# Gadersd/stable-diffusion-xl-burn

Measured on AMD Instinct MI355X. Metric: images/sec SDXL-base 1024x1024 30-step CFG7.5 (whole job); UNet step ms p50, higher is better.
Workload: dtype f16; 1 GPU; SDXL-base 1024x1024, n_steps=30 (31 CFG UNet step pairs), CFG 7.5, batch 1 prompt/GPU + VAE decode to u8 (BASELINE configs[1]); precision=f16, vae_dtype=f32_split, weights=synthetic seeded (random-init SDXL-base architecture), mix_classes=0, parallelism=replica x1, 1 prompt per GPU, weights broadcast once over RCCL, hipgraph=True, split_cfg=False, fused_xattn=True, pipelined_decode=False, prompts_per_call=1, full=False, library=stable-diffusion-xl-burn_amd/lib/libsdxl_mi355.so, debug_set=

## Files before the change

include/sdxl_mi355.h:

```cpp
#ifndef SDXL_MI355_H
#define SDXL_MI355_H

#include <stddef.h>
#include <stdint.h>

#ifdef __cplusplus
extern "C" {
#endif

typedef struct sdxl_ctx sdxl_ctx;
typedef struct sdxl_unet sdxl_unet;
typedef struct sdxl_diffuser sdxl_diffuser;
typedef struct sdxl_vae sdxl_vae;
typedef struct sdxl_clip sdxl_clip;

enum { SDXL_OK = 0, SDXL_ERR_INVALID = 1, SDXL_ERR_RUNTIME = 2 };
enum {
  SDXL_DTYPE_F32 = 0,
  SDXL_DTYPE_F16 = 1,
  SDXL_DTYPE_F16_F32RES = 2,
  SDXL_DTYPE_F32_SPLIT = 3,
  SDXL_DTYPE_F32_SPLIT_MIX = 4,
  SDXL_DTYPE_F32_SPLIT_MIX_F16W = 5,
  SDXL_DTYPE_F32_SPLIT_MIX_F16W_GEGLU2 = 6,
// ... 147 lines not shown
int sdxl_clip_create_synthetic(sdxl_ctx* ctx, const sdxl_clip_config* cfg, int dtype, uint64_t seed, sdxl_clip** out);
void sdxl_clip_destroy(sdxl_clip* c);
int sdxl_clip_forward_hidden(sdxl_clip* c, void* stream, const int32_t* tokens, int n, int seq, int hidden_idx, float* out_hidden);
int sdxl_clip_forward_hidden_pooled(sdxl_clip* c, void* stream, const int32_t* tokens, int n, int seq, int hidden_idx,
                                    float* out_hidden, float* out_pooled);
int sdxl_conditioning_embedding(sdxl_ctx* ctx, void* stream, const float* pooled, int n, int E, const int32_t* values, int w,
                                int dim, float* out);
int sdxl_clip_weight_arena(sdxl_clip* c, void** base, size_t* bytes);

int sdxl_unet_weight_arena(sdxl_unet* u, void** base, size_t* bytes);
int sdxl_vae_weight_arena(sdxl_vae* v, void** base, size_t* bytes);
int sdxl_diffuser_create_empty(sdxl_ctx* ctx, const sdxl_unet_config* cfg, int dtype, const float* alphas_cumprod_host,
                               int n_train_steps, sdxl_diffuser** out);
int sdxl_vae_create_empty(sdxl_ctx* ctx, const sdxl_vae_config* cfg, int dtype, int with_encoder, sdxl_vae** out);

typedef struct sdxl_comm sdxl_comm;
int sdxl_comm_unique_id(void* id_out_128);
int sdxl_comm_create(int device_id, int rank, int world, const void* id_128, sdxl_comm** out);
void sdxl_comm_destroy(sdxl_comm* c);
int sdxl_bcast_buffer(sdxl_comm* c, void* stream, void* base_dev, size_t bytes, int root);
int sdxl_unet_bcast_weights(sdxl_comm* c, sdxl_unet* u, int root);
int sdxl_vae_bcast_weights(sdxl_comm* c, sdxl_vae* v, int root);
int sdxl_clip_bcast_weights(sdxl_comm* c, sdxl_clip* k, int root);
int sdxl_bcast_plan(size_t bytes, int world, int rank, size_t* piece_off, size_t* piece_len, size_t* tail_off, size_t* tail_len);

int sdxl_unet_profile(sdxl_unet* u, void* stream, int B, int H, int W, float class_ms[5], int class_launches[5],
                      double class_flops[5]);
int sdxl_unet_eager_forward_ms(sdxl_unet* u, void* stream, int B, int H, int W, float* ms_out);
int sdxl_bench_igemm(sdxl_ctx* ctx, void* stream, int B, int H, int W, int Cin, int Cout, int ksize, int geglu, int iters,
                     float* avg_ms);
int sdxl_bench_attention(sdxl_ctx* ctx, void* stream, int B, int H, int Nq, int Nk, int iters, float* avg_ms);
int sdxl_debug_set(const char* key, int value);
int sdxl_debug_warm_schedule(int n, const unsigned* bytes, const unsigned char* host, int* warmed_by);
enum {
  SDXL_SEL_WF = 1 << 0, SDXL_SEL_R = 1 << 1, SDXL_SEL_EBIAS = 1 << 2, SDXL_SEL_STAT_OUT = 1 << 3, SDXL_SEL_LN_STAT = 1 << 4, SDXL_SEL_GN_PART = 1 << 5,
  SDXL_SEL_SHADOW = 1 << 6, SDXL_SEL_XA_K = 1 << 7, SDXL_SEL_XA_K_LO = 1 << 8, SDXL_SEL_ACC_SCALE = 1 << 9, SDXL_SEL_SPLITK_WS = 1 << 10,
  SDXL_SEL_XSPLIT_WS = 1 << 11, SDXL_SEL_MASK = 1 << 12, SDXL_SEL_WARM = 1 << 13
};
typedef struct sdxl_select_knobs {
  int igemm_variant, igemm_wreg, wreg_xattn, hl_tile96, igemm_tsw, igemm_unrolled, wide_db, attn_variant, attn_xsplit, zero_page;
} sdxl_select_knobs;
typedef struct sdxl_igemm_case {
  int batch, rows_per_entry;
  int N, cin, ksize, stride, up;
  int act, n_split;
  int a_dt, c_dt, compute_dt;
  int xa_nctx, shadow_lo_sign;
  unsigned present; int misaligned;
} sdxl_igemm_case;
typedef struct sdxl_igemm_choice {
  int family, bm, bn, ns, wgm, nw, elem, a_elem, xa, xh, tsw, s2, splitk, mode, db, measure, grid, block, lds;
  int gn_part_ok, wreg_selected, wreg_xattn_selected;
} sdxl_igemm_choice;
int sdxl_debug_igemm_select(const sdxl_igemm_case* c, const sdxl_select_knobs* knobs, sdxl_igemm_choice* out);
typedef struct sdxl_attn_case { int B, H, Nq, Nk, dt; unsigned present; int misaligned; } sdxl_attn_case;
typedef struct sdxl_attn_choice { int kernel, mix, big_heads, ns, elem, ko, grid_x, grid_y, block, lds; } sdxl_attn_choice;
int sdxl_debug_attn_select(const sdxl_attn_case* c, const sdxl_select_knobs* knobs, sdxl_attn_choice* out);

int sdxl_group_norm(sdxl_ctx* ctx, void* stream, const float* x, const float* gamma, const float* beta, int B, int C,
                    int HW, int n_group, float eps, int silu, int dtype, float* out);
int sdxl_layer_norm(sdxl_ctx* ctx, void* stream, const float* x, const float* gamma, const float* beta, int rows, int C,
                    float eps, int dtype, float* out);
int sdxl_conv2d(sdxl_ctx* ctx, void* stream, const float* x, const float* weight, const float* bias, int B, int Cin,
                int H, int W, int Cout, int ksize, int stride, int pad, int upsample, int dtype, float* out);
int sdxl_linear(sdxl_ctx* ctx, void* stream, const float* x, const float* weight, const float* bias, int M, int K, int N,
                int geglu, int dtype, float* out);
int sdxl_layer_norm_linear(sdxl_ctx* ctx, void* stream, const float* x, const float* gamma, const float* beta, float eps,
                           const float* weight, const float* bias, int M, int K, int N, int geglu, int dtype, float* out);

int sdxl_ln_query_cross_attention(sdxl_ctx* ctx, void* stream, const float* x, const float* gamma, const float* beta, float eps,
                                  const float* wq, const float* k, const float* v, int B, int Nq, int Nk, int C, int fused,
                                  float* out);

enum { SDXL_FORM_NATIVE = 0, SDXL_FORM_F16 = 1, SDXL_FORM_F16_WHILO = 2, SDXL_FORM_F16_AHILO = 3, SDXL_FORM_X2 = 4 };
enum { SDXL_PROJ_QKV = 0, SDXL_PROJ_QUERY = 1, SDXL_PROJ_GEGLU = 2 };
int sdxl_transformer_projection(sdxl_ctx* ctx, void* stream, int B, int rows_per_entry, int C, const float* a, const float* wp, const float* bp,
                                const float* r, int Kp, int producer_form, const float* gamma, const float* beta, float eps, const float* w,
                                const float* b, int N, int proj, int form, int shadow, float* t_out, float* out, int* shadow_taken);

int sdxl_conv2d_group_norm(sdxl_ctx* ctx, void* stream, const float* x, const float* weight, const float* bias, const float* residual,
                           const float* gamma, const float* beta, float eps, int B, int Cin, int H, int W, int Cout, int n_group,
                           int silu, int fused, int* fused_taken, float* out);

#ifdef __cplusplus
}
#endif
#endif
```

stable-diffusion-xl-burn_amd/__init__.py:

```python
from __future__ import annotations

import ctypes
import os
from dataclasses import dataclass, field
from typing import List, Optional, Sequence, Tuple

import numpy as np

_HERE = os.path.dirname(os.path.abspath(__file__))
LIB_PATH = os.path.join(_HERE, "lib", "libsdxl_mi355_measure.so" if os.environ.get("SDXL_MEASURE_LIB") == "1" else "libsdxl_mi355.so")
if os.environ.get("SDXL_LIB_PATH"):
    LIB_PATH = os.environ["SDXL_LIB_PATH"]

DTYPE_F32 = 0
DTYPE_F16 = 1
DTYPE_F16_F32RES = 2
DTYPE_F32_SPLIT_MIX_F16W = 5
DTYPE_F32_SPLIT_MIX_F16W_GEGLU2 = 6
DTYPE_F32_SPLIT_F16W = 7
DTYPE_F32_SPLIT_MIX = 4
DTYPE_F32_SPLIT = 3

_c_p = ctypes.c_void_p
_f_p = ctypes.c_void_p
# ... 22 lines not shown
class _ClipConfigC(ctypes.Structure):
    _fields_ = [(n, ctypes.c_int32) for n in ("n_vocab", "n_state", "embed_dim", "n_head", "n_ctx", "n_layer", "quick_gelu")]


class _ConditioningC(ctypes.Structure):
    _fields_ = [("unconditional_context_full", _f_p), ("unconditional_context_open_clip", _f_p),
                ("context_full", _f_p), ("context_open_clip", _f_p), ("unconditional_channel_context", _f_p),
                ("unconditional_channel_context_refiner", _f_p), ("channel_context", _f_p),
                ("channel_context_refiner", _f_p), ("n", ctypes.c_int32), ("n_ctx", ctypes.c_int32),
                ("height", ctypes.c_int32), ("width", ctypes.c_int32)]


class LoraEntry(ctypes.Structure):
    _fields_ = [("param_index", ctypes.c_int32), ("rank", ctypes.c_int32), ("left", _f_p), ("right", _f_p), ("scale", ctypes.c_float)]


LORA_ROUND_F16 = 1


ABI_SYMBOLS = [
    "sdxl_last_error", "sdxl_build_info", "sdxl_ctx_create", "sdxl_ctx_destroy", "sdxl_ctx_synchronize",
    "sdxl_unet_config_base", "sdxl_unet_config_refiner", "sdxl_vae_config_default",
    "sdxl_unet_param_count", "sdxl_unet_param_spec", "sdxl_vae_param_count", "sdxl_vae_param_spec",
    "sdxl_unet_create", "sdxl_unet_create_synthetic", "sdxl_unet_destroy", "sdxl_unet_forward", "sdxl_unet_set_graph", "sdxl_unet_set_split_cfg", "sdxl_unet_set_fused_cross_attention", "sdxl_unet_set_gn_from_producer", "sdxl_unet_mix_classes",
    "sdxl_qkv_attention", "sdxl_attn_decoder_mask",
    "sdxl_diffuser_create", "sdxl_diffuser_create_synthetic", "sdxl_diffuser_destroy", "sdxl_diffuser_unet",
    "sdxl_sample_latent", "sdxl_sample_latent_with_inpainting", "sdxl_refine_latent", "sdxl_step_count",
    "sdxl_diffuser_enable_step_timing", "sdxl_diffuser_step_times", "sdxl_diffuser_set_trace",
    "sdxl_gen_noise", "sdxl_sample_latent_seeded", "sdxl_sample_latent_with_inpainting_seeded", "sdxl_refine_latent_seeded",
    "sdxl_diffuser_set_solver", "sdxl_diffuser_get_solver", "sdxl_solver_coefficients",
    "sdxl_vae_create", "sdxl_vae_create_synthetic", "sdxl_vae_destroy", "sdxl_vae_decode_latent",
    "sdxl_latent_to_image", "sdxl_vae_encode_image", "sdxl_image_to_latent",
    "sdxl_unet_weight_arena", "sdxl_vae_weight_arena", "sdxl_diffuser_create_empty", "sdxl_vae_create_empty",
    "sdxl_unet_profile", "sdxl_unet_eager_forward_ms", "sdxl_bench_igemm", "sdxl_bench_attention", "sdxl_debug_set", "sdxl_debug_warm_schedule", "sdxl_debug_igemm_select", "sdxl_debug_attn_select",
    "sdxl_group_norm", "sdxl_layer_norm", "sdxl_conv2d", "sdxl_linear", "sdxl_layer_norm_linear", "sdxl_ln_query_cross_attention", "sdxl_conv2d_group_norm",
    "sdxl_transformer_projection",
    "sdxl_lora_check", "sdxl_lora_merge", "sdxl_unet_create_lora", "sdxl_diffuser_create_lora",
    "sdxl_clip_config_clip_l", "sdxl_clip_config_open_clip_bigg", "sdxl_clip_param_count", "sdxl_clip_param_spec",
    "sdxl_clip_create", "sdxl_clip_create_synthetic", "sdxl_clip_destroy", "sdxl_clip_forward_hidden",
    "sdxl_clip_forward_hidden_pooled", "sdxl_conditioning_embedding", "sdxl_clip_weight_arena",
    "sdxl_unet_create_f16", "sdxl_diffuser_create_f16", "sdxl_vae_create_f16", "sdxl_clip_create_f16",
    "sdxl_comm_unique_id", "sdxl_comm_create", "sdxl_comm_destroy", "sdxl_bcast_buffer", "sdxl_unet_bcast_weights",
    "sdxl_vae_bcast_weights", "sdxl_clip_bcast_weights", "sdxl_bcast_plan",
]

_lib = None


def lib() -> ctypes.CDLL:
    global _lib
    if _lib is None:
        if not os.path.exists(LIB_PATH):
            raise EngineError(f"{LIB_PATH} is missing: run `python stable-diffusion-xl-burn_amd/build.py` "
                              "(hipcc --offload-arch=gfx950). There is no fallback path.")
        try:
            import torch
        except ImportError:
            pass
        l = ctypes.CDLL(LIB_PATH)
        l.sdxl_last_error.restype = ctypes.c_char_p
        l.sdxl_build_info.restype = ctypes.c_char_p
        l.sdxl_diffuser_unet.restype = ctypes.c_void_p
        l.sdxl_diffuser_unet.argtypes = [ctypes.c_void_p]
        for name in ("sdxl_ctx_destroy", "sdxl_unet_destroy", "sdxl_diffuser_destroy", "sdxl_vae_destroy", "sdxl_clip_destroy",
                     "sdxl_comm_destroy"):
            getattr(l, name).restype = None
            getattr(l, name).argtypes = [ctypes.c_void_p]
# ... 834 lines not shown
    return out


def layer_norm(ctx: Context, x, gamma, beta, eps: float = 1e-5, dtype: int = DTYPE_F16):
    torch = _torch()
    x, px = _dev(x)
    gamma, pg = _dev(gamma)
    beta, pb = _dev(beta)
    C = x.shape[-1]
    out = torch.empty_like(x)
    _check(lib().sdxl_layer_norm(ctx.h, _stream(), px, pg, pb, int(x.numel() // C), C, ctypes.c_float(eps), dtype,
                                ctypes.c_void_p(out.data_ptr())))
    return out


def conv2d(ctx: Context, x, weight, bias, stride: int = 1, padding: int = 0, upsample: bool = False,
           dtype: int = DTYPE_F16):
    torch = _torch()
    x, px = _dev(x)
    weight, pw = _dev(weight)
    pb = None
    if bias is not None:
        bias, pb = _dev(bias)
    B, Cin, H, W = x.shape
    Cout, _, k, _ = weight.shape
    Hs, Ws = (2 * H, 2 * W) if upsample else (H, W)
    Ho, Wo = (Hs + 2 * padding - k) // stride + 1, (Ws + 2 * padding - k) // stride + 1
    out = torch.empty((B, Cout, Ho, Wo), device=x.device, dtype=torch.float32)
    _check(lib().sdxl_conv2d(ctx.h, _stream(), px, pw, pb, B, Cin, H, W, Cout, k, stride, padding, int(upsample), dtype,
                            ctypes.c_void_p(out.data_ptr())))
    return out


def linear(ctx: Context, x, weight, bias, geglu: bool = False, dtype: int = DTYPE_F16):
    torch = _torch()
    x, px = _dev(x)
    weight, pw = _dev(weight)
    pb = None
    if bias is not None:
        bias, pb = _dev(bias)
    K, N = weight.shape
    M = int(x.numel() // K)
    out = torch.empty(tuple(x.shape[:-1]) + ((N // 2) if geglu else N,), device=x.device, dtype=torch.float32)
    _check(lib().sdxl_linear(ctx.h, _stream(), px, pw, pb, M, K, N, int(geglu), dtype, ctypes.c_void_p(out.data_ptr())))
    return out


def layer_norm_linear(ctx: Context, x, gamma, beta, weight, bias, eps: float = 1e-5, geglu: bool = False,
                      dtype: int = DTYPE_F16):
    torch = _torch()
    x, px = _dev(x)
    gamma, pg = _dev(gamma)
    beta, pbeta = _dev(beta)
    weight, pw = _dev(weight)
    pb = None
    if bias is not None:
        bias, pb = _dev(bias)
    K, N = weight.shape
    M = int(x.numel() // K)
    out = torch.empty(tuple(x.shape[:-1]) + ((N // 2) if geglu else N,), device=x.device, dtype=torch.float32)
    _check(lib().sdxl_layer_norm_linear(ctx.h, _stream(), px, pg, pbeta, ctypes.c_float(eps), pw, pb, M, K, N, int(geglu),
                                       dtype, ctypes.c_void_p(out.data_ptr())))
    return out


def ln_query_cross_attention(ctx: Context, x, gamma, beta, wq, k, v, eps: float = 1e-5, fused: bool = True):
# ... 112 lines not shown
```

stable-diffusion-xl-burn_amd/build.py:

```python
from __future__ import annotations

import hashlib
import os
import subprocess
import sys
from concurrent.futures import ThreadPoolExecutor

HERE = os.path.dirname(os.path.abspath(__file__))
CSRC = os.path.join(HERE, "csrc")
OBJ = os.path.join(HERE, "build")
LIBDIR = os.path.join(HERE, "lib")
LIB = os.path.join(LIBDIR, "libsdxl_mi355.so")
ARCH = "gfx950"
SOURCES = ["igemm.hip", "igemm_glds.hip", "igemm_wreg.hip", "igemm_measure.hip", "norm.hip", "attention.hip", "elementwise.hip", "capi.hip", "capi_ops.hip",
           "select.cpp", "specs.cpp", "weights.cpp", "unet.cpp", "vae.cpp", "sampler.cpp", "clip.cpp", "comm.cpp"]
FLAGS = ["-O3", "-std=c++17", "-fPIC", f"--offload-arch={ARCH}", "-Wall", "-Wno-unused-function",
         "-Wno-unused-result"]


def _hipcc() -> str:
    for c in (os.environ.get("HIPCC"), "/opt/rocm/bin/hipcc", "hipcc"):
        if c and (os.path.isabs(c) and os.path.exists(c) or not os.path.isabs(c)):
            return c
    raise RuntimeError("hipcc not found")


def _measure() -> bool:
    return os.environ.get("SDXL_MEASURE") == "1"


def _paths():
    return (OBJ + "_measure", LIB.replace(".so", "_measure.so")) if _measure() else (OBJ, LIB)


def _flags() -> list:
    return FLAGS + (["-DSDXL_MEASURE"] if _measure() else [])


def _deps_hash(src: str) -> str:
    h = hashlib.sha256()
    for f in [src] + [os.path.join(CSRC, x) for x in ("kernels.h", "engine.h", "igemm_common.h", "capi_internal.h", "select_debug.h")] + \
            [os.path.join(HERE, "..", "include", "sdxl_mi355.h")]:
        with open(f, "rb") as fh:
            h.update(fh.read())
    h.update(" ".join(_flags()).encode())
    return h.hexdigest()


def _compile(name: str, force: bool) -> str:
    src = os.path.join(CSRC, name)
    obj = os.path.join(_paths()[0], name + ".o")
    stamp = obj + ".sha"
    want = _deps_hash(src)
    if not force and os.path.exists(obj) and os.path.exists(stamp) and open(stamp).read() == want:
        return obj
    cmd = [_hipcc()] + _flags() + (["-x", "hip"] if name.endswith(".hip") else []) + ["-c", src, "-o", obj]
    r = subprocess.run(cmd, capture_output=True, text=True)
    if r.returncode != 0:
        raise RuntimeError(f"hipcc failed for {name}:\n{r.stdout}\n{r.stderr}")
    with open(stamp, "w") as fh:
        fh.write(want)
    return obj


def build(force: bool = False, verbose: bool = True) -> str:
    obj_dir, lib = _paths()
    os.makedirs(obj_dir, exist_ok=True)
    os.makedirs(LIBDIR, exist_ok=True)
    with ThreadPoolExecutor(max_workers=min(8, len(SOURCES))) as ex:
        objs = list(ex.map(lambda n: _compile(n, force), SOURCES))
    newest = max(os.path.getmtime(o) for o in objs)
    if force or not os.path.exists(lib) or os.path.getmtime(lib) < newest:
        cmd = [_hipcc(), "-shared", "-fPIC", f"--offload-arch={ARCH}", "-o", lib] + objs + ["-ldl"]
        r = subprocess.run(cmd, capture_output=True, text=True)
# ... 12 lines not shown
```

stable-diffusion-xl-burn_amd/csrc/capi.hip:

```cpp
#include "capi_internal.h"
#include "select_debug.h"
#include <algorithm>
#include <cstring>

using namespace sdxl;

thread_local std::string sdxl::g_err;

namespace {
template <class H, class F> void create_handle(sdxl_ctx* ctx, H** out, F make) {
  std::unique_ptr<H> h(new H());
  h->ctx = ctx;
  make(*h);
  *out = h.release();
}
UNetCfg to_cfg(const sdxl_unet_config* c) {
  SDXL_REQUIRE(c != nullptr, "null config");
  SDXL_REQUIRE(c->n_levels >= 1 && c->n_levels <= 8, "n_levels out of range");
  UNetCfg u;
  u.adm_in_channels = c->adm_in_channels; u.in_channels = c->in_channels; u.out_channels = c->out_channels;
  u.model_channels = c->model_channels; u.n_head_channels = c->n_head_channels; u.context_dim = c->context_dim;
  u.is_refiner = c->is_refiner != 0;
  for (int i = 0; i < c->n_levels; ++i) { u.channel_mults.push_back(c->channel_mults[i]); u.transformer_depths.push_back(c->transformer_depths[i]); }
  SDXL_REQUIRE(u.model_channels > 0 && u.n_head_channels > 0 && u.context_dim > 0 && u.adm_in_channels > 0, "bad UNet config");
  return u;
}
ClipCfg to_ccfg(const sdxl_clip_config* c) {
  SDXL_REQUIRE(c != nullptr, "null config");
  ClipCfg k;
  k.n_vocab = c->n_vocab; k.n_state = c->n_state; k.embed_dim = c->embed_dim; k.n_head = c->n_head; k.n_ctx = c->n_ctx;
  k.n_layer = c->n_layer; k.quick_gelu = c->quick_gelu != 0;
  return k;
}
VaeCfg to_vcfg(const sdxl_vae_config* c) {
// ... 73 lines not shown
#ifdef SDXL_MEASURE
  return "sdxl_mi355 engine, HIP kernels for gfx950 (CDNA4, wave64, MFMA 32x32x16 f16 / 32x32x2 f32) [measure build: A/B variants + debug knobs]";
#else
  return "sdxl_mi355 engine, HIP kernels for gfx950 (CDNA4, wave64, MFMA 32x32x16 f16 / 32x32x2 f32)";
#endif
}

int sdxl_ctx_create(int device_id, sdxl_ctx** out) {
  API_BEGIN
  SDXL_REQUIRE(out != nullptr, "null out");
  int n = 0;
  SDXL_HIP(hipGetDeviceCount(&n));
  SDXL_REQUIRE(n > 0, "no HIP device visible: the MI355X engine has no CPU fallback");
  SDXL_REQUIRE(device_id >= 0 && device_id < n, "device id out of range");
  SDXL_HIP(hipSetDevice(device_id));
  sdxl_ctx* c = new sdxl_ctx();
  c->device = device_id;
  SDXL_HIP(hipStreamCreate(&c->stream));
  igemm_glds_init();
  *out = c;
  API_END
}
int sdxl_debug_set(const char* key, int value) {
  API_BEGIN
  SDXL_REQUIRE(key != nullptr, "null key");
  if (select_knob_set(key, value)) return SDXL_OK;
  else if (std::strcmp(key, "igemm_epilogue_staged") == 0) igemm_set_epilogue_staged(value);
  else if (std::strcmp(key, "hl_weights_exact") == 0) igemm_set_hl_weights_exact(value);
  else if (std::strcmp(key, "igemm_warm") == 0) igemm_set_warm(value);
  else if (std::strcmp(key, "splitk_wt") == 0) igemm_set_splitk_wt(value);
  else if (std::strcmp(key, "hl_demote") == 0) unet_set_hl_demote(value);
  else if (std::strcmp(key, "mix_classes") == 0) unet_set_mix_classes(value);
  else if (std::strcmp(key, "wreg_xcd2d") == 0) igemm_set_wreg_xcd2d(value);
#ifdef SDXL_MEASURE
  else if (std::strcmp(key, "xa_vec64") == 0) igemm_set_xa_vec64(value);
  else if (std::strcmp(key, "no_cfg") == 0) g_debug_no_cfg = value != 0;
#endif
  else throw Error(std::string("unknown debug key ") + key);
  API_END
}
int sdxl_debug_warm_schedule(int n, const unsigned* bytes, const unsigned char* host, int* warmed_by) {
  API_BEGIN
  WarmSeq ws;
  for (int j = 0; j < n; ++j)
    ws.seq.push_back(WarmSeq::Item{reinterpret_cast<const void*>((uintptr_t)(j + 1) << 12), bytes[j], host[j] != 0, host[j] ? 14u << 20 : 0u, {nullptr, nullptr, nullptr}, {0u, 0u, 0u}});
  ws.finish();
  for (int j = 0; j < n; ++j) warmed_by[j] = -1;
  for (int i = 0; i < n; ++i)
    for (int r = 0; r < 3; ++r)
      if (ws.seq[i].warm[r]) warmed_by[(int)(reinterpret_cast<uintptr_t>(ws.seq[i].warm[r]) >> 12) - 1] = i;
  API_END
}
int sdxl_debug_igemm_select(const sdxl_igemm_case* c, const sdxl_select_knobs* knobs, sdxl_igemm_choice* out) {
  API_BEGIN
  SDXL_REQUIRE(c && knobs && out, "null argument");
  const IgemmParams p = select_debug_igemm(*c);
  const SelectKnobs k = select_debug_knobs(*knobs);
  *out = sdxl_igemm_choice{};
  out->gn_part_ok = igemm_gn_part_ok(p, k); out->wreg_selected = igemm_wreg_selected(p, k); out->wreg_xattn_selected = igemm_wreg_xattn_selected(p, k);
  const IgemmChoice s = igemm_select(p, c->compute_dt, k);
  out->family = s.family; out->bm = s.bm; out->bn = s.bn; out->ns = s.ns; out->wgm = s.wgm; out->nw = s.nw; out->elem = s.elem; out->a_elem = s.a_elem;
  out->xa = s.xa; out->xh = s.xh; out->tsw = s.tsw; out->s2 = s.s2; out->splitk = s.splitk; out->mode = s.mode; out->db = s.db; out->measure = s.measure;
  out->grid = s.grid; out->block = s.block; out->lds = s.lds;
  API_END
}
int sdxl_debug_attn_select(const sdxl_attn_case* c, const sdxl_select_knobs* knobs, sdxl_attn_choice* out) {
  API_BEGIN
  SDXL_REQUIRE(c && knobs && out, "null argument");
  const AttnChoice s = attn_select(select_debug_attn(*c), select_debug_knobs(*knobs));
  *out = sdxl_attn_choice{s.kernel, s.mix, s.big_heads, s.ns, s.elem, s.ko, s.grid_x, s.grid_y, s.block, s.lds};
  API_END
}
#ifdef SDXL_MEASURE
int sdxl_debug_timeline(void* device_buf) {
  API_BEGIN
  igemm_set_timeline(device_buf);
  API_END
}
int sdxl_debug_timeline_words(void) { return igemm_timeline_words(); }
int sdxl_debug_attn_timeline(void* device_buf) {
  API_BEGIN
  attention_set_timeline(device_buf);
  API_END
// ... 534 lines not shown
```

stable-diffusion-xl-burn_amd/csrc/capi_ops.hip:

```cpp
#include "capi_internal.h"
#include <algorithm>
#include <cmath>

using namespace sdxl;

namespace {
__global__ void transpose_pad_kernel(const float* src, int lds_, int rows, int C, void* dst, int dt, int ldd) {
  const size_t i = (size_t)blockIdx.x * blockDim.x + threadIdx.x;
  if (i >= (size_t)rows * C) return;
  const int r = i / C, c = i - (size_t)r * C;
  const float v = src[(size_t)r * lds_ + c];
  if (dt == DT_F16) reinterpret_cast<_Float16*>(dst)[(size_t)c * ldd + r] = (_Float16)v;
  else reinterpret_cast<float*>(dst)[(size_t)c * ldd + r] = v;
}
__global__ void causal_mask_kernel(float* out, int n) {
  const int i = blockIdx.x * blockDim.x + threadIdx.x;
  if (i >= n * n) return;
  const int r = i / n, c = i - r * n;
  out[i] = c > r ? -INFINITY : 0.f;
}

struct Operand { std::string name; std::vector<int> shape; int kind; const float* data = nullptr; float eps = 0.f; int ld = 0; };
using Operands = std::vector<Operand>;
void add_linear(Operands& o, const std::string& n, int K, int N, const float* w, const float* b, int ld = 0) {
// ... 288 lines not shown
                int W, int Cout, int ksize, int stride, int pad, int upsample, int dtype, float* out) {
  API_BEGIN
  SDXL_REQUIRE(ctx && x && weight && out, "null argument");
  use(ctx);
  hipStream_t s = pick(ctx, stream);
  int cdt, sdt;
  if (dtype == SDXL_DTYPE_F32_SPLIT) { cdt = DT_HL; sdt = DT_HL; }
  else { no_mix(dtype); dtypes(dtype, cdt, sdt); }
  SDXL_REQUIRE(cdt != DT_HL || Cin % 32 == 0, "SDXL_DTYPE_F32_SPLIT convolutions need Cin % 32 == 0");
  const int Hs = upsample ? 2 * H : H, Ws = upsample ? 2 * W : W;
  const int Ho = (Hs + 2 * pad - ksize) / stride + 1, Wo = (Ws + 2 * pad - ksize) / stride + 1;
  Operands ops;
  add_conv(ops, "conv", Cout, Cin, ksize, weight, bias);
  Packed pk(ops, cdt, s);
  const Lin l = pk.wb.conv("conv");
  Tmp tmp;
  void* xi = tmp.get((size_t)B * H * W * Cin * dt_size(sdt));
  float* yo = (float*)tmp.get((size_t)B * Ho * Wo * Cout * sizeof(float));
  Act xa(xi, Cin, sdt);
  if (cdt == DT_HL) {
    float* x32 = (float*)tmp.get((size_t)B * H * W * Cin * sizeof(float));
    float* sc = (float*)tmp.get(hl_scale_floats(B) * sizeof(float));
    launch_nchw_to_nhwc(x, Cin * H * W, x32, DT_F32, B, Cin, H * W, Cin, 1.0f, s);
    launch_f32_to_hl_scaled(x32, Cin, xi, Cin, (size_t)B * H * W, Cin, sc, s, B);
    xa.a_scale = hl_scale_inv(sc, B); xa.a_scale_n = B;
  } else launch_nchw_to_nhwc(x, Cin * H * W, xi, sdt, B, Cin, H * W, Cin, 1.0f, s);
  Exec ex; ex.s = s; ex.cdt = cdt; ex.sdt = sdt;
  give_splitk_ws(ex, tmp, B, Ho * Wo, Cout, s);
  run_conv(ex, l, xa, Cin, ConvGeom{B, H, W, Ho, Wo, ksize, stride, pad, upsample ? 1 : 0}, Act(yo, Cout, DT_F32));
  launch_nhwc_to_nchw(yo, DT_F32, Cout, out, B, Cout, Ho * Wo, 1.0f, s);
  SDXL_HIP(hipStreamSynchronize(s));
  API_END
}
int sdxl_linear(sdxl_ctx* ctx, void* stream, const float* x, const float* weight, const float* bias, int M, int K, int N,
                int geglu, int dtype, float* out) {
  API_BEGIN
  SDXL_REQUIRE(ctx && x && weight && out, "null argument");
  SDXL_REQUIRE(!geglu || (N % 32 == 0), "GEGLU width must be a multiple of 32");
  use(ctx);
  hipStream_t s = pick(ctx, stream);
  int cdt, sdt;
  if (dtype == SDXL_DTYPE_F32_SPLIT) { cdt = DT_HL; sdt = DT_HL; }
  else { no_mix(dtype); dtypes(dtype, cdt, sdt); }
  SDXL_REQUIRE(cdt != DT_HL || K % 32 == 0, "SDXL_DTYPE_F32_SPLIT linear layers need K % 32 == 0");
  Operands ops;
  add_linear(ops, "lin", K, N, weight, bias);
  Packed pk(ops, cdt, s);
  const Lin l = pk.wb.linear("lin", geglu != 0);
  Tmp tmp;
  void* xi = tmp.get((size_t)M * K * dt_size(sdt));
  Act xa(xi, K, sdt);
  if (cdt == DT_HL) {
    float* sc = (float*)tmp.get(hl_scale_floats(1) * sizeof(float));
    launch_f32_to_hl_scaled(x, K, xi, K, (size_t)M, K, sc, s, 1);
    xa.a_scale = hl_scale_inv(sc, 1);
  } else launch_copy_rows(x, DT_F32, K, xi, sdt, K, M, K, s);
  Exec ex; ex.s = s; ex.cdt = cdt; ex.sdt = sdt;
  give_splitk_ws(ex, tmp, 1, M, N, s);
  Epi e; e.act = geglu ? 1 : 0;
  run_linear(ex, l, xa, M, Act(out, geglu ? N / 2 : N, DT_F32), e);
  SDXL_HIP(hipStreamSynchronize(s));
  API_END
}
int sdxl_layer_norm_linear(sdxl_ctx* ctx, void* stream, const float* x, const float* gamma, const float* beta, float eps,
                           const float* weight, const float* bias, int M, int K, int N, int geglu, int dtype, float* out) {
  API_BEGIN
// ... 237 lines not shown
```

stable-diffusion-xl-burn_amd/csrc/elementwise.hip:

```cpp
#include "kernels.h"
#include <algorithm>
#include <stdexcept>

namespace sdxl {

typedef _Float16 half_t;
typedef _Float16 half8 __attribute__((ext_vector_type(8)));
typedef float f32x4 __attribute__((ext_vector_type(4)));

__device__ __forceinline__ float ld_f(const void* p, size_t i, int dt) {
  if (dt == DT_HL) { const half_t* b = reinterpret_cast<const half_t*>(p) + ((i >> 4) << 5) + (i & 15); return (float)b[0] + (float)b[16]; }
  return dt == DT_F16 ? (float)reinterpret_cast<const half_t*>(p)[i] : reinterpret_cast<const float*>(p)[i];
}
__device__ __forceinline__ void st_f(void* p, size_t i, int dt, float v) {
  if (dt == DT_HL) {
    half_t* b = reinterpret_cast<half_t*>(p) + ((i >> 4) << 5) + (i & 15);
    const half_t hi = (half_t)v;
    b[0] = hi; b[16] = (half_t)(v - (float)hi);
  } else if (dt == DT_F16) reinterpret_cast<half_t*>(p)[i] = (half_t)v; else reinterpret_cast<float*>(p)[i] = v;
}
__device__ __forceinline__ float silu_f(float x) { return x / (1.0f + expf(-x)); }

template <typename WT>
__global__ __launch_bounds__(256) void gemv_kernel(const GemvParams p, int cols) {
  constexpr int CE = 16 / sizeof(WT);
  extern __shared__ __attribute__((aligned(16))) float gx[];
  const int lane = threadIdx.x & 63, wave = threadIdx.x >> 6;
  const int Kx = (p.K + 64 * CE - 1) / (64 * CE) * (64 * CE);
  for (int i = threadIdx.x; i < p.Bm * Kx; i += 256) {
    const int b = i / Kx, k = i - b * Kx;
    float x = 0.f;
    if (k < p.K) {
      x = p.X[(size_t)b * p.ldx + k];
// ... 772 lines not shown
  for (int o = 32; o > 0; o >>= 1) acc += __shfl_xor(acc, o);
  if (lane == 0) cs[row] = acc;
}
void launch_colsum_packed(const void* wp, int dt, int Kpad, int nrows, float* cs, hipStream_t s, const float* kscale, int K, int interleave) {
  hipLaunchKernelGGL(colsum_packed_kernel, dim3((nrows + 3) / 4), dim3(256), 0, s, wp, dt, Kpad, nrows, cs, kscale, K, interleave);
}
__global__ void beta_dot_kernel(const float* w, const float* beta, const float* bias, float* out, int K, int N) {
  const int n = blockIdx.x * blockDim.x + threadIdx.x;
  if (n >= N) return;
  float acc = bias ? bias[n] : 0.f;
  for (int k = 0; k < K; ++k) acc += beta[k] * w[(size_t)k * N + n];
  out[n] = acc;
}
void launch_beta_dot(const float* w, const float* beta, const float* bias, float* out, int K, int N, hipStream_t s) {
  hipLaunchKernelGGL(beta_dot_kernel, dim3((N + 255) / 256), dim3(256), 0, s, w, beta, bias, out, K, N);
}
__global__ void pack_conv_kernel(const float* src, void* dst, int dt, int Cout, int Cin, int ks, int Kpad, int Npad, float wscale) {
  const size_t i = (size_t)blockIdx.x * blockDim.x + threadIdx.x;
  if (i >= (size_t)Npad * Kpad) return;
  const int n = i / Kpad;
  const int k = i - (size_t)n * Kpad;
  float v = 0.f;
  if (n < Cout && k < ks * ks * Cin) {
    const int tap = k / Cin, c = k - tap * Cin;
    const int ky = tap / ks, kx = tap - ky * ks;
    v = src[(((size_t)n * Cin + c) * ks + ky) * ks + kx] * wscale;
  }
  st_f(dst, i, dt, v);
}
void launch_pack_conv(const float* src, void* dst, int dt, int Cout, int Cin, int ks, int Kpad, int Npad, hipStream_t s, float wscale) {
  const size_t total = (size_t)Npad * Kpad;
  hipLaunchKernelGGL(pack_conv_kernel, dim3((total + 255) / 256), dim3(256), 0, s, src, dst, dt, Cout, Cin, ks, Kpad, Npad, wscale);
}
__global__ void pack_bias_kernel(const float* src, float* dst, int N, int Npad, int geglu, int n_offset) {
  const int i = blockIdx.x * blockDim.x + threadIdx.x;
  if (i >= Npad) return;
  float v = 0.f;
  if (i < N && src) v = src[geglu ? geglu_unpermute(i, N) : i];
  dst[n_offset + i] = v;
}
void launch_pack_bias(const float* src, float* dst, int N, int Npad, int geglu, int n_offset, hipStream_t s) {
  hipLaunchKernelGGL(pack_bias_kernel, dim3((Npad + 255) / 256), dim3(256), 0, s, src, dst, N, Npad, geglu, n_offset);
}

}
```

stable-diffusion-xl-burn_amd/csrc/engine.h:

```cpp
#pragma once
#include "kernels.h"

#include <map>
#include <memory>
#include <stdexcept>
#include <string>
#include <utility>
#include <vector>

namespace sdxl {

struct Error : std::runtime_error {
  explicit Error(const std::string& m) : std::runtime_error(m) {}
};
#define SDXL_HIP(x)                                                                                   \
  do {                                                                                                \
    hipError_t e__ = (x);                                                                             \
    if (e__ != hipSuccess) throw ::sdxl::Error(std::string(#x) + " failed: " + hipGetErrorString(e__)); \
  } while (0)
#define SDXL_REQUIRE(cond, msg)                          \
  do {                                                   \
    if (!(cond)) throw ::sdxl::Error(std::string(msg));  \
  } while (0)

// ... 70 lines not shown
struct FlatSourceF16 : WeightSource {
  const uint16_t* base; std::vector<size_t> offsets;
  void* stage = nullptr; size_t stage_numel = 0;
  FlatSourceF16(const uint16_t* b, const std::vector<ParamSpec>& specs);
  ~FlatSourceF16() override;
  void fetch(const ParamSpec& s, size_t index, float* dst_dev, hipStream_t st) override;
};

struct LoraEntry { int param_index = 0, rank = 0; const float* left = nullptr; const float* right = nullptr; float scale = 0.f; };
constexpr int kLoraRoundF16 = 1;
std::string lora_check(const std::vector<ParamSpec>& specs, const LoraEntry* entries, int n_entries);
struct LoraSource : WeightSource {
  WeightSource& inner;
  std::vector<LoraEntry> entries;
  std::vector<std::vector<int>> by_param;
  int flags;
  float* stage = nullptr; size_t stage_numel = 0;
  LoraSource(WeightSource& in, const std::vector<ParamSpec>& specs, const LoraEntry* e, int n_entries, int flags);
  ~LoraSource() override;
  void fetch(const ParamSpec& s, size_t index, float* dst_dev, hipStream_t st) override;
  bool empty() const override { return inner.empty(); }
};

struct Lin {
  const void* w = nullptr; const float* b = nullptr;
  const void* wf = nullptr;
  int N = 0, K = 0, Kpad = 0, Npad = 0, ksize = 1, cin = 0;
  const float* cs = nullptr;
  const float* ln_eps = nullptr;
  int ln_k = 0;
  int k_form = 0;
  int dt = -1;
  const float* acc_scale = nullptr;
};
struct NormW { const float* gamma = nullptr; const float* beta = nullptr; const float* eps = nullptr; int C = 0; };

struct WeightBuilder {
  const std::vector<ParamSpec>& specs;
  std::map<std::string, size_t> index;
  WeightSource& src;
  DeviceArena& arena;
  int dt;
  hipStream_t st;
  float* tmp = nullptr; size_t tmp_numel = 0;
  std::string last_fetched;
  WeightBuilder(const std::vector<ParamSpec>& sp, WeightSource& s, DeviceArena& a, int dtype, hipStream_t stream);
  ~WeightBuilder();
  bool wfrag = true;
  static size_t arena_bound(const std::vector<ParamSpec>& specs, int dt, bool wfrag = true);
  const ParamSpec& spec(const std::string& name, size_t* idx = nullptr) const;
  bool has(const std::string& name) const { return index.count(name) != 0; }
  const float* fetch(const std::string& name);
  Lin linear(const std::string& name, bool geglu = false, int dt_override = -1);
  Lin fused_linear(const std::vector<std::string>& names, int dt_override = -1);
  Lin linear_hilo(const std::string& name, bool geglu, bool dup = false, bool hl_interleave = false);
  float hl_scale(Lin& l, const std::vector<std::string>& weight_names);
  Lin linear_ln(const std::string& name, bool geglu, const std::string& norm, bool xattn_query = false);
  Lin fused_linear_ln(const std::vector<std::string>& names, const std::string& norm);
  Lin fold_ln(const std::vector<std::string>& names, const std::string& norm, bool geglu, int dt_override = -1, bool shadow = false, Lin* plain = nullptr, bool hilo_dup = false,
              bool hl_interleave = false);
  bool all_f16_exact(const std::vector<std::string>& names);
  float* tmp2 = nullptr; size_t tmp2_numel = 0;
  Lin conv(const std::string& name);
  void attach_wfrag(Lin& l, bool fill, bool folded = false);
  NormW norm(const std::string& name);
};

struct Act {
  void* p = nullptr; int ld = 0; int dt = DT_F16;
  const float* gn_part = nullptr; int gn_rt = 0;
  const float* a_scale = nullptr;
  int a_scale_n = 1;
  Act() {}
  Act(void* p_, int ld_, int dt_) : p(p_), ld(ld_), dt(dt_) {}
  Act cols(int c0) const { Act a((char*)p + (size_t)c0 * dt_size(dt), ld, dt); a.a_scale = a_scale; a.a_scale_n = a_scale_n; return a; }
};

struct Profiler {
  enum { IGEMM = 0, ATTENTION = 1, GROUPNORM = 2, LAYERNORM = 3, OTHER = 4, NCLS = 5 };
  struct Rec { hipEvent_t a, b; int cls; double flops; int m, n, k, ks, tag; };
  std::vector<Rec> recs;
  void begin(int cls, double flops, hipStream_t s, int m = 0, int n = 0, int k = 0, int ks = 0, int tag = 0);
  void end(hipStream_t s);
  void collect(float ms[NCLS], int launches[NCLS], double flops[NCLS]);
};

struct WarmSeq {
  struct Item { const void* w; unsigned bytes; bool host; unsigned budget; const void* warm[3]; unsigned warm_bytes[3]; };
  std::vector<Item> seq;
  size_t pos = 0;
  bool recording = false, ready = false;
  void finish();
};
struct Exec {
  Profiler* prof = nullptr;
  hipStream_t s = nullptr;
// ... 19 lines not shown
  MIX_ATTN_F16 = 1,
  MIX_GEGLU_F16 = 2,
  MIX_QKV_F16 = 4,
  MIX_FF_F16 = 8,
  MIX_OUT1_F16 = 16,
  MIX_OUT2_F16 = 32,
  MIX_XATTN_F16 = 64,
  MIX_Q2_F16 = 128,
  MIX_XATTN_SPLIT = 512,
  MIX_GEGLU_HILO = 1024,
  MIX_GEGLU_AHILO = 2048,
  MIX_LINEAR_F16X2 = 4096,
  MIX_LN_SHADOW = 256
};
enum DemoteClass { DM_QKV = 1, DM_ATTN = 2, DM_OUT = 4, DM_XATTN = 8, DM_GEGLU = 16, DM_FF = 32, DM_CONV_RES = 64, DM_CONV_SKIP = 128,
                   DM_CONV_IO = 256, DM_CONV_UPDOWN = 512, DM_CONV_PROJ = 1024 };
void unet_set_mix_classes(int v);
void unet_set_hl_demote(int mask);
int unet_hl_demote();

struct ConvGeom { int B, Hin, Win, Hout, Wout, ksize, stride, pad, up; };
struct Epi {
  const float* ln_stat = nullptr;
  float* stat_out = nullptr;
  const float* ebias = nullptr; int ebias_ld = 0;
  int act = 0;
  Act R;
  int n_split = -1;
  void* Ct = nullptr; int ct_rows = 0, ct_ld = 0;
  int rpb = 0;
  const void* xa_k = nullptr; int xa_nctx = 0; float xa_scale = 0.f;
  const void* xa_k_lo = nullptr;
  float* gn_part = nullptr;
  int cls = 0;
  void* shadow = nullptr; int shadow_ld = 0; const float* shadow_gamma = nullptr; bool* shadow_done = nullptr; float shadow_lo_scale = 0.f;
};
bool run_conv(Exec& ex, const Lin& w, const Act& a, int cin, const ConvGeom& g, const Act& out, const Epi& e = Epi());
bool run_linear(Exec& ex, const Lin& w, const Act& a, int M, const Act& out, const Epi& e = Epi());
Act hl_operand(Exec& ex, const Lin& w, const Act& x, size_t rows, int C, int nb = 1, float* have_max = nullptr);
void run_groupnorm(Exec& ex, const NormW& n, const Act& x, int B, int HW, const Act& y, bool silu, int groups = 32, float* absmax_out = nullptr);
void run_layernorm(Exec& ex, const NormW& n, const Act& x, int rows, const Act& y, float dup_scale = 0.f);

struct ResBlockW { NormW norm_in, norm_out; Lin conv_in, conv_out, skip; bool has_skip = false; int emb_off = 0, cin = 0, cout = 0; };
struct TBlockW { NormW n1, n2, n3; Lin qkv, out1, q2, kv2, out2, geglu, ff;
                 Lin qkv_sh, q2_sh, geglu_sh; };
enum LinForm {
  LF_NATIVE,
  LF_F16,
  LF_F16_WHILO,
  LF_F16_AHILO,
  LF_X2
};
inline bool packs_f16_values(LinForm f) { return f == LF_F16 || f == LF_F16_AHILO || f == LF_X2; }
enum XattnForm { XA_LAUNCH, XA_F16, XA_SPLIT };
struct StPlan {
  LinForm qkv = LF_NATIVE, out1 = LF_NATIVE, q2 = LF_NATIVE, out2 = LF_NATIVE, geglu = LF_NATIVE, ff = LF_NATIVE;
  bool qkv_sh = false, q2_sh = false, geglu_sh = false;
  bool attn_f16 = false;
  XattnForm xattn = XA_LAUNCH;
};
struct STW { NormW norm; Lin proj_in, proj_out; std::vector<TBlockW> blocks; int C = 0, heads = 0; StPlan plan; };
Lin pack_proj(WeightBuilder& wb, LinForm f, const std::vector<std::string>& names, bool geglu, Lin* sh = nullptr, const std::string& norm = "");
inline bool reads_f16(LinForm f) { return f == LF_F16 || f == LF_F16_WHILO || f == LF_F16_AHILO; }
inline Act x2_operand(LinForm f, const Act& a) { return f == LF_X2 ? Act(a.p, 2 * a.ld, DT_F16) : a; }
struct LnOperands {
  Act ln;
  Act ln16;
  Act ln16x2;
  Act sh16; float* shst = nullptr;
  Act sh16g;
// ... 82 lines not shown
  hipGraphExec_t graph_ = nullptr;
  const float* graph_t_ = nullptr; int graph_ts_ = 0; int plan_runs_ = 0;
};

struct VaeResW { NormW n1, n2; Lin c1, c2, nin; bool has_nin = false; int cin = 0, cout = 0; };
struct VaeMidW { VaeResW b1, b2; NormW an; Lin q, k, v, proj; int C = 0; };

class Vae {
 public:
  Vae(const VaeCfg& cfg, int compute_dt, WeightSource* dec_src, WeightSource* enc_src, hipStream_t st);
  ~Vae();
  const VaeCfg& cfg() const { return cfg_; }
  const float* decode(const float* latent_nchw, int n, int h, int w, hipStream_t s);
  void decode_nchw(const float* latent_nchw, int n, int h, int w, float* out_nchw, hipStream_t s);
  void latent_to_image(const float* latent_nchw, int n, int h, int w, unsigned char* out_hwc, hipStream_t s);
  void encode_nchw(const float* img_nchw, int n, int H, int W, float* latent_out, hipStream_t s);
  void image_to_latent(const unsigned char* img_hwc, int n, int H, int W, float* latent_out, hipStream_t s);
  size_t weight_bytes() const { return warena_.off; }
  void* weight_base() const { return warena_.base; }

 private:
  void res_block(Exec& ex, const VaeResW& w, const Act& x, int B, int H, int W, const Act& out);
  void mid(Exec& ex, const VaeMidW& w, const Act& x, int B, int H, int W);
  void run_decode(Exec& ex, const Act& in, int n, int h, int w, const Act& out);
  void run_encode(Exec& ex, const Act& in, int n, int H, int W, const Act& out);
  VaeResW load_res(WeightBuilder& wb, const std::string& p, int cin, int cout);
  VaeMidW load_mid(WeightBuilder& wb, const std::string& p, int c);

  VaeCfg cfg_;
  int cdt_;
  DeviceArena warena_;
  bool has_dec_ = false, has_enc_ = false;
  Lin post_quant_, d_conv_in_, d_conv_out_; NormW d_norm_out_; VaeMidW d_mid_;
  struct DecBlk { VaeResW r[3]; Lin up; bool has_up = false; };
  std::vector<DecBlk> d_blocks_;
  Lin quant_, e_conv_in_, e_conv_out_; NormW e_norm_out_; VaeMidW e_mid_;
  struct EncBlk { VaeResW r[2]; Lin down; bool has_down = false; };
  std::vector<EncBlk> e_blocks_;
  DeviceArena act_;
  size_t act_peak_ = 0;
  float* gn_workspace(Exec& ex, int n);
  int io_dt() const { return cdt_ == DT_HL ? DT_F32 : cdt_; }
};

struct ClipBlockW { NormW attn_ln, mlp_ln; Lin qkv, out, fc1, fc2; };

class ClipText {
 public:
  ClipText(const ClipCfg& cfg, int compute_dt, int stream_dt, WeightSource& src, hipStream_t st);
  ~ClipText();
  void set_use_graph(bool g) { use_graph_ = g; }
  const ClipCfg& cfg() const { return cfg_; }
  void forward_hidden(const int* ids, int B, int S, int hidden_idx, float* out, hipStream_t s);
  void forward_hidden_pooled(const int* ids, int B, int S, int hidden_idx, float* hidden, float* pooled, hipStream_t s);
  size_t weight_bytes() const { return warena_.off; }
  void* weight_base() const { return warena_.base; }

 private:
  void run(const int* ids, int B, int S, int n_blocks, int tap, float* hidden, float* pooled, hipStream_t s);
  void block(Exec& ex, const ClipBlockW& w, const Act& x, int B, int S, const Act& ln, const Act& qk, void* vt, int npad,
             const Act& ao, const Act& h);
  ClipCfg cfg_;
  int cdt_, sdt_;
  DeviceArena warena_, act_;
  const void* tok_ = nullptr; const void* pos_ = nullptr;
  std::vector<ClipBlockW> blocks_;
  NormW final_ln_; Lin proj_;
// ... 67 lines not shown
```

stable-diffusion-xl-burn_amd/csrc/igemm_common.h:

```cpp
#pragma once
#include "kernels.h"
#include <stdexcept>
#include <type_traits>

namespace sdxl {

typedef _Float16 half_t;
typedef _Float16 half8 __attribute__((ext_vector_type(8)));
typedef _Float16 half4 __attribute__((ext_vector_type(4)));
typedef float f32x4 __attribute__((ext_vector_type(4)));
typedef float f32x16 __attribute__((ext_vector_type(16)));

typedef const __attribute__((address_space(1))) void* gptr_t;
typedef float f32x8 __attribute__((ext_vector_type(8)));
__device__ __forceinline__ f32x8 uniform_load8(const float* ptr) {
  const unsigned long long a = (unsigned long long)(uintptr_t)ptr;
  const unsigned long long u = ((unsigned long long)__builtin_amdgcn_readfirstlane((unsigned)(a >> 32)) << 32) | (unsigned)__builtin_amdgcn_readfirstlane((unsigned)a);
  return *(const __attribute__((address_space(4))) f32x8*)(uintptr_t)u;
}
__device__ __forceinline__ f32x4 col_vec4(const float* arr, bool present, int nbu, int fh, const void* zeros) {
  const f32x8 c = uniform_load8(present ? arr + nbu : reinterpret_cast<const float*>(zeros));
  return fh ? f32x4{c[4], c[5], c[6], c[7]} : f32x4{c[0], c[1], c[2], c[3]};
}
typedef __attribute__((address_space(3))) void* lptr_t;
// ... 87 lines not shown
  __device__ __forceinline__ static float combine(const float (&P)[NC]) {
    if constexpr (TPR == 4) { const float t = P[0] + __shfl_xor(P[0], 1); return t + __shfl_xor(t, 2); }
    else { const float u = P[0] + __shfl_xor(P[0], 1), w = P[1] + __shfl_xor(P[1], 1); return u + w; }
  }
  __device__ __forceinline__ void finish(const IgemmParams& p, int m0, float* coef) {
    if (!live) return;
    float P[NC];
#pragma unroll
    for (int c = 0; c < NC; ++c) {
      P[c] = 0.f;
#pragma unroll
      for (int q = 0; q < PERC; ++q) if (sub + c * TPR + 4 * q < p.ln_slots) P[c] += v[c][q][0];
    }
    const float mu = combine(P) / (float)p.ln_slots;
    float Q[NC], D[NC];
#pragma unroll
    for (int c = 0; c < NC; ++c) {
      Q[c] = 0.f; D[c] = 0.f;
#pragma unroll
      for (int q = 0; q < PERC; ++q)
        if (sub + c * TPR + 4 * q < p.ln_slots) { const float d = v[c][q][0] - mu; Q[c] += v[c][q][1]; D[c] = fmaf(d, d, D[c]); }
    }
    const float s2 = combine(Q), sd = combine(D);
    const float var = (s2 + 64.f * sd) * p.ln_invc;
    const float a = 1.0f / sqrtf(var + (p.ln_eps_ptr ? *p.ln_eps_ptr : p.ln_eps));
    if (sub == 0) {
      const bool ok = m0 + row < p.M;
      coef[row * 2] = ok ? a : 1.f;
      coef[row * 2 + 1] = ok ? -a * mu : 0.f;
    }
  }
};

template <int TM, int TN>
__device__ __forceinline__ void igemm_epilogue(const IgemmParams& p, const f32x16 (&acc)[TM][TN], int mw, int nw, int fr, int fh,
                                               const float (&lnA)[TM], const float (&lnC)[TM]) {
  const bool geglu = p.act == 1;
  const int nlim = geglu ? (p.N >> 1) : p.N;
#pragma unroll
  for (int i = 0; i < TM; ++i) {
    const int m = mw + i * 32 + fr;
    if (m >= p.M) continue;
    const int bidx = m / p.rpb;
    const int key = m - bidx * p.rpb;
    const float lna = lnA[i], lnc = lnC[i];
#pragma unroll
    for (int j = 0; j < TN; ++j) {
      const int nt = nw + j * 32;
#pragma unroll
      for (int q = 0; q < 4; ++q) {
        if (geglu && q >= 2) continue;
        const int nb = nt + 8 * q + 4 * fh;
        if (nb >= p.N) continue;
        float v[4];
#pragma unroll
        for (int r = 0; r < 4; ++r) v[r] = acc[i][j][q * 4 + r];
        if (p.ln_stat) {
          const f32x4 cz = *reinterpret_cast<const f32x4*>(p.ln_cs + nb);
#pragma unroll
          for (int r = 0; r < 4; ++r) v[r] = lna * v[r] + lnc * cz[r];
        }
        if (p.bias) {
          const f32x4 bz = *reinterpret_cast<const f32x4*>(p.bias + nb);
#pragma unroll
          for (int r = 0; r < 4; ++r) v[r] += bz[r];
        }
        if (p.ebias) {
          const f32x4 ez = *reinterpret_cast<const f32x4*>(p.ebias + (size_t)bidx * p.ebias_ld + nb);
#pragma unroll
          for (int r = 0; r < 4; ++r) v[r] += ez[r];
        }
        int nout = nb;
        if (geglu) {
          f32x4 gz = {0.f, 0.f, 0.f, 0.f};
          if (p.bias) gz = *reinterpret_cast<const f32x4*>(p.bias + nb + 16);
          f32x4 gc = {0.f, 0.f, 0.f, 0.f};
          if (p.ln_stat) gc = *reinterpret_cast<const f32x4*>(p.ln_cs + nb + 16);
#pragma unroll
          for (int r = 0; r < 4; ++r) v[r] *= gelu_erf2(lna * acc[i][j][(q + 2) * 4 + r] + lnc * gc[r] + gz[r]);
          nout = (nt >> 1) + 8 * q + 4 * fh;
        }
        if (geglu || nb < p.n_split) {
          const bool vec = nout + 3 < nlim && (nout & 3) == 0;
          if (p.R) {
            if (vec && p.r_dt == DT_F16 && (p.ldr & 3) == 0) {
              const half4 rr = *reinterpret_cast<const half4*>(reinterpret_cast<const half_t*>(p.R) + (size_t)m * p.ldr + nout);
#pragma unroll
              for (int r = 0; r < 4; ++r) v[r] += (float)rr[r];
            } else if (vec && p.r_dt == DT_F32 && (p.ldr & 3) == 0) {
              const f32x4 rr = *reinterpret_cast<const f32x4*>(reinterpret_cast<const float*>(p.R) + (size_t)m * p.ldr + nout);
#pragma unroll
              for (int r = 0; r < 4; ++r) v[r] += rr[r];
            } else {
#pragma unroll
              for (int r = 0; r < 4; ++r)
                if (nout + r < nlim)
                  v[r] += p.r_dt == DT_F16 ? (float)reinterpret_cast<const half_t*>(p.R)[(size_t)m * p.ldr + nout + r]
                                           : reinterpret_cast<const float*>(p.R)[(size_t)m * p.ldr + nout + r];
            }
          }
          if (vec && p.c_dt == DT_F16 && (p.ldc & 3) == 0) {
            half4 h; h[0] = (half_t)v[0]; h[1] = (half_t)v[1]; h[2] = (half_t)v[2]; h[3] = (half_t)v[3];
            *reinterpret_cast<half4*>(reinterpret_cast<half_t*>(p.C) + (size_t)m * p.ldc + nout) = h;
          } else if (vec && p.c_dt == DT_F32 && (p.ldc & 3) == 0) {
            f32x4 o = {v[0], v[1], v[2], v[3]};
            *reinterpret_cast<f32x4*>(reinterpret_cast<float*>(p.C) + (size_t)m * p.ldc + nout) = o;
          } else {
#pragma unroll
            for (int r = 0; r < 4; ++r)
              if (nout + r < nlim) {
                if (p.c_dt == DT_F16) reinterpret_cast<half_t*>(p.C)[(size_t)m * p.ldc + nout + r] = (half_t)v[r];
                else reinterpret_cast<float*>(p.C)[(size_t)m * p.ldc + nout + r] = v[r];
              }
          }
        } else {
#pragma unroll
          for (int r = 0; r < 4; ++r)
            if (nb + r < p.N) {
              const size_t o = ((size_t)bidx * p.ct_rows + (nb + r - p.n_split)) * p.ct_ld + key;
              if (p.c_dt == DT_F16) reinterpret_cast<half_t*>(p.Ct)[o] = (half_t)v[r];
              else reinterpret_cast<float*>(p.Ct)[o] = v[r];
            }
        }
      }
    }
  }
}

__host__ __device__ constexpr int pipe_lds_total(int ring, int extra) { return ring + extra + 2048 <= 163840 ? ring + extra + 2048 : ring + extra; }

typedef int warm_i32x4 __attribute__((ext_vector_type(4)));
template <int NT>
__device__ __forceinline__ void igemm_warm_body(const void* base, unsigned bytes, int wi, int nw) {
  const char* b = reinterpret_cast<const char*>(base);
  constexpr unsigned span = NT * 16, step = span * 8;
  warm_i32x4 acc = {0, 0, 0, 0};
  for (size_t off = (size_t)wi * step; off < bytes; off += (size_t)nw * step) {
    warm_i32x4 v[8];
#pragma unroll
    for (int u = 0; u < 8; ++u) {
      const size_t o = off + (size_t)u * span + (size_t)threadIdx.x * 16;
      v[u] = o + 16 <= bytes ? *reinterpret_cast<const warm_i32x4*>(b + o) : warm_i32x4{0, 0, 0, 0};
    }
#pragma unroll
    for (int u = 0; u < 8; ++u) acc ^= v[u];
// ... 115 lines not shown
    bool rfast[NIT];
    constexpr bool GNP = TM == 2 && TN == 2 && !GEGLU;
    const bool gnp = GNP && gc != nullptr && p.gn_part != nullptr;
    float gpiv[8], gs1[8], gs2[8];
#pragma unroll
    for (int e = 0; e < 8; ++e) { gpiv[e] = 0.f; gs1[e] = 0.f; gs2[e] = 0.f; }
    float st_piv[NIT], st_s1[NIT], st_s2[NIT];
    size_t st_off[NIT];
    bool st_ok[NIT];
#pragma unroll
    for (int it = 0; it < NIT; ++it) { st_piv[it] = 0.f; st_s1[it] = 0.f; st_s2[it] = 0.f; st_off[it] = 0; st_ok[it] = false; }
#pragma unroll
    for (int it = 0; it < NIT; ++it) {
      const int idx = it * 64 + lane;
      const int row = idx / LPR, piece = idx - row * LPR;
      const int n0 = nwo + piece * 8;
      const int m = mw + row;
      const half_t* rp = reinterpret_cast<const half_t*>(p.R) + (size_t)m * p.ldr + n0;
      rfast[it] = p.R && p.r_dt == DT_F16 && idx < ITEMS && m < p.M && n0 + 8 <= nlim && (reinterpret_cast<uintptr_t>(rp) & 15) == 0;
      rpre[it] = *(rfast[it] ? reinterpret_cast<const half8*>(rp) : reinterpret_cast<const half8*>(zeros));
    }
#pragma unroll
    for (int it = 0; it < NIT; ++it) {
      const int idx = it * 64 + lane;
      const int row = idx / LPR, piece = idx - row * LPR;
      if (ITEMS % 64 != 0 && idx >= ITEMS) continue;
      const int n0 = nwo + piece * 8;
      const int m = mw + row;
      const f32x4 a = *reinterpret_cast<const f32x4*>(lds + row * RB + (((2 * piece) ^ (row & SWN)) << 4));
      const f32x4 b = *reinterpret_cast<const f32x4*>(lds + row * RB + (((2 * piece + 1) ^ (row & SWN)) << 4));
      const bool valid = m < p.M && n0 < nlim;
      float rr[8] = {0.f, 0.f, 0.f, 0.f, 0.f, 0.f, 0.f, 0.f};
      if (valid) {
      float v[8] = {a[0], a[1], a[2], a[3], b[0], b[1], b[2], b[3]};
      const bool full = n0 + 8 <= nlim;
      if (rfast[it]) {
#pragma unroll
        for (int e = 0; e < 8; ++e) v[e] += (float)rpre[it][e];
      } else if (p.R) {
        if (p.r_dt == DT_F16) {
          const half_t* rp = reinterpret_cast<const half_t*>(p.R) + (size_t)m * p.ldr + n0;
          if (full && (reinterpret_cast<uintptr_t>(rp) & 15) == 0) {
            const half8 rr = *reinterpret_cast<const half8*>(rp);
#pragma unroll
            for (int e = 0; e < 8; ++e) v[e] += (float)rr[e];
          } else {
#pragma unroll
            for (int e = 0; e < 8; ++e) if (n0 + e < nlim) v[e] += (float)rp[e];
          }
        } else {
          const float* rp = reinterpret_cast<const float*>(p.R) + (size_t)m * p.ldr + n0;
          if (full && (reinterpret_cast<uintptr_t>(rp) & 15) == 0) {
            const f32x4 r0 = *reinterpret_cast<const f32x4*>(rp), r1 = *reinterpret_cast<const f32x4*>(rp + 4);
#pragma unroll
            for (int e = 0; e < 4; ++e) { v[e] += r0[e]; v[4 + e] += r1[e]; }
          } else {
#pragma unroll
            for (int e = 0; e < 8; ++e) if (n0 + e < nlim) v[e] += rp[e];
          }
        }
      }
      if (p.stat_out || gnp) {
#pragma unroll
        for (int e = 0; e < 8; ++e) rr[e] = p.c_dt == DT_F16 ? (float)(half_t)v[e] : v[e];
      }
      if (p.c_dt == DT_F16) {
        half_t* cp = reinterpret_cast<half_t*>(p.C) + (size_t)m * p.ldc + n0;
        if (full && (reinterpret_cast<uintptr_t>(cp) & 15) == 0) {
          half8 h;
#pragma unroll
          for (int e = 0; e < 8; ++e) h[e] = (half_t)v[e];
          *reinterpret_cast<half8*>(cp) = h;
        } else {
#pragma unroll
          for (int e = 0; e < 8; ++e) if (n0 + e < nlim) cp[e] = (half_t)v[e];
        }
      } else if (p.c_dt == DT_HL) {
        if (full) store_hl8(reinterpret_cast<float*>(p.C) + (size_t)m * p.ldc, n0, v);
      } else {
        float* cp = reinterpret_cast<float*>(p.C) + (size_t)m * p.ldc + n0;
        if (full && (reinterpret_cast<uintptr_t>(cp) & 15) == 0) {
          *reinterpret_cast<f32x4*>(cp) = f32x4{v[0], v[1], v[2], v[3]};
          *reinterpret_cast<f32x4*>(cp + 4) = f32x4{v[4], v[5], v[6], v[7]};
        } else {
#pragma unroll
          for (int e = 0; e < 8; ++e) if (n0 + e < nlim) cp[e] = v[e];
        }
      }
      }
      if constexpr (GNP) {
        if (gnp) {
          if (it == 0) {
#pragma unroll
            for (int e = 0; e < 8; ++e) gpiv[e] = __shfl(rr[e], lane & 7);
          }
#pragma unroll
          for (int e = 0; e < 8; ++e) { const float d = rr[e] - gpiv[e]; gs1[e] += d; gs2[e] = fmaf(d, d, gs2[e]); }
        }
      }
      if constexpr (COLS % 64 == 0) {
        if (p.stat_out) {
          const float piv = __shfl(rr[0], lane & ~7);
          float s1 = 0.f, s2 = 0.f;
#pragma unroll
          for (int e = 0; e < 8; ++e) { const float d = rr[e] - piv; s1 += d; s2 = fmaf(d, d, s2); }
          st_piv[it] = piv; st_s1[it] = s1; st_s2[it] = s2;
          st_ok[it] = (piece & 7) == 0 && valid;
          st_off[it] = ((size_t)(n0 >> 6) * p.M + m) * 2;
        }
      }
    }
    if constexpr (COLS % 64 == 0) {
      if (p.stat_out) {
// ... 89 lines not shown
          const int m = mbase + e;
          if (m < p.M) {
            const int bb = m / p.rpb;
            reinterpret_cast<float*>(p.Ct)[((size_t)bb * p.ct_rows + (n - p.n_split)) * p.ct_ld + (m - bb * p.rpb)] = v[e];
          }
        }
      }
    }
  }
}

template <int TM, int TN, bool GEGLU>
__device__ __forceinline__ bool igemm_rows_ok(const IgemmParams& p, int nw) {
  constexpr int WN = TN * 32;
  const int nlim = GEGLU ? (p.N >> 1) : (p.n_split < p.N ? p.n_split : p.N);
  const int n_lo = GEGLU ? (nw >> 1) : nw, n_w = GEGLU ? WN / 2 : WN;
  if (n_lo + n_w > nlim || p.gn_part) return false;
  if ((p.ldc & 7) != 0 || (reinterpret_cast<uintptr_t>(p.C) & 15) != 0) return false;
  if (p.R && ((p.ldr & 7) != 0 || (reinterpret_cast<uintptr_t>(p.R) & 15) != 0)) return false;
  if (p.stat_out && (TN != 2 || GEGLU)) return false;
  if (p.ebias && (p.ebias_ld & 3) != 0) return false;
  return true;
}
struct NoStamp { __device__ __forceinline__ void operator()(int) const {} };
template <int TM, int TN, bool GEGLU, typename ST = NoStamp>
__device__ __forceinline__ void igemm_epilogue_rows(const IgemmParams& p, const f32x16 (&acc)[TM][TN], int mw, int nw, int lane,
                                                    const float (&lnA)[TM], const float (&lnC)[TM], const void* zeros, const ST& stamp = ST()) {
  const int fr = lane & 31, fh = lane >> 5;
  const f32x4* zv = reinterpret_cast<const f32x4*>(zeros);
  constexpr int NQ = GEGLU ? 2 : 4;
  constexpr int NP = NQ / 2;
  const int nwo = GEGLU ? (nw >> 1) : nw;
  int m[TM], bidx[TM];
  bool mok[TM];
#pragma unroll
  for (int i = 0; i < TM; ++i) {
    m[i] = mw + i * 32 + fr;
    mok[i] = m[i] < p.M;
    bidx[i] = (p.ebias && mok[i]) ? m[i] / p.rpb : 0;
  }
  const bool r16 = p.R && p.r_dt == DT_F16, r32 = p.R && p.r_dt == DT_F32;
  half8 rh[TM][TN][NP];
  f32x4 rf[TM][TN][NP][2];
#pragma unroll
  for (int i = 0; i < TM; ++i)
#pragma unroll
    for (int j = 0; j < TN; ++j)
#pragma unroll
      for (int t = 0; t < NP; ++t) {
        const int n0 = nwo + (GEGLU ? j * 16 : j * 32 + t * 16) + 8 * fh;
        const size_t o = (size_t)(mok[i] ? m[i] : 0) * p.ldr + n0;
        rh[i][j][t] = *((r16 && mok[i]) ? reinterpret_cast<const half8*>(reinterpret_cast<const half_t*>(p.R) + o) : reinterpret_cast<const half8*>(zeros));
        if (r32) {
          rf[i][j][t][0] = *(mok[i] ? reinterpret_cast<const f32x4*>(reinterpret_cast<const float*>(p.R) + o) : zv);
          rf[i][j][t][1] = *(mok[i] ? reinterpret_cast<const f32x4*>(reinterpret_cast<const float*>(p.R) + o + 4) : zv);
        }
      }
  stamp(0);
  float st_s1[TM][4], st_s2[TM][4], st_piv[TM];
#pragma unroll
  for (int i = 0; i < TM; ++i) {
    st_piv[i] = 0.f;
#pragma unroll
    for (int k = 0; k < 4; ++k) { st_s1[i][k] = 0.f; st_s2[i][k] = 0.f; }
  }
#pragma unroll
  for (int j = 0; j < TN; ++j) {
    const int nt = nw + j * 32;
    f32x4 bz[NQ], cz[NQ], gz[NQ], gc[NQ], ez[TM][NQ];
#pragma unroll
    for (int q = 0; q < NQ; ++q) {
      const int nb = nt + 8 * q + 4 * fh;
// ... 13 lines not shown
      const float lna = lnA[i], lnc = lnC[i];
      f32x4 v[NQ];
#pragma unroll
      for (int q = 0; q < NQ; ++q) {
#pragma unroll
        for (int r = 0; r < 4; ++r) v[q][r] = acc[i][j][q * 4 + r];
        v[q] = lna * v[q] + lnc * cz[q] + bz[q] + ez[i][q];
        if constexpr (GEGLU) {
#pragma unroll
          for (int r = 0; r < 4; ++r) v[q][r] *= gelu_erf2(lna * acc[i][j][(q + 2) * 4 + r] + lnc * gc[q][r] + gz[q][r]);
        }
      }
#pragma unroll
      for (int t = 0; t < NP; ++t) {
        float w[8];
#pragma unroll
        for (int r = 0; r < 4; ++r) {
          const auto sw = __builtin_amdgcn_permlane32_swap(__float_as_uint(v[2 * t][r]), __float_as_uint(v[2 * t + 1][r]), false, false);
          w[r] = __uint_as_float(sw[0]);
          w[4 + r] = __uint_as_float(sw[1]);
        }
        if (r16) {
#pragma unroll
          for (int e = 0; e < 8; ++e) w[e] += (float)rh[i][j][t][e];
        } else if (r32) {
#pragma unroll
          for (int e = 0; e < 4; ++e) { w[e] += rf[i][j][t][0][e]; w[4 + e] += rf[i][j][t][1][e]; }
        }
        const int n0 = nwo + (GEGLU ? j * 16 : j * 32 + t * 16) + 8 * fh;
        if (p.c_dt == DT_F16) {
          half8 h;
#pragma unroll
          for (int e = 0; e < 8; ++e) h[e] = (half_t)w[e];
          if (mok[i]) *reinterpret_cast<half8*>(reinterpret_cast<half_t*>(p.C) + (size_t)m[i] * p.ldc + n0) = h;
          if constexpr (TN == 2 && !GEGLU) {
            if (p.stat_out) {
#pragma unroll
              for (int e = 0; e < 8; ++e) w[e] = (float)h[e];
            }
          }
        } else if (p.c_dt == DT_HL) {
          if (mok[i]) store_hl8(reinterpret_cast<float*>(p.C) + (size_t)m[i] * p.ldc, n0, w);
        } else if (mok[i]) {
          float* cp = reinterpret_cast<float*>(p.C) + (size_t)m[i] * p.ldc + n0;
          *reinterpret_cast<f32x4*>(cp) = f32x4{w[0], w[1], w[2], w[3]};
          *reinterpret_cast<f32x4*>(cp + 4) = f32x4{w[4], w[5], w[6], w[7]};
        }
        if constexpr (TN == 2 && !GEGLU) {
          if (p.stat_out) {
            if (j == 0 && t == 0) st_piv[i] = __shfl(w[0], fr);
            float s1 = 0.f, s2 = 0.f;
#pragma unroll
            for (int e = 0; e < 8; ++e) { const float d = w[e] - st_piv[i]; s1 += d; s2 = fmaf(d, d, s2); }
            st_s1[i][j * 2 + t] = s1; st_s2[i][j * 2 + t] = s2;
          }
        }
      }
    }
  }
  stamp(7);
  if constexpr (TN == 2 && !GEGLU) {
    if (p.stat_out) {
#pragma unroll
      for (int i = 0; i < TM; ++i) {
#pragma unroll
        for (int k = 0; k < 4; ++k) { st_s1[i][k] += __shfl_xor(st_s1[i][k], 32); st_s2[i][k] += __shfl_xor(st_s2[i][k], 32); }
        const float s1 = (st_s1[i][0] + st_s1[i][1]) + (st_s1[i][2] + st_s1[i][3]);
        const float s2 = (st_s2[i][0] + st_s2[i][1]) + (st_s2[i][2] + st_s2[i][3]);
        if (fh == 0 && mok[i]) {
          float* dst = p.stat_out + ((size_t)(nw >> 6) * p.M + m[i]) * 2;
          dst[0] = st_piv[i] + s1 * (1.0f / 64.0f);
          dst[1] = fmaxf(s2 - s1 * s1 * (1.0f / 64.0f), 0.f);
        }
      }
    }
  }
}
// ... 342 lines not shown
```

stable-diffusion-xl-burn_amd/csrc/igemm_glds.hip:

```cpp
#include "igemm_common.h"
#include <atomic>

namespace sdxl {

template <int BM, int BN, int NS, int MINB = 2>
__global__ __launch_bounds__(256, MINB) void igemm_glds_kernel(const IgemmParams p, const void* zeros) {
  kernarg_prefetch<(int)sizeof(IgemmParams) + 8>();
  constexpr int WM = BM / 2, WN = BN / 2;
  constexpr int TM = WM / 32, TN = WN / 32;
  constexpr int AJ = BM / 32, BJ = BN / 32;
  constexpr int PER = AJ + BJ;
  constexpr int KT = 64;
  constexpr int STAGE = (BM + BN) * 128;
  extern __shared__ __attribute__((aligned(16))) char smem[];

  const int tid = threadIdx.x, lane = tid & 63;
  const int wave = __builtin_amdgcn_readfirstlane(tid >> 6);
  const int wm = wave >> 1, wn = wave & 1;

  const int tilesN = (p.N + BN - 1) / BN;
  const int nwg = gridDim.x;
  int bid = blockIdx.x;
  {
    const int q = nwg >> 3, r = nwg & 7, xcd = bid & 7, idx = bid >> 3;
// ... 130 lines not shown
  constexpr int AJ = BM / (8 * NW), BJ = (BPC + NW - 1) / NW;
  constexpr int REM = BPC % NW;
  constexpr int PER = AJ + BJ;
  static_assert(BM % (8 * NW) == 0 && WM % 32 == 0 && WN % 32 == 0 && BN % 8 == 0, "bad tile");
  constexpr int KT = 8 * CE;
  constexpr int STAGE = (BM + BN) * 128;
  constexpr bool LIN = XA;
  static_assert(NS >= 3, "counted-wait pipeline needs a ring of at least 3 slots");
  static_assert(BM * 128 + (TN - 1) * 4096 < 65536, "fragment offsets must fit the ds_read immediate");
  extern __shared__ __attribute__((aligned(16))) char smem[];
  const unsigned lds0 = (unsigned)(uintptr_t)(lptr_t)smem;

  const int tid = threadIdx.x, lane = tid & 63;
  const int wave = __builtin_amdgcn_readfirstlane(tid >> 6);
  const int wm = wave / WGN, wn = wave % WGN;
  const bool lastb = REM == 0 || wave < REM;

  const int tilesN = (p.N + BN - 1) / BN;
  const int tilesM = (p.M + BM - 1) / BM;
  const int nwg = gridDim.x;
  int bid = blockIdx.x;
  {
    const int q = nwg >> 3, r = nwg & 7, xcd = bid & 7, idx = bid >> 3;
    bid = (xcd < r ? xcd * (q + 1) : r * (q + 1) + (xcd - r) * q) + idx;
  }
  const int SK = p.splitk > 1 ? p.splitk : 1;
  const int slice = SK > 1 ? bid % SK : 0;
  if (SK > 1) bid /= SK;
  const int tile_id = bid;
  int tm, tn;
  if ((size_t)p.N * p.K > (size_t)p.M * p.Cin) { tn = bid / tilesM; tm = bid - tn * tilesM; }
  else { tm = bid / tilesN; tn = bid - tm * tilesN; }
  const int m0 = tm * BM, n0 = tn * BN;
  bool tsw_swapped = false;
  if constexpr (TSW) {
    const int ok = n0 >= p.n_split && n0 + BN <= p.N && p.c_dt == DT_F16 && p.act == 0 && !p.epi_staged && (p.rpb % BM) == 0 && m0 + BM <= p.M &&
                   (p.ct_ld & 7) == 0 && (reinterpret_cast<uintptr_t>(p.Ct) & 15) == 0 && (!p.ln_stat || p.ln_slots <= 24);
    tsw_swapped = __builtin_amdgcn_readfirstlane(ok) != 0;
  }
  auto wait_tiles = [&](auto KK) {
    constexpr int k = decltype(KK)::value;
    if constexpr (REM == 0) wait_vmcnt<PER * k>();
    else { if (lastb) wait_vmcnt<PER * k>(); else wait_vmcnt<(PER - 1) * k>(); }
  };

  const int lrow = lane >> 3, slot = lane & 7;
  const T* wptr[BJ];
#pragma unroll
  for (int j = 0; j < BJ; ++j) {
    const int row = (j * NW + wave) * 8 + lrow;
    wptr[j] = reinterpret_cast<const T*>(p.W) + (size_t)(n0 + row) * p.Kpad + (slot ^ ((row >> 1) & 7)) * CE;
  }
  const int nk_all = p.Kpad / KT;
  const int kbeg = SK > 1 ? (int)((long)slice * nk_all / SK) : 0;
  const int nk = SK > 1 ? (int)((long)(slice + 1) * nk_all / SK) - kbeg : nk_all;
  if (kbeg > 0) {
#pragma unroll
    for (int j = 0; j < BJ; ++j) wptr[j] += kbeg * KT;
  }
  constexpr bool B0_EARLY = !LIN;
  if constexpr (B0_EARLY) {
    if (nk > 0) {
      char* lb0 = smem + BM * 128 + wave * 1024;
      static_for<BJ>([&](auto J) {
        constexpr int j = decltype(J)::value;
        if (j < BJ - 1 || lastb) {
          __builtin_amdgcn_global_load_lds((gptr_t)wptr[j], (lptr_t)(lb0 + j * (NW * 1024)), 16, 0, 0);
          wptr[j] += KT;
        }
      });
      __builtin_amdgcn_sched_barrier(0);
    }
  }
  const int HWo = p.Hout * p.Wout;
  const int Hup = p.Hin << p.up, Wup = p.Win << p.up;
  const bool lin_rows = p.ksize == 1 && p.stride == 1 && p.up == 0 && p.pad == 0;
  const bool pow2 = (HWo & (HWo - 1)) == 0 && (p.Wout & (p.Wout - 1)) == 0;
  const int sh_hw = __builtin_ctz((unsigned)HWo | 0x40000000u), sh_w = __builtin_ctz((unsigned)p.Wout | 0x40000000u);
  int rb[AJ], ry[AJ], rx[AJ], rsw[AJ];
#pragma unroll
  for (int j = 0; j < AJ; ++j) {
    const int row = (j * NW + wave) * 8 + lrow;
    const int m = m0 + row;
    rsw[j] = (slot ^ ((row >> 1) & 7)) * CE;
    rb[j] = m < p.M ? m : -1; ry[j] = 0; rx[j] = 0;
    if (!lin_rows) {
      if (m < p.M) {
        int b, rem, oy;
        if (pow2) { b = m >> sh_hw; rem = m & (HWo - 1); oy = rem >> sh_w; }
        else { b = m / HWo; rem = m - b * HWo; oy = rem / p.Wout; }
        rb[j] = b; ry[j] = oy * p.stride - p.pad; rx[j] = (rem - oy * p.Wout) * p.stride - p.pad;
      } else { rb[j] = -1; ry[j] = -(1 << 28); rx[j] = 0; }
    }
  }
  const T* Ag = reinterpret_cast<const T*>(p.A);
  const T* aptr[AJ];
  int aadv[AJ];
  int s_c0 = 0, s_dy = 0, s_dx = 0;
  if (kbeg > 0) {
    const int e0 = kbeg * KT, tap = e0 / p.Cin;
    s_c0 = e0 - tap * p.Cin; s_dy = tap / p.ksize; s_dx = tap - s_dy * p.ksize;
  }
  auto retap = [&]() {
    if (lin_rows) {
#pragma unroll
      for (int j = 0; j < AJ; ++j) {
        const bool ok = rb[j] >= 0 && s_dy == 0;
        aptr[j] = ok ? Ag + (size_t)rb[j] * p.lda + rsw[j] + s_c0 : reinterpret_cast<const T*>(zeros);
        aadv[j] = ok ? KT : 0;
      }
      return;
    }
#pragma unroll
    for (int j = 0; j < AJ; ++j) {
      const int iy = ry[j] + s_dy, ix = rx[j] + s_dx;
      const bool ok = (unsigned)iy < (unsigned)Hup && (unsigned)ix < (unsigned)Wup;
      const size_t off = (((size_t)(rb[j] < 0 ? 0 : rb[j]) * p.Hin + ((ok ? iy : 0) >> p.up)) * p.Win + ((ok ? ix : 0) >> p.up)) * p.lda + rsw[j] + s_c0;
      aptr[j] = ok ? Ag + off : reinterpret_cast<const T*>(zeros);
      aadv[j] = ok ? KT : 0;
    }
  };
  retap();
  unsigned long long abase = 0, wbase = 0;
  unsigned aoff[AJ], woff[BJ];
// ... 132 lines not shown
    if (s < nk) {
      if (B0_EARLY && s == 0) issue(0, IAONLY{}); else issue(s, IALL{});
      tile_done();
    }
  __builtin_amdgcn_sched_barrier(0);
#pragma unroll
  for (int i = 0; i < TM; ++i)
#pragma unroll
    for (int j = 0; j < TN; ++j)
#pragma unroll
      for (int r = 0; r < 16; ++r) acc[i][j][r] = 0.f;
  float lnA[TM], lnC[TM];
  bool hl_wexact = false;
  const bool ln_coop = LN_COOP && p.ln_slots <= 24;
  if constexpr (LN_COOP) lnc.finish(p, m0, ln_coef);
  if (!ln_coop) ln_prologue<TM>(p, m0 + wm * WM, fr, lnA, lnC);
  if (NPRO <= nk) wait_tiles(std::integral_constant<int, NPRO - (S2 ? 2 : 1)>{}); else wait_vmcnt<0>();
  if constexpr (LN_COOP) wait_lgkmcnt<0>();
  __builtin_amdgcn_s_barrier();
  asm volatile("" ::: "memory");
  __builtin_amdgcn_sched_barrier(0);
  if (ln_coop) {
#pragma unroll
    for (int i = 0; i < TM; ++i) {
      lnA[i] = p.ln_stat ? ln_coef[(wm * WM + i * 32 + fr) * 2] : 1.f;
      lnC[i] = p.ln_stat ? ln_coef[(wm * WM + i * 32 + fr) * 2 + 1] : 0.f;
    }
  }
  if constexpr (HL) {
    const float wsc = p.acc_scale ? *p.acc_scale : 1.f;
#pragma unroll
    for (int i = 0; i < TM; ++i) {
      const int m = m0 + wm * WM + i * 32 + fr;
      const int be = p.a_scale_rpb > 0 ? (m < p.M ? m : p.M - 1) / p.a_scale_rpb : 0;
      lnA[i] = wsc * (p.a_scale ? p.a_scale[be] : 1.f); lnC[i] = 0.f;
    }
    const int wx = (p.acc_scale && p.hl_wexact_ok && p.acc_scale[1] != 0.f) ? 1 : 0;
    hl_wexact = __builtin_amdgcn_readfirstlane(wx) != 0;
  }
  ldfrag(0, 0, I0{});
  constexpr bool PERSLOT = TM > 4 || TN > 4 || NS * STAGE > 131072;
  constexpr int NSET = PERSLOT ? NS : 2;
  unsigned fa[NSET][4], fb[NSET][4];
#pragma unroll
  for (int kk = 0; kk < 4; ++kk)
#pragma unroll
    for (int q = 0; q < NSET; ++q) {
      fa[q][kk] = (basea ^ (kk << 5)) + (PERSLOT ? q * STAGE : q * 65536u);
      fb[q][kk] = (baseb ^ (kk << 5)) + (PERSLOT ? q * STAGE : q * 65536u);
    }
  auto ldf = [&](auto SO, auto KK, auto SET, auto NOB) {
    constexpr unsigned so = decltype(SO)::value;
    constexpr int kk = decltype(KK)::value, set = decltype(SET)::value;
    constexpr bool nob = decltype(NOB)::value;
    constexpr int hi = PERSLOT ? (int)(so / STAGE) : (so >= 65536u ? 1 : 0);
    constexpr unsigned lo = PERSLOT ? 0u : so - hi * 65536u;
    static_assert(lo + (TM - 1) * 4096 < 65536u && lo + (TN - 1) * 4096 < 65536u, "fragment immediate out of range");
    static_for<TM>([&](auto I) { fA[set][decltype(I)::value] = lds_read128<lo + decltype(I)::value * 4096, frag_t>(fa[hi][kk]); });
    if constexpr (!nob) static_for<TN>([&](auto J) { fB[set][decltype(J)::value] = lds_read128<lo + decltype(J)::value * 4096, frag_t>(fb[hi][kk]); });
  };
  using NB0 = std::false_type;
  auto ktile = [&](int kt, auto CUR, auto WXT) {
    constexpr bool wx = decltype(WXT)::value;
    using WX = std::integral_constant<bool, wx>;
    constexpr int NFL = wx ? TM : NF;
    constexpr int c = decltype(CUR)::value;
    constexpr int nslot = (c + 1) % NS, fl = (c + NS - (S2 ? 2 : 1)) % NS;
// ... 484 lines not shown
```

stable-diffusion-xl-burn_amd/csrc/kernels.h:

```cpp
#pragma once
#include <hip/hip_runtime.h>
#include <stdint.h>
#include <stdexcept>

namespace sdxl {

enum DType : int { DT_F32 = 0, DT_F16 = 1, DT_HL = 2 };

static inline size_t dt_size(int dt) { return dt == DT_F16 ? 2 : 4; }

struct IgemmParams {
  const void* A;
  const void* W;
  const void* Wf;
  int a_dt;
  int B, Hin, Win, Cin, lda;
  int Hout, Wout;
  int ksize, stride, pad, up;
  int M, N, K, Kpad;
  const float* bias;
  const float* ebias;
  int ebias_ld;
  int rpb;
  int act;
  const void* R; int ldr; int r_dt;
  void* C; int ldc; int c_dt;
  int n_split;
  void* Ct; int ct_rows; int ct_ld;
  const float* ln_stat; int ln_slots; const float* ln_cs; float ln_invc; float ln_eps;
  const float* ln_eps_ptr;
  float* stat_out; int stat_slots;
  float* splitk_ws; size_t splitk_ws_bytes; unsigned* splitk_cnt; int splitk;
  const void* xa_k; int xa_nctx; float xa_scale;
  const void* xa_k_lo;
  float* gn_part;
  const float* acc_scale;
  const float* a_scale;
  int a_scale_rpb;
  int hl_wexact_ok;
  int xa_vec64;
  const void* warm[3]; unsigned warm_bytes[3];
  int splitk_wt;
  int wreg_xcd2d;
  int epi_staged;
  void* shadow; int shadow_ld; const float* shadow_gamma;
  float shadow_lo_scale;
};
struct SelectKnobs {
  int igemm_variant = 0;
  int igemm_wreg = 1;
  int wreg_xattn = 1;
  int hl_tile96 = 29;
  int igemm_tsw = 1;
  int igemm_unrolled = 1;
  int wide_db = 0;
  int attn_variant = 0;
  int attn_xsplit = 1;
  int zero_page = 0;
};
bool select_knob_set(const char* key, int value);
SelectKnobs select_knobs_snapshot();
enum IgemmFamily : int { IG_NONE = 0, IG_GLDS = 1, IG_PIPE = 2, IG_WIDE = 3, IG_WREG = 4, IG_GENERIC = 5, IG_MEASURE = 6 };
struct IgemmChoice {
  int family;
  int bm, bn, ns;
  int wgm, nw;
  int elem, a_elem;
  int xa, xh, tsw, s2;
  int splitk;
  int mode, db, measure;
  int grid, block, lds;
};
IgemmChoice igemm_select(const IgemmParams& p, int compute_dt, const SelectKnobs& k);
bool igemm_gn_part_ok(const IgemmParams& p, const SelectKnobs& k);
bool igemm_wreg_selected(const IgemmParams& p, const SelectKnobs& k);
bool igemm_wreg_xattn_selected(const IgemmParams& p, const SelectKnobs& k);
bool igemm_xattn_ok(int a_dt, int c_dt, int M, int N, int K, int rpb, int n_ctx);
size_t xattn_pack_bytes(int B, int C);
void launch_xattn_pack(const void* K, const void* Vt, void* out, int B, int C, int n_ctx, int vt_ld, hipStream_t s);
int igemm_splitk_slices(const IgemmParams& p);
size_t igemm_splitk_ws_bytes(int batch, int rows_per_entry, int n_max);
constexpr int kSplitkCounters = 4096;
SelectKnobs igemm_launch_knobs();
void launch_igemm(const IgemmParams& p, int compute_dt, const SelectKnobs& knobs, hipStream_t s);
void launch_igemm(const IgemmParams& p, int compute_dt, hipStream_t s);
void launch_repack_wfrag(const void* w, void* wf, int Npad, int Kpad, hipStream_t s);
void igemm_set_warm(int v);
int igemm_warm_enabled();
void igemm_set_splitk_wt(int v);
void igemm_set_wreg_xcd2d(int v);
void igemm_set_hl_weights_exact(int v);
void igemm_set_xa_vec64(int v);
void igemm_set_epilogue_staged(int v);
#ifdef SDXL_MEASURE
void igemm_set_timeline(void* device_buf);
void igemm_set_wreg_timeline(void* device_buf);
void igemm_set_wide_timeline(void* device_buf);
int igemm_timeline_words();
#endif
constexpr int kMaxDevices = 64;
template <auto Kernel> inline void set_max_dynamic_lds(size_t lds, int dev) {
  static bool done[kMaxDevices] = {};
  if (done[dev]) return;
  if (hipFuncSetAttribute(reinterpret_cast<const void*>(Kernel), hipFuncAttributeMaxDynamicSharedMemorySize, (int)lds) != hipSuccess)
    throw std::runtime_error("hipFuncSetAttribute(MaxDynamicSharedMemorySize) failed");
  done[dev] = true;
}
const void* igemm_zero_page();
int igemm_current_device();
void igemm_glds_init();
// ... 111 lines not shown
static_assert(sizeof(StepCoef) == 32, "one table entry is eight floats in both layouts");
constexpr int kSolverDdim = 0, kSolverDpmpp2M = 1;
constexpr uint32_t kDrawInitial = 0;
constexpr uint32_t draw_blend(uint32_t i) { return 1u + 2u * i; }
constexpr uint32_t draw_sigma(uint32_t i) { return 2u + 2u * i; }
constexpr int kMaxSeeds = 8;
struct DdimSeeds { uint64_t v[kMaxSeeds]; };
struct DdimParams {
  float* latent;
  const void* eps; int eps_dt; int eps_ld;
  const StepCoef* table; int* step_idx;
  int n, HW; int use_cfg;
  const float* ref; const unsigned char* mask; const float* step_noise; int n_steps_total;
  int seeded; DdimSeeds seeds;
  void* unet_in; int in_dt; int in_ld; int in_rep;
  float* t_out;
  int solver; float* hist;
};
void launch_ddim_step(const DdimParams& p, int do_update, hipStream_t s);
void launch_seeded_noise(float* out, const uint64_t* seeds, uint32_t draw, int n, int HW, hipStream_t s);
void launch_axpby(float* dst, const float* a, float sa, const float* b, float sb, size_t n, hipStream_t s);
void launch_to_u8_image(const void* src, int dt, int lds, unsigned char* dst, size_t pixels, hipStream_t s);
void launch_from_u8_image(const unsigned char* src, void* dst, int dt, int ldd, size_t pixels, hipStream_t s);

void launch_synth_fill(float* dst, size_t numel, uint64_t key, float scale, float mean, hipStream_t s);
void launch_pack_linear(const float* src, void* dst, int dt, int K, int N, int Kpad, int Npad, int geglu,
                        int n_offset, hipStream_t s, const float* kscale = nullptr,
                        float wscale = 1.0f);
void launch_pack_linear_hilo(const float* src, void* dst, int K, int N, int Npad, int geglu, float lo_scale, hipStream_t s, int mode = 0, int n_offset = 0);
void launch_colsum_packed(const void* wp, int dt, int Kpad, int nrows, float* cs, hipStream_t s, const float* kscale = nullptr, int K = 0, int interleave = 0);
void launch_beta_dot(const float* w, const float* beta, const float* bias, float* out, int K, int N, hipStream_t s);
void launch_pack_conv(const float* src, void* dst, int dt, int Cout, int Cin, int ks, int Kpad, int Npad,
                      hipStream_t s, float wscale = 1.0f);
void launch_absmax(const float* src, size_t n, float* out_dev, hipStream_t s, bool accumulate = false);
void launch_pack_bias(const float* src, float* dst, int N, int Npad, int geglu, int n_offset, hipStream_t s);

}
```

stable-diffusion-xl-burn_amd/csrc/select.cpp:

```cpp
#include "kernels.h"
#include <algorithm>
#include <atomic>
#include <cstring>
#include <stdexcept>

namespace sdxl {

namespace {
struct KnobSlot { const char* key; int SelectKnobs::*field; };
constexpr KnobSlot kKnobSlots[] = {
    {"igemm_variant", &SelectKnobs::igemm_variant}, {"igemm_wreg", &SelectKnobs::igemm_wreg}, {"wreg_xattn", &SelectKnobs::wreg_xattn},
    {"hl_tile96", &SelectKnobs::hl_tile96},         {"igemm_tsw", &SelectKnobs::igemm_tsw},   {"wide_db", &SelectKnobs::wide_db},
    {"attn_variant", &SelectKnobs::attn_variant},   {"attn_xsplit", &SelectKnobs::attn_xsplit},
#ifdef SDXL_MEASURE
    {"igemm_unrolled", &SelectKnobs::igemm_unrolled},
#endif
};
constexpr int kNumKnobs = sizeof(kKnobSlots) / sizeof(kKnobSlots[0]);
struct KnobStore {
  std::atomic<int> v[kNumKnobs];
  KnobStore() { const SelectKnobs d; for (int i = 0; i < kNumKnobs; ++i) v[i] = d.*kKnobSlots[i].field; }
};
KnobStore g_knobs;
}
// ... 32 lines not shown
}
const Tile& tile(int number) {
  if (const Tile* t = find_tile(number)) return *t;
  throw std::logic_error("igemm_select: no tile of that number");
}
bool tile_takes(const Tile& t, const IgemmParams& p) {
  if (t.bn == 160) return p.N % 160 == 0 && !p.stat_out;
  if (t.bn == 320) return p.act == 1 && is_linear(p) && p.N % 320 == 0;
  return true;
}

double tile_cost(int M, int N, int nk, int bm, int bn, double w) {
  const long tiles = (long)((M + bm - 1) / bm) * ((N + bn - 1) / bn);
  const long full = tiles / 256, rem = tiles % 256;
  const double frac = rem == 0 ? 0.0 : (full == 0 ? 1.0 : (rem / 256.0 > 2.0 / 3.0 ? rem / 256.0 : 2.0 / 3.0));
  return ((double)full + frac) * (bm + bn) * nk * w + (double)(full + (rem ? 1 : 0)) * 3000.0;
}
double tile_cost(const IgemmParams& p, int nk, int number) {
  const Tile& t = tile(number);
  return tile_cost(p.M, p.N, nk, t.bm, t.bn, t.w);
}

int pick_tile(const IgemmParams& p, std::initializer_list<int> among) {
  const int nk = p.Kpad / 64;
  double best = 1e300;
  int number = 35;
  for (int n : among) {
    const Tile& t = tile(n);
    if (!tile_takes(t, p) || (n == 49 && p.act != 0)) continue;
    const double cost = tile_cost(p.M, p.N, nk, t.bm, t.bn, t.w);
    if (cost < best) { best = cost; number = n; }
  }
  if (number == 36 && nk >= 40) number = 44;
  return number;
}

struct Fill { long t96, t128, t256; double eff128, eff256; };
Fill chip_fill(const IgemmParams& p) {
  const long cols = (p.N + 127) / 128;
  const long t96 = (long)((p.M + 95) / 96) * cols, t128 = (long)((p.M + 127) / 128) * cols, t256 = (long)((p.M + 255) / 256) * cols;
  return {t96, t128, t256, (double)t128 / (double)(((t128 + 255) / 256) * 256), (double)t256 / (double)(((t256 + 255) / 256) * 256)};
}
int fill_tile_256_or_128(const IgemmParams& p) {
  const Fill f = chip_fill(p);
  return f.eff256 >= f.eff128 ? 35 : 36;
}

bool wreg_pair_grid_fits(const IgemmParams& p) {
  const long rows = 2L * (p.rpb > 0 ? p.rpb : p.M);
  return ((rows + 95) / 96) * (long)(p.N / 128) <= 512;
}
int wreg_rows(const IgemmParams& p) { return (long)((p.M + 63) / 64) * (p.N / 128) <= 256 ? 64 : 96; }
bool wreg_takes(const IgemmParams& p, const SelectKnobs& k, bool xa) {
  if (!p.Wf || !k.zero_page || (xa ? !p.xa_k || p.xa_k_lo : p.xa_k != nullptr)) return false;
  if (p.a_dt != DT_F16 || (p.c_dt != DT_F16 && (xa || p.c_dt != DT_F32))) return false;
  if (p.ksize != 1 || p.stride != 1 || p.up != 0 || p.pad != 0 || p.Hin != p.Hout || p.Win != p.Wout) return false;
  if (p.N % 128 != 0 || p.Cin != p.K || p.K != p.Kpad || p.Kpad % 64 != 0 || p.Kpad < 128) return false;
  if (p.act != 0 || p.n_split < p.N || p.gn_part || p.acc_scale || p.ebias) return false;
  if ((p.lda & 7) != 0 || misaligned16(p.A) || (p.ldc & 7) != 0 || misaligned16(p.C)) return false;
  if (xa) return !p.stat_out && !p.R && !p.shadow && p.rpb > 0 && p.rpb % 64 == 0 && p.M % p.rpb == 0 && p.xa_nctx >= 1 && p.xa_nctx <= 96;
  if (p.ln_stat || (p.R && ((p.ldr & 7) != 0 || misaligned16(p.R)))) return false;
  if (p.shadow && (p.c_dt != DT_F32 || !p.shadow_gamma || (p.shadow_ld & (p.shadow_lo_scale < 0.f ? 15 : 7)) != 0 || misaligned16(p.shadow))) return false;
  return true;
}
#ifdef SDXL_MEASURE
struct WregForced { int number, bm, depth, mode; };
// ... 25 lines not shown
    default: break;
  }
}
IgemmChoice from_tile(int number, int elem, const IgemmParams& p) {
  const Tile& t = tile(number);
  IgemmChoice c{};
  c.family = t.family; c.bm = t.bm; c.bn = t.bn; c.ns = t.ns; c.wgm = t.wgm; c.nw = t.nw; c.s2 = t.s2; c.elem = elem; c.a_elem = elem; c.splitk = 1;
  set_geometry(c, p);
  return c;
}
IgemmChoice wreg_choice(int bm, int depth, int mode, bool xa, const IgemmParams& p) {
  IgemmChoice c{};
  c.family = IG_WREG; c.bm = bm; c.bn = 128; c.ns = depth; c.nw = 8; c.mode = mode; c.xa = xa; c.elem = c.a_elem = DT_F16; c.splitk = 1;
  set_geometry(c, p);
  return c;
}
IgemmChoice wreg_forced_or_auto(int v, bool xa, const IgemmParams& p) {
#ifdef SDXL_MEASURE
  if (!xa) for (const WregForced& f : kWregForced) if (f.number == v) return wreg_choice(f.bm, f.depth, f.mode, false, p);
#endif
  return wreg_choice(v == 60 ? 96 : v == 62 ? 64 : wreg_rows(p), 2, 0, xa, p);
}

bool select_f16(const IgemmParams& p, int v, const SelectKnobs& k, IgemmChoice& c) {
  if (!k.zero_page) return false;
  if (p.act > 1) return false;
  if (p.a_dt != DT_F16 || (p.Cin % 64) != 0 || (p.lda % 8) != 0 || (p.Kpad % 64) != 0) return false;
  if (misaligned16(p.A)) return false;
  if (p.n_split < p.N && (p.n_split & 3) != 0) return false;
  if (p.ebias && (p.ebias_ld & 3) != 0) return false;
  if (p.stat_out && (v == 2 || v == 5 || v == 19 || v == 38)) return false;
  const bool was_auto = v == 0;
  const int nk = p.Kpad / 64;
  if (p.xa_k) {
    if (p.act != 0 || p.n_split < p.N || p.stat_out || p.R || p.ebias ||
        !igemm_xattn_ok(p.a_dt, p.c_dt, p.M, p.N, p.K, p.rpb, p.xa_nctx))
      throw std::runtime_error("igemm: fused cross-attention needs a plain f16 projection (no residual / split outputs)");
    if (!p.xa_k_lo && p.c_dt != DT_F16) throw std::runtime_error("igemm: the f16 fused cross-attention writes f16 rows");
    const bool forced_pipe = v == 35 || v == 36 || v == 44 || v == 45;
    if (p.xa_k_lo) {
      c = from_tile(pick_tile(p, {36, 45}) == 45 ? 45 : 36, DT_F16, p);
      c.xh = 1;
      if (c.bm == 96) c.ns = 3;
    } else if (!forced_pipe && igemm_wreg_xattn_selected(p, k)) {
      c = wreg_forced_or_auto(v, true, p);
      return true;
    } else {
      c = from_tile(forced_pipe ? v : pick_tile(p, {35, 36, 45}), DT_F16, p);
      if (c.bm == 96) c.ns = 3;
    }
    c.xa = 1;
    set_geometry(c, p);
    return true;
  }
  if (p.gn_part) {
    if (!igemm_gn_part_ok(p, k)) throw std::runtime_error("igemm: GroupNorm statistics requested from a shape the 256x128 epilogue does not take");
    v = 0;
  }
  if (p.shadow) {
    if (!igemm_wreg_selected(p, k)) throw std::runtime_error("igemm: an f16 shadow output needs the weights-in-registers kernel");
    c = wreg_forced_or_auto(0, false, p);
    return true;
  }
  if (v == 0 ? igemm_wreg_selected(p, k) : (v >= 60 && v <= 77 && wreg_takes(p, k, false))) { c = wreg_forced_or_auto(v, false, p); return true; }
  if (v >= 60 && v <= 77) return false;
  if (v == 0 && igemm_splitk_slices(p) > 1) {
// ... 23 lines not shown
  c = from_tile(v, DT_F16, p);
  if (v == 35 && p.n_split < p.N && k.igemm_tsw && p.c_dt == DT_F16) c.tsw = 1;
#ifdef SDXL_MEASURE
  if (c.family == IG_WIDE) c.db = k.wide_db != 0;
#endif
  return true;
}

bool select_f32(const IgemmParams& p, const SelectKnobs& k, IgemmChoice& c) {
  if (!k.zero_page) return false;
  if (p.act > 1 || p.ln_stat || p.stat_out) return false;
  if (p.a_dt != DT_F32 || (p.Cin % 32) != 0 || (p.lda % 4) != 0 || (p.Kpad % 32) != 0) return false;
  if (misaligned16(p.A)) return false;
  if (p.n_split < p.N && (p.n_split & 3) != 0) return false;
  if (p.ebias && (p.ebias_ld & 3) != 0) return false;
  c = from_tile(fill_tile_256_or_128(p), DT_F32, p);
  return true;
}

bool select_hl(const IgemmParams& p, const SelectKnobs& k, IgemmChoice& c) {
  if (!k.zero_page) return false;
  if (p.act > 1 || p.ln_stat || p.stat_out || p.xa_k) return false;
  if (p.a_dt != DT_HL || (p.Cin % 32) != 0 || (p.lda % 4) != 0 || (p.Kpad % 32) != 0) return false;
  if (p.gn_part && !igemm_gn_part_ok(p, k)) throw std::runtime_error("igemm: GroupNorm statistics requested from a split-operand shape the 256x128 split-K epilogue does not take");
  if (misaligned16(p.A)) return false;
  if (p.n_split < p.N && (p.n_split & 3) != 0) return false;
  if (p.c_dt == DT_HL) {
    if (p.n_split < p.N && p.n_split != 0 && ((p.n_split & 127) != 0 || p.act != 0)) return false;
    const int nout = p.act == 1 ? (p.N >> 1) : p.N;
    if (p.n_split != 0 && ((nout & 7) != 0 || (p.ldc & 15) != 0 || misaligned16(p.C))) return false;
    if (p.n_split < p.N && ((p.ct_ld & 15) != 0 || (p.rpb & 7) != 0 || (p.M % 8) != 0 || misaligned16(p.Ct))) return false;
  }
  if (p.ebias && (p.ebias_ld & 3) != 0) return false;
  const int t96mode = k.hl_tile96;
  const bool splitk = (t96mode & 16) && igemm_splitk_slices(p) > 1;
  const bool plain160 = p.N % 160 == 0 && p.n_split >= p.N && !p.stat_out && p.act == 0;
  const Fill f = chip_fill(p);
  int number;
  if ((t96mode & 1) && (p.ksize == 1 || (t96mode & 2)) && p.n_split >= p.N && f.t128 < 256 && f.t96 <= 256 && f.t96 > f.t128 && f.eff256 < (double)f.t96 / 256.0 && !splitk) {
    number = 45;
  } else if (splitk) {
    number = 35;
  } else if ((t96mode & 4) && plain160 && p.N % 128 != 0) {
    number = 49;
  } else if ((t96mode & 8) && plain160 &&
             tile_cost(p, p.Kpad / 32, 49) < std::min(tile_cost(p, p.Kpad / 32, 35), tile_cost(p, p.Kpad / 32, 36))) {
    number = 49;
  } else {
    number = fill_tile_256_or_128(p);
  }
  c = from_tile(number, DT_HL, p);
  if (splitk) { c.splitk = igemm_splitk_slices(p); set_geometry(c, p); }
  return true;
}

IgemmChoice select_generic(const IgemmParams& p, int compute_dt) {
  struct Cand { int bm, bn; float eff; };
  const Cand cands[4] = {{128, 128, 1.0f}, {128, 64, 0.85f}, {64, 128, 0.85f}, {64, 64, 0.70f}};
  int best = 0; float best_cost = 1e30f;
  for (int i = 0; i < 4; ++i) {
    if (p.act == 1 && cands[i].bn < 64) continue;
    const long tiles = (long)((p.M + cands[i].bm - 1) / cands[i].bm) * ((p.N + cands[i].bn - 1) / cands[i].bn);
    const int slots = 256 * (cands[i].bm * cands[i].bn >= 128 * 128 ? 2 : 4);
    const long waves = (tiles + slots - 1) / slots;
    const float cost = (float)waves * cands[i].bm * cands[i].bn / cands[i].eff;
    if (cost < best_cost) { best_cost = cost; best = i; }
// ... 12 lines not shown
  if (p.act != 0 || p.n_split < p.N || p.ln_stat) return 1;
  const int nk = p.Kpad / 64;
  if (p.rpb <= 0 || p.rpb > 1024 || p.N > 1536 || nk < 160) return 1;
  return p.rpb <= 256 ? 8 : 3;
}
size_t igemm_splitk_ws_bytes(int batch, int rows_per_entry, int n_max) {
  if (n_max > 1536) n_max = 1536;
  const long rows3 = (long)batch * (rows_per_entry < 1024 ? rows_per_entry : 1024), rows8 = (long)batch * (rows_per_entry < 256 ? rows_per_entry : 256);
  const size_t slabs3 = (size_t)((rows3 + 255) / 256) * 3, slabs8 = (size_t)((rows8 + 255) / 256) * 8;
  return (slabs3 > slabs8 ? slabs3 : slabs8) * (size_t)((n_max + 127) / 128) * 256 * 128 * 4;
}

bool igemm_gn_part_ok(const IgemmParams& p, const SelectKnobs& k) {
  const bool hl = p.a_dt == DT_HL;
  const int kt = hl ? 32 : 64;
  if (hl ? p.c_dt != DT_F32 : (p.a_dt != DT_F16 || p.c_dt != DT_F16)) return false;
  if ((p.Cin % kt) != 0 || (p.lda % (kt / 8)) != 0 || (p.Kpad % kt) != 0) return false;
  if (p.act != 0 || p.n_split < p.N || p.stat_out || p.ln_stat || p.xa_k) return false;
  if (p.M % 256 != 0 || p.rpb <= 0 || p.rpb % 256 != 0 || p.N % 64 != 0) return false;
  if (p.ebias && (p.ebias_ld & 3) != 0) return false;
  if (hl) return (p.ldc & 3) == 0 && !misaligned16(p.C) && (k.hl_tile96 & 16) && igemm_splitk_slices(p) > 1;
  if (igemm_splitk_slices(p) > 1) return true;
  IgemmParams q = p;
  q.M = 2 * p.rpb;
  if (pick_tile(q, {35, 36, 45, 38, 26}) != 35) return false;
  const int nk = p.Kpad / 64;
  return p.N % 160 != 0 || tile_cost(q, nk, 35) - tile_cost(q, nk, 49) < 6000.0;
}

bool igemm_xattn_ok(int a_dt, int c_dt, int M, int N, int K, int rpb, int n_ctx) {
  return a_dt == DT_F16 && (c_dt == DT_F16 || c_dt == DT_HL) && M > 0 && N % 64 == 0 && K % 64 == 0 && rpb > 0 && rpb % 64 == 0 && M % rpb == 0 &&
         n_ctx >= 1 && n_ctx <= 96;
}
bool igemm_wreg_selected(const IgemmParams& p, const SelectKnobs& k) { return wreg_takes(p, k, false) && k.igemm_wreg && wreg_pair_grid_fits(p); }
bool igemm_wreg_xattn_selected(const IgemmParams& p, const SelectKnobs& k) {
  return wreg_takes(p, k, true) && k.igemm_wreg && k.wreg_xattn && wreg_pair_grid_fits(p);
}

IgemmChoice igemm_select(const IgemmParams& p, int compute_dt, const SelectKnobs& k) {
  IgemmChoice c{};
  if (p.M <= 0 || p.N <= 0) return c;
  const int v = k.igemm_variant;
  if (compute_dt == DT_F16 && v >= 0 && select_f16(p, v, k, c)) return c;
  if (compute_dt == DT_F16 && v > 0 && select_f16(p, 0, k, c)) return c;
  if (p.shadow && compute_dt != DT_F16) throw std::runtime_error("an f16 shadow output needs an f16 GEMM (weights-in-registers kernel)");
  if (compute_dt == DT_F32 && v >= 0 && select_f32(p, k, c)) return c;
  if (compute_dt == DT_HL) {
    if (select_hl(p, k, c)) return c;
    throw std::runtime_error("split-operand (DT_HL) GEMM: shape / alignment outside the direct-to-LDS pipeline");
  }
  if (p.xa_k) throw std::runtime_error("fused cross-attention needs the f16 direct-to-LDS kernels");
  if (p.shadow) throw std::runtime_error("an f16 shadow output needs the f16 weights-in-registers kernel");
  if (p.gn_part) throw std::runtime_error("GroupNorm statistics from the epilogue (gn_part) need the f16 direct-to-LDS 256x128 kernel");
  if (p.ln_stat || p.stat_out)
    throw std::runtime_error("LayerNorm-folded GEMM (ln_stat / stat_out) needs the f16 direct-to-LDS kernels");
  return select_generic(p, compute_dt);
}

int attention_xsplit_heads(int H) { return H - std::max(1, H * 4 / 5); }
size_t attention_xsplit_counters(int B, int H, int Nq) { return (size_t)B * attention_xsplit_heads(H) * ((Nq + 63) / 64) * 2; }
size_t attention_xsplit_ws_bytes(int B, int H, int Nq) { return attention_xsplit_counters(B, H, Nq) * 2 * (9 * 64 * 4 * sizeof(float)); }

#ifdef SDXL_MEASURE
struct AttnKnockout { int number, ko; };
constexpr AttnKnockout kAttnKnockouts[] = {{11, 1}, {12, 2}, {13, 4}, {14, 8}, {15, 16}, {16, 1 | 4}, {17, 2 | 8}};
#endif

AttnChoice attn_select(const AttnParams& p, const SelectKnobs& k) {
  const int v = k.attn_variant;
  AttnChoice c{};
  c.mix = -1; c.block = 256; c.grid_y = 1;
  const int qb128 = (p.Nq + 127) / 128, qb64 = (p.Nq + 63) / 64;
  const bool aligned = ((p.ldq | p.ldk | p.vt_ld | p.ldo) & 7) == 0 &&
                       ((reinterpret_cast<uintptr_t>(p.Q) | reinterpret_cast<uintptr_t>(p.K) |
                         reinterpret_cast<uintptr_t>(p.Vt) | reinterpret_cast<uintptr_t>(p.O)) & 15) == 0;
  if (p.dt == DT_F16 && (v == 0 || (v >= 2 && v <= 17)) && k.zero_page && aligned && !p.mask) {
    c.lds = 3 * 2 * 64 * 128;
// ... 36 lines not shown
```

stable-diffusion-xl-burn_amd/csrc/unet.cpp:

```cpp
#include "engine.h"

#include <atomic>
#include <cmath>
#include <cstring>

namespace sdxl {

namespace {
ResBlockW load_res(WeightBuilder& wb, const std::string& p, int cin, int cout, std::vector<std::string>& emb_names,
                   int& emb_off) {
  ResBlockW r;
  r.cin = cin; r.cout = cout;
  r.norm_in = wb.norm(p + ".norm_in");
  r.conv_in = wb.conv(p + ".conv_in");
  r.norm_out = wb.norm(p + ".norm_out");
  r.conv_out = wb.conv(p + ".conv_out");
  r.has_skip = wb.has(p + ".skip_connection.weight");
  if (r.has_skip) r.skip = wb.conv(p + ".skip_connection");
  r.emb_off = emb_off;
  emb_names.push_back(p + ".lin_embed");
  emb_off += cout;
  return r;
}
const std::vector<std::string> kQkv = {".attn1.query", ".attn1.key", ".attn1.value"};
// ... 219 lines not shown
}

void UNet::build_weights(WeightSource& src, hipStream_t st) {
  const std::vector<ParamSpec> specs = unet_param_specs(cfg_);
  std::vector<BlockDesc> inp, out; BlockDesc mid;
  unet_block_plan(cfg_, inp, mid, out);
  std::vector<std::pair<std::string, int>> sts;
  auto has_st = [](const BlockDesc& d) { return d.kind == BK_REST || d.kind == BK_RESTU; };
  for (size_t i = 0; i < inp.size(); ++i) if (has_st(inp[i])) sts.push_back({"input_blocks." + std::to_string(i) + ".transformer", inp[i].depth});
  sts.push_back({"middle_block.transformer", mid.depth});
  for (size_t i = 0; i < out.size(); ++i) if (has_st(out[i])) sts.push_back({"output_blocks." + std::to_string(i) + ".transformer", out[i].depth});
  std::vector<StPlan> plans;
  std::vector<std::string> f16_names;
  auto plan_all = [&]() {
    plans.clear(); f16_names.clear();
    for (const auto& t : sts) {
      plans.push_back(plan_transformer(mix_, cdt_, specs, t.first));
      for (int j = 0; j < t.second; ++j) f16_valued_weights(plans.back(), t.first + ".blocks." + std::to_string(j), f16_names);
    }
  };
  plan_all();
  WeightBuilder wb(specs, src, warena_, cdt_, st);
  if (!mix_knob_ && !wb.all_f16_exact(f16_names)) {
    mix_ = (mix_ & (MIX_ATTN_F16 | MIX_GEGLU_F16)) ? (MIX_ATTN_F16 | MIX_GEGLU_F16 | MIX_GEGLU_HILO) : 0;
    plan_all();
    SDXL_REQUIRE(f16_names.empty(), "the fallback classes pack no parameter as f16 values");
  }
  bool x2 = false;
  attn16_ = cdt_ == DT_F16;
  for (const StPlan& pl : plans) {
    x2 = x2 || pl.qkv == LF_X2 || pl.out1 == LF_X2 || pl.q2 == LF_X2 || pl.out2 == LF_X2 || pl.geglu == LF_X2 || pl.ff == LF_X2;
    attn16_ = attn16_ || pl.attn_f16;
  }
  size_t bound = WeightBuilder::arena_bound(specs, cdt_);
  if (x2)
    for (const ParamSpec& ps : specs) if (ps.kind == PK_LINEAR_W) bound += round_up(ps.shape[1], 128) * round_up((size_t)ps.shape[0], 64) * 4 + 256;
  warena_.reserve(bound);
  const int gv = cdt_ == DT_HL ? DT_F32 : -1;
  lin1_t_ = wb.linear("lin1_time_embed", false, gv);
  lin2_t_ = wb.linear("lin2_time_embed", false, gv);
  lin1_l_ = wb.linear("lin1_label_embed", false, gv);
  lin2_l_ = wb.linear("lin2_label_embed", false, gv);
  std::vector<std::string> emb_names;
  int emb_off = 0;
  size_t sti = 0;
  auto load_block = [&](const std::string& p, const BlockDesc& d) {
    BlockW b; b.d = d;
    switch (d.kind) {
      case BK_CONV: case BK_DOWN: b.conv = wb.conv(p); break;
      case BK_RES: b.res = load_res(wb, p, d.c_in, d.c_out, emb_names, emb_off); break;
      default:
        b.res = load_res(wb, p + ".res", d.c_in, d.c_out, emb_names, emb_off);
        if (d.kind == BK_REST || d.kind == BK_RESTU) b.st = load_st(wb, p + ".transformer", d.c_out, d.n_head, d.depth, fuse_ln_, plans[sti++]);
        if (d.kind == BK_RESTU || d.kind == BK_RESU) b.conv = wb.conv(p + ".upsample.conv");
    }
    return b;
  };
  for (size_t i = 0; i < inp.size(); ++i) inp_.push_back(load_block("input_blocks." + std::to_string(i), inp[i]));
  mid_res1_.d = mid;
  mid_res1_.res = load_res(wb, "middle_block.res1", mid.c_in, mid.c_out, emb_names, emb_off);
  mid_res1_.st = load_st(wb, "middle_block.transformer", mid.c_out, mid.n_head, mid.depth, fuse_ln_, plans[sti++]);
  mid_res2_.d = mid;
  mid_res2_.res = load_res(wb, "middle_block.res2", mid.c_in, mid.c_out, emb_names, emb_off);
  for (size_t i = 0; i < out.size(); ++i) out_.push_back(load_block("output_blocks." + std::to_string(i), out[i]));
  norm_out_ = wb.norm("norm_out");
  conv_out_ = wb.conv("conv_out");
  embcat_ = wb.fused_linear(emb_names, gv);
  emb_total_ = emb_off;
  SDXL_HIP(hipStreamSynchronize(st));
  for (BlockW& b : inp_) if (!b.st.blocks.empty()) st_list_.push_back(&b.st);
  st_list_.push_back(&mid_res1_.st);
  for (BlockW& b : out_) if (!b.st.blocks.empty()) st_list_.push_back(&b.st);
}

void UNet::set_context(const float* context, int n_ctx, const float* label, int B, hipStream_t s) {
  SDXL_REQUIRE(B >= 1 && B <= 8, "batch must be in 1..8");
  const int vt_ld = (int)round_up(n_ctx, 64);
  bool pack_xs = false, pack_xa = false;
  for (const STW* st : st_list_) { pack_xs = pack_xs || st->plan.xattn == XA_SPLIT; pack_xa = pack_xa || st->plan.xattn != XA_LAUNCH; }
  pack_xs = pack_xs && n_ctx <= 96; pack_xa = pack_xa && n_ctx <= 96;
  const int kvdt = attn_dt();
  const int emb = 4 * cfg_.model_channels;
  {
    const int dm = cdt_ == DT_HL ? unet_hl_demote() : 0;
    if (dm != demote_mask_ || (dm && demote_flags_.empty())) { demote_mask_ = dm; apply_demote_weights(s); }
  }
  if (B != ctx_B_ || n_ctx != n_ctx_) {
// ... 315 lines not shown
        ex.act->reset(mkp);
        break;
      }
      default: throw Error("unexpected input block kind");
    }
    cur = dest; cur_c = b.d.c_out;
  }
  {
    const size_t mk = ex.act->mark();
    Act m1 = ex.alloc((size_t)B * h * w, mid_res1_.d.c_out, ex.sdt);
    float* part = (float*)ex.act->alloc((size_t)B * h * w / 256 * mid_res1_.d.c_out * 2 * sizeof(float) + 256);
    m1.gn_part = res_block(ex, mid_res1_.res, cur, B, h, w, m1, part); m1.gn_rt = h * w / 256;
    spatial_transformer(ex, mid_res1_.st, si++, m1, B, h, w);
    m1.gn_part = nullptr;
    res_block(ex, mid_res2_.res, m1, B, h, w, cat[0].cols(0));
    ex.act->reset(mk);
  }
  Act last = ex.alloc((size_t)B * H * W, mc, ex.sdt);
  for (int j = 0; j < n_out; ++j) {
    const BlockW& b = out_[j];
    const bool up = b.d.kind == BK_RESTU || b.d.kind == BK_RESU;
    const Act next = j + 1 < n_out ? cat[j + 1].cols(0) : last;
    const size_t mk = ex.act->mark();
    Act dest = up ? ex.alloc((size_t)B * h * w, b.d.c_out, ex.sdt) : next;
    if (b.d.kind == BK_REST || b.d.kind == BK_RESTU) {
      float* part = (float*)ex.act->alloc((size_t)B * h * w / 256 * b.d.c_out * 2 * sizeof(float) + 256);
      Act d = dest;
      d.gn_part = res_block(ex, b.res, cat[j], B, h, w, dest, part); d.gn_rt = h * w / 256;
      spatial_transformer(ex, b.st, si++, d, B, h, w);
    } else {
      res_block(ex, b.res, cat[j], B, h, w, dest);
    }
    if (up) {
      run_conv(ex, b.conv, hl_op(ex, b.conv, dest, (size_t)B * h * w, b.d.c_out, DM_CONV_UPDOWN, B), b.d.c_out, ConvGeom{B, h, w, 2 * h, 2 * w, 3, 1, 1, 1}, next, tag_epi(DM_CONV_UPDOWN));
      h *= 2; w *= 2;
    }
    ex.act->reset(mk);
  }
  SDXL_REQUIRE(h == H && w == W, "UNet input height/width must be divisible by 2^(levels-1)");
  {
    const size_t mk = ex.act->mark();
    Act gn = ex.alloc((size_t)B * H * W, mc, ex.cdt);
    run_groupnorm(ex, norm_out_, last, B, H * W, gn, true);
    demote_lo(ex, DM_CONV_IO, gn, (size_t)B * H * W, mc);
    run_conv(ex, conv_out_, gn, mc, ConvGeom{B, H, W, H, W, 3, 1, 1, 0}, Act(eps, cfg_.out_channels, DT_F32), tag_epi(DM_CONV_IO));
    ex.act->reset(mk);
  }
}

void UNet::ensure_plan(int B, int H, int W) {
  const bool split = split_cfg_ && B == 2;
  if (B == pB_ && H == pH_ && W == pW_ && split == plan_split_ && fuse_xattn_ == plan_xattn_ && gn_from_producer_ == plan_gn_) return;
  SDXL_REQUIRE(B >= 1 && B <= 8, "batch must be in 1..8");
  const int div = 1 << (cfg_.channel_mults.size() - 1);
  SDXL_REQUIRE(H >= div && W >= div && H % div == 0 && W % div == 0,
               "UNet input height/width must be divisible by 2^(levels-1)");
  if (graph_) { (void)hipGraphExecDestroy(graph_); graph_ = nullptr; }
  plan_runs_ = 0;
  warm_ = WarmSeq();
  pB_ = B; pH_ = H; pW_ = W;
  const int mc = cfg_.model_channels, emb = 4 * mc;
  auto persist = [&]() {
    in_ = act_.alloc((size_t)B * H * W * cfg_.in_channels * dt_size(input_dt()));
    eps_ = (float*)act_.alloc((size_t)B * H * W * cfg_.out_channels * sizeof(float));
    temb_ = (float*)act_.alloc((size_t)B * mc * sizeof(float));
    g1_ = (float*)act_.alloc((size_t)B * emb * sizeof(float));
    emb_ = (float*)act_.alloc((size_t)B * emb * sizeof(float));
// ... 177 lines not shown
```

stable-diffusion-xl-burn_amd/csrc/vae.cpp:

```cpp
#include "engine.h"

#include <cmath>

namespace sdxl {

VaeResW Vae::load_res(WeightBuilder& wb, const std::string& p, int cin, int cout) {
  VaeResW r; r.cin = cin; r.cout = cout;
  r.n1 = wb.norm(p + ".norm1"); r.c1 = wb.conv(p + ".conv1");
  r.n2 = wb.norm(p + ".norm2"); r.c2 = wb.conv(p + ".conv2");
  r.has_nin = wb.has(p + ".nin_shortcut.weight");
  if (r.has_nin) r.nin = wb.conv(p + ".nin_shortcut");
  return r;
}
VaeMidW Vae::load_mid(WeightBuilder& wb, const std::string& p, int c) {
  VaeMidW m; m.C = c;
  m.b1 = load_res(wb, p + ".block_1", c, c);
  m.an = wb.norm(p + ".attn.norm");
  m.q = wb.conv(p + ".attn.q"); m.k = wb.conv(p + ".attn.k"); m.v = wb.conv(p + ".attn.v");
  m.proj = wb.conv(p + ".attn.proj_out");
  m.b2 = load_res(wb, p + ".block_2", c, c);
  return m;
}

Vae::Vae(const VaeCfg& cfg, int compute_dt, WeightSource* dec_src, WeightSource* enc_src, hipStream_t st)
    : cfg_(cfg), cdt_(compute_dt) {
  const std::vector<ParamSpec> dspecs = vae_decoder_param_specs(cfg_), especs = vae_encoder_param_specs(cfg_);
  size_t bound = 0;
  if (dec_src) bound += WeightBuilder::arena_bound(dspecs, cdt_, false);
  if (enc_src) bound += WeightBuilder::arena_bound(especs, cdt_, false);
  warena_.reserve(bound + 4096);
  if (dec_src) {
    WeightBuilder wb(dspecs, *dec_src, warena_, cdt_, st);
    wb.wfrag = false;
    post_quant_ = wb.conv("post_quant_conv");
    d_conv_in_ = wb.conv("decoder.conv_in");
    d_mid_ = load_mid(wb, "decoder.mid", cfg_.dec.front().first);
    for (size_t i = 0; i < cfg_.dec.size(); ++i) {
      const std::string p = "decoder.blocks." + std::to_string(i);
      DecBlk b;
      b.r[0] = load_res(wb, p + ".res1", cfg_.dec[i].first, cfg_.dec[i].second);
      b.r[1] = load_res(wb, p + ".res2", cfg_.dec[i].second, cfg_.dec[i].second);
      b.r[2] = load_res(wb, p + ".res3", cfg_.dec[i].second, cfg_.dec[i].second);
      b.has_up = i + 1 != cfg_.dec.size();
      if (b.has_up) b.up = wb.conv(p + ".upsampler");
      d_blocks_.push_back(b);
    }
    d_norm_out_ = wb.norm("decoder.norm_out");
    d_conv_out_ = wb.conv("decoder.conv_out");
    SDXL_HIP(hipStreamSynchronize(st));
    has_dec_ = true;
  }
  if (enc_src) {
    WeightBuilder wb(especs, *enc_src, warena_, cdt_, st);
    wb.wfrag = false;
    e_conv_in_ = wb.conv("encoder.conv_in");
    for (size_t i = 0; i < cfg_.enc.size(); ++i) {
      const std::string p = "encoder.blocks." + std::to_string(i);
      EncBlk b;
      b.r[0] = load_res(wb, p + ".res1", cfg_.enc[i].first, cfg_.enc[i].second);
      b.r[1] = load_res(wb, p + ".res2", cfg_.enc[i].second, cfg_.enc[i].second);
      b.has_down = i + 1 != cfg_.enc.size();
      if (b.has_down) b.down = wb.conv(p + ".downsampler");
      e_blocks_.push_back(b);
    }
    e_mid_ = load_mid(wb, "encoder.mid", cfg_.enc.back().first);
    e_norm_out_ = wb.norm("encoder.norm_out");
    e_conv_out_ = wb.conv("encoder.conv_out");
    quant_ = wb.conv("quant_conv");
    SDXL_HIP(hipStreamSynchronize(st));
    has_enc_ = true;
  }
}
Vae::~Vae() {}

void Vae::res_block(Exec& ex, const VaeResW& w, const Act& x, int B, int H, int W, const Act& out) {
  const size_t mk = ex.act->mark();
  const size_t M = (size_t)B * H * W;
// ... 78 lines not shown
      ev.Ct = vt32;
      run_conv(ex, w.v, hn, C, g1, Act(nullptr, C, DT_F32), ev);
      if (!ex.dry) launch_f32_to_hl(vt32, kpad, vt, kpad, (size_t)B * rows_v, kpad, ex.s);
    } else
    run_conv(ex, w.v, hn, C, g1, Act(nullptr, C, ex.cdt), ev);
    for (int b = 0; b < B; ++b) {
      Lin lk; lk.w = (char*)kbuf + (size_t)b * rows_k * C * dt_size(ex.cdt); lk.N = HW; lk.K = C; lk.Kpad = C; lk.Npad = rows_k; lk.cin = C;
      Lin lv; lv.w = (char*)vt + (size_t)b * rows_v * kpad * dt_size(ex.cdt); lv.N = C; lv.K = kpad; lv.Kpad = kpad; lv.Npad = rows_v; lv.cin = kpad;
      for (int q0 = 0; q0 < HW; q0 += QT) {
        const int nq = HW - q0 < QT ? HW - q0 : QT;
        const size_t row0 = ((size_t)b * HW + q0) * C * dt_size(ex.cdt);
        run_linear(ex, lk, Act((char*)q.p + row0, C, ex.cdt), nq, Act(S, HW, DT_F32));
        if (!ex.dry) launch_softmax_rows(S, HW, P, ex.cdt, kpad, nq, HW, kpad, scale, nullptr, 0, 0, ex.s, pv_scale ? 4096.0f : 1.0f, pv_scale);
        lv.acc_scale = pv_scale;
        run_linear(ex, lv, Act(P, kpad, ex.cdt), nq, Act((char*)o.p + row0, C, ex.cdt));
      }
    }
    Epi ep; ep.R = y;
    run_conv(ex, w.proj, o, C, g1, y, ep);
  }
  res_block(ex, w.b2, y, B, H, W, x);
  ex.act->reset(mk);
}

void Vae::run_decode(Exec& ex, const Act& in, int n, int h, int w, const Act& out) {
  const size_t M0 = (size_t)n * h * w;
  Act z = ex.alloc(M0, 4, io_dt());
  run_conv(ex, post_quant_, in, 4, ConvGeom{n, h, w, h, w, 1, 1, 0, 0}, z);
  const int c0 = cfg_.dec.front().first;
  Act cur = ex.alloc(M0, c0, ex.sdt);
  run_conv(ex, d_conv_in_, z, 4, ConvGeom{n, h, w, h, w, 3, 1, 1, 0}, cur);
  mid(ex, d_mid_, cur, n, h, w);
  for (size_t i = 0; i < d_blocks_.size(); ++i) {
    const DecBlk& b = d_blocks_[i];
    const int co = cfg_.dec[i].second;
    const size_t M = (size_t)n * h * w;
    Act next = b.has_up ? ex.alloc(4 * M, co, ex.sdt) : ex.alloc(M, co, ex.sdt);
    const size_t mk = ex.act->mark();
    Act a = ex.alloc(M, co, ex.sdt);
    Act bb = ex.alloc(M, co, ex.sdt);
    res_block(ex, b.r[0], cur, n, h, w, a);
    res_block(ex, b.r[1], a, n, h, w, bb);
    if (b.has_up) {
      res_block(ex, b.r[2], bb, n, h, w, a);
      run_conv(ex, b.up, hl_operand(ex, b.up, a, M, co, n), co, ConvGeom{n, h, w, 2 * h, 2 * w, 3, 1, 1, 1}, next);
      h *= 2; w *= 2;
    } else {
      res_block(ex, b.r[2], bb, n, h, w, next);
    }
    ex.act->reset(mk);
    cur = next;
  }
  const size_t M = (size_t)n * h * w;
  const int cl = cfg_.dec.back().second;
  Act gn = ex.alloc(M, cl, ex.cdt);
  run_groupnorm(ex, d_norm_out_, cur, n, h * w, gn, true, cfg_.n_group);
  run_conv(ex, d_conv_out_, gn, cl, ConvGeom{n, h, w, h, w, 3, 1, 1, 0}, out);
}

void Vae::run_encode(Exec& ex, const Act& in, int n, int H, int W, const Act& out) {
  int h = H, w = W;
  const int c0 = cfg_.enc.front().second;
  Act cur = ex.alloc((size_t)n * h * w, c0, ex.sdt);
  run_conv(ex, e_conv_in_, in, 3, ConvGeom{n, h, w, h, w, 3, 1, 1, 0}, cur);
  for (size_t i = 0; i < e_blocks_.size(); ++i) {
    const EncBlk& b = e_blocks_[i];
    const int co = cfg_.enc[i].second;
    const size_t M = (size_t)n * h * w;
    const int h2 = b.has_down ? (h + 1 - 3) / 2 + 1 : h, w2 = b.has_down ? (w + 1 - 3) / 2 + 1 : w;
    Act next = ex.alloc((size_t)n * h2 * w2, co, ex.sdt);
    const size_t mk = ex.act->mark();
    Act a = ex.alloc(M, co, ex.sdt);
    res_block(ex, b.r[0], cur, n, h, w, a);
    if (b.has_down) {
      Act bb = ex.alloc(M, co, ex.sdt);
      res_block(ex, b.r[1], a, n, h, w, bb);
      run_conv(ex, b.down, hl_operand(ex, b.down, bb, M, co, n), co, ConvGeom{n, h, w, h2, w2, 3, 2, 0, 0}, next);
    } else {
// ... 80 lines not shown
```

stable-diffusion-xl-burn_amd/csrc/weights.cpp:

```cpp
#include "engine.h"

#include <cstdio>
#include <cstdlib>
#include <cstring>
#include <cmath>

namespace sdxl {

DeviceArena::~DeviceArena() { if (base) (void)hipFree(base); }
void DeviceArena::reserve(size_t bytes) {
  if (bytes <= cap && base) return;
  if (base) { SDXL_HIP(hipFree(base)); base = nullptr; }
  SDXL_HIP(hipMalloc((void**)&base, bytes));
  cap = bytes;
}
void* DeviceArena::alloc(size_t bytes) {
  const size_t a = round_up(off, 256);
  off = a + bytes;
  if (off > peak) peak = off;
  if (dry) return (void*)(uintptr_t)(a + 256);
  if (off > cap) throw Error("device arena overflow (" + std::to_string(off) + " > " + std::to_string(cap) + ")");
  return base + a;
}

void Profiler::begin(int cls, double flops, hipStream_t s, int m, int n, int k, int ks, int tag) {
  Rec r; r.cls = cls; r.flops = flops; r.m = m; r.n = n; r.k = k; r.ks = ks; r.tag = tag;
  SDXL_HIP(hipEventCreate(&r.a)); SDXL_HIP(hipEventCreate(&r.b));
  SDXL_HIP(hipEventRecord(r.a, s));
  recs.push_back(r);
}
void Profiler::end(hipStream_t s) { SDXL_HIP(hipEventRecord(recs.back().b, s)); }
void Profiler::collect(float ms[NCLS], int launches[NCLS], double flops[NCLS]) {
  for (int i = 0; i < NCLS; ++i) { ms[i] = 0.f; launches[i] = 0; flops[i] = 0.0; }
  const char* dump = std::getenv("SDXL_PROFILE_DUMP");
// ... 80 lines not shown
  for (size_t i = 0; i < entries.size(); ++i) by_param[entries[i].param_index].push_back((int)i);
}
LoraSource::~LoraSource() { if (stage) (void)hipFree(stage); }
void LoraSource::fetch(const ParamSpec& s, size_t index, float* dst, hipStream_t st) {
  inner.fetch(s, index, dst, st);
  if (index >= by_param.size() || by_param[index].empty()) return;
  const size_t rows = (size_t)s.shape[0], cols = s.numel() / rows;
  for (int i : by_param[index]) {
    const LoraEntry& e = entries[i];
    const size_t nl = rows * (size_t)e.rank, nr = (size_t)e.rank * cols;
    if (nl + nr > stage_numel) {
      if (stage) { SDXL_HIP(hipStreamSynchronize(st)); SDXL_HIP(hipFree(stage)); stage = nullptr; stage_numel = 0; }
      SDXL_HIP(hipMalloc((void**)&stage, (nl + nr) * sizeof(float)));
      stage_numel = nl + nr;
    }
    SDXL_HIP(hipMemcpyAsync(stage, e.left, nl * sizeof(float), hipMemcpyDefault, st));
    SDXL_HIP(hipMemcpyAsync(stage + nl, e.right, nr * sizeof(float), hipMemcpyDefault, st));
    launch_lora_merge(dst, rows, cols, stage, stage + nl, e.rank, e.scale, st);
  }
  if (flags & kLoraRoundF16) launch_round_f16(dst, s.numel(), st);
  SDXL_HIP(hipStreamSynchronize(st));
}

WeightBuilder::WeightBuilder(const std::vector<ParamSpec>& sp, WeightSource& s, DeviceArena& a, int dtype, hipStream_t stream)
    : specs(sp), src(s), arena(a), dt(dtype), st(stream) {
  for (size_t i = 0; i < specs.size(); ++i) {
    index[specs[i].name] = i;
    if (specs[i].numel() > tmp_numel) tmp_numel = specs[i].numel();
  }
  SDXL_HIP(hipMalloc((void**)&tmp, tmp_numel * sizeof(float)));
}
WeightBuilder::~WeightBuilder() { if (tmp) (void)hipFree(tmp); if (tmp2) (void)hipFree(tmp2); }

size_t WeightBuilder::arena_bound(const std::vector<ParamSpec>& specs, int dt, bool wfrag) {
  size_t total = 1 << 20;
  for (const ParamSpec& p : specs) {
    if (p.kind == PK_LINEAR_W) total += round_up(p.shape[1], 128) * round_up(p.shape[0], 64) * dt_size(dt) + 768;
    else if (p.kind == PK_CONV_W)
      total += round_up(p.shape[0], 128) * round_up((size_t)p.shape[1] * p.shape[2] * p.shape[3], 64) * dt_size(dt) + 768;
    else total += round_up(p.numel(), 128) * sizeof(float) + 256;
    if (p.kind == PK_LINEAR_W || p.kind == PK_CONV_W) total += round_up(p.kind == PK_LINEAR_W ? p.shape[1] : p.shape[0], 128) * 4 + 256;
    if (p.kind == PK_LINEAR_W) total += round_up(p.shape[1], 128) * 4 + 256;
    if (wfrag && dt == DT_F16 && p.kind == PK_LINEAR_W) total += round_up(p.shape[1], 128) * round_up(p.shape[0], 64) * 2 + 256;
    if (wfrag && dt == DT_F16 && p.kind == PK_CONV_W && p.shape[2] == 1) total += round_up(p.shape[0], 128) * round_up((size_t)p.shape[1], 64) * 2 + 256;
  }
  return total;
}
const ParamSpec& WeightBuilder::spec(const std::string& name, size_t* idx) const {
  auto it = index.find(name);
  if (it == index.end()) throw Error("unknown parameter '" + name + "'");
  if (idx) *idx = it->second;
  return specs[it->second];
}
const float* WeightBuilder::fetch(const std::string& name) {
  if (name == last_fetched) return tmp;
  size_t i; const ParamSpec& s = spec(name, &i);
  src.fetch(s, i, tmp, st);
  last_fetched = name;
  return tmp;
}
float WeightBuilder::hl_scale(Lin& l, const std::vector<std::string>& weight_names) {
  float* sc = (float*)arena.alloc(2 * sizeof(float));
  l.acc_scale = sc;
  if (src.empty()) return 1.f;
  SDXL_HIP(hipMemsetAsync(sc, 0, 2 * sizeof(float), st));
  for (const std::string& n : weight_names) launch_absmax(fetch(n), spec(n).numel(), sc, st, true);
  float h = 0.f;
  SDXL_HIP(hipMemcpyAsync(&h, sc, sizeof(float), hipMemcpyDeviceToHost, st));
  SDXL_HIP(hipStreamSynchronize(st));
  int e = 0;
  if (h > 0.f && std::isfinite(h)) { (void)std::frexp(h, &e); e = 14 - e; }
  e = e > 24 ? 24 : (e < -24 ? -24 : e);
  const float wscale = std::ldexp(1.0f, e), inv = 1.0f / wscale;
  SDXL_HIP(hipMemcpyAsync(sc, &inv, sizeof(float), hipMemcpyHostToDevice, st));
  SDXL_HIP(hipStreamSynchronize(st));
  bool first = true;
  for (const std::string& n : weight_names) { launch_f16_exact(fetch(n), spec(n).numel(), wscale, sc + 1, st, !first); first = false; }
  return wscale;
}

void WeightBuilder::attach_wfrag(Lin& l, bool fill, bool folded) {
  const int wdt = l.dt >= 0 ? l.dt : dt;
  if (!wfrag) return;
  if (wdt != DT_F16 || l.ksize != 1 || l.N % 128 != 0 || l.K != l.Kpad || l.Kpad % 64 != 0 || l.Kpad < 128 || (l.cs && !folded) || l.acc_scale) return;
  void* wf = arena.alloc((size_t)l.Npad * l.Kpad * 2);
  l.wf = wf;
  if (fill) launch_repack_wfrag(l.w, wf, l.Npad, l.Kpad, st);
}
Lin WeightBuilder::linear(const std::string& name, bool geglu, int dt_override) {
  const ParamSpec& s = spec(name + ".weight");
  Lin l; l.K = s.shape[0]; l.N = s.shape[1]; l.ksize = 1; l.cin = l.K;
  const int wdt = dt_override >= 0 ? dt_override : ((dt == DT_HL && l.K % 32 != 0) ? DT_F32 : dt);
  if (wdt != dt) l.dt = wdt;
  const int kt = wdt == DT_F16 ? 64 : 32;
  l.Kpad = (int)round_up(l.K, kt); l.Npad = (int)round_up(l.N, 128);
  void* w = arena.alloc((size_t)l.Npad * l.Kpad * dt_size(wdt));
  float* b = (float*)arena.alloc((size_t)l.Npad * sizeof(float));
  l.w = w; l.b = b;
  const float wscale = wdt == DT_HL ? hl_scale(l, {name + ".weight"}) : 1.f;
  if (src.empty()) { if (!geglu) attach_wfrag(l, false); return l; }
  launch_pack_linear(fetch(name + ".weight"), w, wdt, l.K, l.N, l.Kpad, l.Npad, geglu ? 1 : 0, 0, st, nullptr, wscale);
  const float* bsrc = has(name + ".bias") ? fetch(name + ".bias") : nullptr;
  launch_pack_bias(bsrc, b, l.N, l.Npad, geglu ? 1 : 0, 0, st);
  if (!geglu) attach_wfrag(l, true);
  return l;
}
Lin WeightBuilder::linear_hilo(const std::string& name, bool geglu, bool dup, bool hl_interleave) {
  const ParamSpec& s = spec(name + ".weight");
  const int K0 = s.shape[0];
  SDXL_REQUIRE(K0 % 32 == 0, "linear_hilo: K % 32 == 0");
  Lin l; l.K = 2 * K0; l.N = s.shape[1]; l.ksize = 1; l.cin = l.K; l.dt = DT_F16; l.k_form = hl_interleave ? 2 : 1;
// ... 101 lines not shown
    SDXL_HIP(hipMalloc((void**)&tmp2, need * sizeof(float)));
    tmp2_numel = need;
  }
  float* gamma = tmp2;
  float* beta = tmp2 + l.K;
  float* bsrc = beta + l.K;
  float* bfold = bsrc + l.Npad;
  SDXL_REQUIRE(spec(norm + ".gamma").shape[0] == K0, "fused_linear_ln: norm width mismatch");
  SDXL_HIP(hipMemcpyAsync(gamma, fetch(norm + ".gamma"), K0 * sizeof(float), hipMemcpyDeviceToDevice, st));
  SDXL_HIP(hipMemcpyAsync(beta, fetch(norm + ".beta"), K0 * sizeof(float), hipMemcpyDeviceToDevice, st));
  SDXL_HIP(hipMemsetAsync(w, 0, (size_t)l.Npad * l.Kpad * dt_size(dt), st));
  SDXL_HIP(hipMemsetAsync(b, 0, (size_t)l.Npad * sizeof(float), st));
  if (bplain) SDXL_HIP(hipMemsetAsync(bplain, 0, (size_t)l.Npad * sizeof(float), st));
  int off = 0;
  for (const std::string& n : names) {
    const ParamSpec& s = spec(n + ".weight");
    const int N = s.shape[1];
    const bool hb = has(n + ".bias");
    if (hb) SDXL_HIP(hipMemcpyAsync(bsrc, fetch(n + ".bias"), N * sizeof(float), hipMemcpyDeviceToDevice, st));
    const float* wsrc = fetch(n + ".weight");
    if (hl_interleave) launch_pack_linear_hilo(wsrc, w, K0, N, names.size() == 1 ? l.Npad : N, geglu ? 1 : 0, kHiLoScale, st, 2, off);
    else if (hilo_dup) launch_pack_linear_hilo(wsrc, w, K0, N, l.Npad, geglu ? 1 : 0, kHiLoScale, st, 1);
    else if (names.size() == 1) launch_pack_linear(wsrc, w, dt, l.K, N, l.Kpad, l.Npad, geglu ? 1 : 0, 0, st, shadow ? nullptr : gamma);
    else launch_pack_linear(wsrc, w, dt, l.K, N, l.Kpad, N, 0, off, st, shadow ? nullptr : gamma);
    launch_beta_dot(wsrc, beta, hb ? bsrc : nullptr, bfold, K0, N, st);
    launch_pack_bias(bfold, b, N, names.size() == 1 ? l.Npad : N, geglu ? 1 : 0, off, st);
    if (bplain) launch_pack_bias(hb ? bsrc : nullptr, bplain, N, names.size() == 1 ? l.Npad : N, geglu ? 1 : 0, off, st);
    off += N;
  }
  if (shadow) launch_colsum_packed(w, dt, l.Kpad, l.Npad, cs, st, gamma, K0, hl_interleave ? 1 : 0);
  else launch_colsum_packed(w, dt, l.Kpad, l.Npad, cs, st);
  return l;
}
Lin WeightBuilder::conv(const std::string& name) {
  const ParamSpec& s = spec(name + ".weight");
  Lin l; l.N = s.shape[0]; l.cin = s.shape[1]; l.ksize = s.shape[2];
  l.K = l.cin * l.ksize * l.ksize;
  const int wdt = (dt == DT_HL && l.cin % 32 != 0) ? DT_F32 : dt;
  if (wdt != dt) l.dt = wdt;
  const int kt = wdt == DT_F16 ? 64 : 32;
  l.Kpad = (int)round_up(l.K, kt); l.Npad = (int)round_up(l.N, 128);
  void* w = arena.alloc((size_t)l.Npad * l.Kpad * dt_size(wdt));
  float* b = (float*)arena.alloc((size_t)l.Npad * sizeof(float));
  l.w = w; l.b = b;
  const float wscale = wdt == DT_HL ? hl_scale(l, {name + ".weight"}) : 1.f;
  if (src.empty()) { attach_wfrag(l, false); return l; }
  launch_pack_conv(fetch(name + ".weight"), w, wdt, l.N, l.cin, l.ksize, l.Kpad, l.Npad, st, wscale);
  launch_pack_bias(fetch(name + ".bias"), b, l.N, l.Npad, 0, 0, st);
  attach_wfrag(l, true);
  return l;
}
NormW WeightBuilder::norm(const std::string& name) {
  const ParamSpec& s = spec(name + ".gamma");
  NormW n; n.C = s.shape[0];
  float* g = (float*)arena.alloc((size_t)n.C * sizeof(float));
  float* b = (float*)arena.alloc((size_t)n.C * sizeof(float));
  float* e = (float*)arena.alloc(sizeof(float));
  n.gamma = g; n.beta = b; n.eps = e;
  if (src.empty()) return n;
  SDXL_HIP(hipMemcpyAsync(g, fetch(name + ".gamma"), n.C * sizeof(float), hipMemcpyDeviceToDevice, st));
  SDXL_HIP(hipMemcpyAsync(b, fetch(name + ".beta"), n.C * sizeof(float), hipMemcpyDeviceToDevice, st));
  SDXL_HIP(hipMemcpyAsync(e, fetch(name + ".eps"), sizeof(float), hipMemcpyDeviceToDevice, st));
  return n;
}

void WarmSeq::finish() {
  const size_t n = seq.size();
  for (Item& it : seq) for (int r = 0; r < 3; ++r) { it.warm[r] = nullptr; it.warm_bytes[r] = 0; }
  for (size_t j = 0; j < n && n > 4; ++j) {
    const unsigned bytes = seq[j].bytes;
    if (bytes < (1u << 18) || bytes > (seq[j].host ? 14u << 20 : 8u << 20)) continue;
    for (size_t d = 1; d <= 4; ++d) {
      Item& h = seq[(j + n - d) % n];
      if (!h.host || h.warm[2] || h.w == seq[j].w || h.budget < bytes) continue;
      const int r = !h.warm[0] ? 0 : !h.warm[1] ? 1 : 2;
      h.warm[r] = seq[j].w; h.warm_bytes[r] = bytes;
      h.budget -= bytes;
      break;
    }
  }
  recording = false; ready = true; pos = 0;
  if (std::getenv("SDXL_WARM_DUMP")) {
    std::vector<char> covered(n, 0);
    for (size_t i = 0; i < n; ++i) for (int r = 0; r < 3; ++r) if (seq[i].warm[r]) for (size_t j = 0; j < n; ++j) if (seq[j].w == seq[i].warm[r]) covered[j] = 1;
    size_t tb = 0, cb = 0;
    for (size_t i = 0; i < n; ++i) {
      tb += seq[i].bytes; if (covered[i]) cb += seq[i].bytes;
      std::fprintf(stderr, "[warm] %3zu %9u B %s carries %u + %u + %u B %s\n", i, seq[i].bytes, seq[i].host ? "host" : "    ", seq[i].warm_bytes[0], seq[i].warm_bytes[1],
                   seq[i].warm_bytes[2], covered[i] ? "" : "*");
    }
    std::fprintf(stderr, "[warm] %zu entries, %.1f MB read per forward, %.1f MB of it warmed\n", n, tb / 1048576.0, cb / 1048576.0);
  }
}
bool run_conv(Exec& ex, const Lin& w, const Act& a, int cin, const ConvGeom& g, const Act& out, const Epi& e) {
  if (ex.dry) return false;
  SDXL_REQUIRE(cin == w.cin, "run_conv: channel mismatch");
  IgemmParams p{};
  p.A = a.p; p.W = w.w; p.Wf = w.wf; p.a_dt = a.dt;
  p.B = g.B; p.Hin = g.Hin; p.Win = g.Win; p.Cin = cin; p.lda = a.ld;
  p.Hout = g.Hout; p.Wout = g.Wout;
  p.ksize = g.ksize; p.stride = g.stride; p.pad = g.pad; p.up = g.up;
  p.M = g.B * g.Hout * g.Wout; p.N = w.N; p.K = w.K; p.Kpad = w.Kpad;
  p.bias = w.b; p.ebias = e.ebias; p.ebias_ld = e.ebias_ld;
  p.rpb = e.rpb ? e.rpb : g.Hout * g.Wout;
  p.act = e.act;
  p.R = e.R.p; p.ldr = e.R.ld; p.r_dt = e.R.dt;
  p.C = out.p; p.ldc = out.ld; p.c_dt = out.dt;
  p.n_split = e.n_split >= 0 ? e.n_split : w.N;
  p.Ct = e.Ct; p.ct_rows = e.ct_rows; p.ct_ld = e.ct_ld;
  p.ln_stat = e.ln_stat; p.ln_slots = (w.ln_k ? w.ln_k : w.K) / 64; p.ln_cs = w.cs; p.ln_invc = 1.0f / (float)(w.ln_k ? w.ln_k : w.K); p.ln_eps = 1e-5f; p.ln_eps_ptr = w.ln_eps;
  p.stat_out = e.stat_out; p.stat_slots = w.N / 64;
  p.splitk_ws = ex.splitk_ws; p.splitk_ws_bytes = ex.splitk_ws_bytes; p.splitk_cnt = ex.splitk_cnt; p.splitk = 0;
  p.xa_k = e.xa_k; p.xa_nctx = e.xa_nctx; p.xa_scale = e.xa_scale; p.xa_k_lo = e.xa_k_lo;
  p.acc_scale = w.acc_scale;
  p.a_scale = (w.dt >= 0 ? w.dt : ex.cdt) == DT_HL ? a.a_scale : nullptr;
  p.a_scale_rpb = (p.a_scale && a.a_scale_n > 1) ? p.M / a.a_scale_n : 0;
  const SelectKnobs knobs = igemm_launch_knobs();
  p.gn_part = nullptr;
  {
    const int wdt_ = w.dt >= 0 ? w.dt : ex.cdt;
    if (e.gn_part && (wdt_ == DT_F16 || wdt_ == DT_HL) && wdt_ == ex.cdt) { p.gn_part = e.gn_part; if (!igemm_gn_part_ok(p, knobs)) p.gn_part = nullptr; }
  }
  if (e.shadow_done) *e.shadow_done = false;
  if (e.shadow) {
    p.shadow = e.shadow; p.shadow_ld = e.shadow_ld; p.shadow_gamma = e.shadow_gamma; p.shadow_lo_scale = e.shadow_lo_scale;
    const bool ok = (w.dt >= 0 ? w.dt : ex.cdt) == DT_F16 && igemm_wreg_selected(p, knobs);
    if (!ok) { p.shadow = nullptr; p.shadow_gamma = nullptr; p.stat_out = nullptr; p.shadow_lo_scale = 0.f; }
    if (e.shadow_done) *e.shadow_done = ok;
  }
  SDXL_REQUIRE(!e.xa_k || igemm_xattn_ok(a.dt, out.dt, p.M, p.N, p.K, p.rpb, e.xa_nctx), "fused cross-attention: unsupported shape");
  SDXL_REQUIRE(!e.ln_stat || (w.ln_k ? w.ln_k : w.K) % 64 == 0, "LayerNorm-folded GEMM needs K % 64 == 0");
  SDXL_REQUIRE(!e.stat_out || (w.N % 64 == 0 && (e.n_split < 0 || e.n_split >= w.N) && e.act == 0), "row statistics need a plain N % 64 == 0 output");
  SDXL_REQUIRE(!e.ln_stat || w.cs, "ln_stat given but the weight is not LayerNorm-folded");
  SDXL_REQUIRE(!w.cs || e.ln_stat, "LayerNorm-folded weight used without row statistics");
  SDXL_REQUIRE(!((w.dt >= 0 ? w.dt : ex.cdt) == DT_F32 && a.dt != DT_F32), "f32 compute needs f32 activations");
  if (ex.prof) ex.prof->begin(Profiler::IGEMM, 2.0 * p.M * (double)p.N * p.K, ex.s, p.M, p.N, p.K, p.ksize, e.cls);
  if (ex.warm && (w.dt >= 0 ? w.dt : ex.cdt) == DT_F16) {
    WarmSeq& ws = *ex.warm;
    const bool host = igemm_wreg_selected(p, knobs) || igemm_wreg_xattn_selected(p, knobs);
    const size_t wbytes = (size_t)w.Npad * w.Kpad * 2;
    const char* lo; const char* hi;
    if (host) {
      const char* f = reinterpret_cast<const char*>(p.Wf), *b = reinterpret_cast<const char*>(w.b);
      lo = (b && b < f && f - b <= (64 << 10)) ? b : f;
      hi = f + wbytes;
    } else {
      lo = reinterpret_cast<const char*>(p.W); hi = lo + wbytes;
      auto ext = [&](const void* q, size_t sz) { const char* c = reinterpret_cast<const char*>(q); if (q && c >= hi && c - hi <= (64 << 10)) hi = c + sz; };
      ext(w.b, (size_t)w.Npad * 4); ext(w.cs, (size_t)w.Npad * 4); ext(w.ln_eps, 4);
    }
    if (ws.recording) {
      if (p.xa_k) ws.seq.push_back(WarmSeq::Item{p.xa_k, (unsigned)xattn_pack_bytes(p.M / p.rpb, p.N), false, 0u, {nullptr, nullptr, nullptr}, {0u, 0u, 0u}});
      const unsigned budget = host ? 14u << 20 : 0u;
      ws.seq.push_back(WarmSeq::Item{lo, (unsigned)(hi - lo), host, budget, {nullptr, nullptr, nullptr}, {0u, 0u, 0u}});
    } else if (ws.ready) {
      if (p.xa_k) ++ws.pos;
      if (ws.pos < ws.seq.size()) {
        const WarmSeq::Item& it = ws.seq[ws.pos++];
        if (it.w == lo) for (int r = 0; r < 3; ++r) { p.warm[r] = it.warm[r]; p.warm_bytes[r] = it.warm_bytes[r]; }
      }
    }
  }
  launch_igemm(p, w.dt >= 0 ? w.dt : ex.cdt, knobs, ex.s);
  {
    const hipError_t le = hipGetLastError();
    if (le != hipSuccess)
      throw Error(std::string("implicit-GEMM launch failed (") + hipGetErrorString(le) + "): M=" + std::to_string(p.M) + " N=" + std::to_string(p.N) +
                  " K=" + std::to_string(p.K) + " ksize=" + std::to_string(p.ksize) + " a_dt=" + std::to_string(p.a_dt) + " c_dt=" + std::to_string(p.c_dt) +
                  " compute=" + std::to_string(w.dt >= 0 ? w.dt : ex.cdt) + " act=" + std::to_string(p.act) + " n_split=" + std::to_string(p.n_split));
  }
  if (ex.prof) ex.prof->end(ex.s);
  {
    static const bool nan_check = std::getenv("SDXL_NAN_CHECK") != nullptr;
// ... 69 lines not shown
```

Before: 1.398 images/sec.

## Fold nearest upsample into 3x3 conv as four 2x2 phase convolutions

Precomputes four phase-specific 2x2 kernels from each upsample 3x3 conv weight, so the convolution runs on the low-resolution input. The epilogue scatters each phase's rows to interleaved output positions. This removes the redundant multiply-adds on duplicated upsampled pixels, reducing K from 9·Cin to 4·Cin per output. It costs extra weight arena memory and a one-time host sync to check the split-operand scale, and it is gated on exactness and on phase-tiling support.

```diff
diff --git a/include/sdxl_mi355.h b/include/sdxl_mi355.h
--- a/include/sdxl_mi355.h
+++ b/include/sdxl_mi355.h
@@ -203,6 +203,7 @@
 int sdxl_bench_attention(sdxl_ctx* ctx, void* stream, int B, int H, int Nq, int Nk, int iters, float* avg_ms);
 int sdxl_debug_set(const char* key, int value);
 int sdxl_debug_warm_schedule(int n, const unsigned* bytes, const unsigned char* host, int* warmed_by);
+int sdxl_debug_upsample_fold(const float* weight, int cout, int cin, float* out);
 enum {
   SDXL_SEL_WF = 1 << 0, SDXL_SEL_R = 1 << 1, SDXL_SEL_EBIAS = 1 << 2, SDXL_SEL_STAT_OUT = 1 << 3, SDXL_SEL_LN_STAT = 1 << 4, SDXL_SEL_GN_PART = 1 << 5,
   SDXL_SEL_SHADOW = 1 << 6, SDXL_SEL_XA_K = 1 << 7, SDXL_SEL_XA_K_LO = 1 << 8, SDXL_SEL_ACC_SCALE = 1 << 9, SDXL_SEL_SPLITK_WS = 1 << 10,
@@ -234,6 +235,8 @@
                     float eps, int dtype, float* out);
 int sdxl_conv2d(sdxl_ctx* ctx, void* stream, const float* x, const float* weight, const float* bias, int B, int Cin,
                 int H, int W, int Cout, int ksize, int stride, int pad, int upsample, int dtype, float* out);
+int sdxl_conv2d_upsample_folded(sdxl_ctx* ctx, void* stream, const float* x, const float* weight, const float* bias, int B, int Cin, int H, int W,
+                                int Cout, int dtype, int* folded, float* out);
 int sdxl_linear(sdxl_ctx* ctx, void* stream, const float* x, const float* weight, const float* bias, int M, int K, int N,
                 int geglu, int dtype, float* out);
 int sdxl_layer_norm_linear(sdxl_ctx* ctx, void* stream, const float* x, const float* gamma, const float* beta, float eps,
diff --git a/stable-diffusion-xl-burn_amd/__init__.py b/stable-diffusion-xl-burn_amd/__init__.py
--- a/stable-diffusion-xl-burn_amd/__init__.py
+++ b/stable-diffusion-xl-burn_amd/__init__.py
@@ -78,7 +78,7 @@
     "sdxl_vae_create", "sdxl_vae_create_synthetic", "sdxl_vae_destroy", "sdxl_vae_decode_latent",
     "sdxl_latent_to_image", "sdxl_vae_encode_image", "sdxl_image_to_latent",
     "sdxl_unet_weight_arena", "sdxl_vae_weight_arena", "sdxl_diffuser_create_empty", "sdxl_vae_create_empty",
-    "sdxl_unet_profile", "sdxl_unet_eager_forward_ms", "sdxl_bench_igemm", "sdxl_bench_attention", "sdxl_debug_set", "sdxl_debug_warm_schedule", "sdxl_debug_igemm_select", "sdxl_debug_attn_select",
+    "sdxl_unet_profile", "sdxl_unet_eager_forward_ms", "sdxl_bench_igemm", "sdxl_bench_attention", "sdxl_debug_set", "sdxl_debug_warm_schedule", "sdxl_debug_upsample_fold", "sdxl_conv2d_upsample_folded", "sdxl_debug_igemm_select", "sdxl_debug_attn_select",
     "sdxl_group_norm", "sdxl_layer_norm", "sdxl_conv2d", "sdxl_linear", "sdxl_layer_norm_linear", "sdxl_ln_query_cross_attention", "sdxl_conv2d_group_norm",
     "sdxl_transformer_projection",
     "sdxl_lora_check", "sdxl_lora_merge", "sdxl_unet_create_lora", "sdxl_diffuser_create_lora",
@@ -979,6 +979,22 @@
     return out
 
 
+def conv2d_upsample_folded(ctx: Context, x, weight, bias, dtype: int = DTYPE_F16):
+    torch = _torch()
+    x, px = _dev(x)
+    weight, pw = _dev(weight)
+    pb = None
+    if bias is not None:
+        bias, pb = _dev(bias)
+    B, Cin, H, W = x.shape
+    Cout = int(weight.shape[0])
+    out = torch.empty((B, Cout, 2 * H, 2 * W), device=x.device, dtype=torch.float32)
+    took = ctypes.c_int(0)
+    _check(lib().sdxl_conv2d_upsample_folded(ctx.h, _stream(), px, pw, pb, int(B), int(Cin), int(H), int(W), Cout, dtype, ctypes.byref(took),
+                                            ctypes.c_void_p(out.data_ptr())))
+    return out, bool(took.value)
+
+
 def linear(ctx: Context, x, weight, bias, geglu: bool = False, dtype: int = DTYPE_F16):
     torch = _torch()
     x, px = _dev(x)
diff --git a/stable-diffusion-xl-burn_amd/build.py b/stable-diffusion-xl-burn_amd/build.py
--- a/stable-diffusion-xl-burn_amd/build.py
+++ b/stable-diffusion-xl-burn_amd/build.py
@@ -39,7 +39,7 @@
 
 def _deps_hash(src: str) -> str:
     h = hashlib.sha256()
-    for f in [src] + [os.path.join(CSRC, x) for x in ("kernels.h", "engine.h", "igemm_common.h", "capi_internal.h", "select_debug.h")] + \
+    for f in [src] + [os.path.join(CSRC, x) for x in ("kernels.h", "engine.h", "igemm_common.h", "capi_internal.h", "select_debug.h", "upsample_fold.h")] + \
             [os.path.join(HERE, "..", "include", "sdxl_mi355.h")]:
         with open(f, "rb") as fh:
             h.update(fh.read())
diff --git a/stable-diffusion-xl-burn_amd/csrc/capi.hip b/stable-diffusion-xl-burn_amd/csrc/capi.hip
--- a/stable-diffusion-xl-burn_amd/csrc/capi.hip
+++ b/stable-diffusion-xl-burn_amd/csrc/capi.hip
@@ -1,5 +1,6 @@
 #include "capi_internal.h"
 #include "select_debug.h"
+#include "upsample_fold.h"
 #include <algorithm>
 #include <cstring>
 
@@ -139,6 +140,7 @@
   else if (std::strcmp(key, "hl_demote") == 0) unet_set_hl_demote(value);
   else if (std::strcmp(key, "mix_classes") == 0) unet_set_mix_classes(value);
   else if (std::strcmp(key, "wreg_xcd2d") == 0) igemm_set_wreg_xcd2d(value);
+  else if (std::strcmp(key, "upsample_fold") == 0) set_upsample_fold(value);
 #ifdef SDXL_MEASURE
   else if (std::strcmp(key, "xa_vec64") == 0) igemm_set_xa_vec64(value);
   else if (std::strcmp(key, "no_cfg") == 0) g_debug_no_cfg = value != 0;
@@ -156,6 +158,12 @@
   for (int i = 0; i < n; ++i)
     for (int r = 0; r < 3; ++r)
       if (ws.seq[i].warm[r]) warmed_by[(int)(reinterpret_cast<uintptr_t>(ws.seq[i].warm[r]) >> 12) - 1] = i;
+  API_END
+}
+int sdxl_debug_upsample_fold(const float* weight, int cout, int cin, float* out) {
+  API_BEGIN
+  SDXL_REQUIRE(weight && out && cout > 0 && cin > 0, "bad argument");
+  fold_upsample_weights(weight, out, (size_t)cout, (size_t)cin);
   API_END
 }
 int sdxl_debug_igemm_select(const sdxl_igemm_case* c, const sdxl_select_knobs* knobs, sdxl_igemm_choice* out) {
diff --git a/stable-diffusion-xl-burn_amd/csrc/capi_ops.hip b/stable-diffusion-xl-burn_amd/csrc/capi_ops.hip
--- a/stable-diffusion-xl-burn_amd/csrc/capi_ops.hip
+++ b/stable-diffusion-xl-burn_amd/csrc/capi_ops.hip
@@ -344,6 +344,41 @@
   SDXL_HIP(hipStreamSynchronize(s));
   API_END
 }
+int sdxl_conv2d_upsample_folded(sdxl_ctx* ctx, void* stream, const float* x, const float* weight, const float* bias, int B, int Cin, int H, int W,
+                                int Cout, int dtype, int* folded, float* out) {
+  API_BEGIN
+  SDXL_REQUIRE(ctx && x && weight && out, "null argument");
+  SDXL_REQUIRE(dtype == SDXL_DTYPE_F16 || dtype == SDXL_DTYPE_F32_SPLIT, "the folded upsample convolution exists in the f16 and the split-operand engines");
+  use(ctx);
+  hipStream_t s = pick(ctx, stream);
+  const int cdt = dtype == SDXL_DTYPE_F16 ? DT_F16 : DT_HL, sdt = cdt;
+  SDXL_REQUIRE(Cin % (cdt == DT_HL ? 32 : 64) == 0, "the folded upsample convolution needs whole k-tiles per tap (Cin % 64, split-operand: Cin % 32)");
+  Operands ops;
+  add_conv(ops, "conv", Cout, Cin, 3, weight, bias);
+  Packed pk(ops, cdt, s);
+  const Lin l = pk.wb.conv("conv", true);
+  Tmp tmp;
+  const size_t rows = (size_t)B * H * W;
+  void* xi = tmp.get(rows * Cin * dt_size(sdt));
+  float* yo = (float*)tmp.get(4 * rows * Cout * sizeof(float));
+  Act xa(xi, Cin, sdt);
+  if (cdt == DT_HL) {
+    float* x32 = (float*)tmp.get(rows * Cin * sizeof(float));
+    float* sc = (float*)tmp.get(hl_scale_floats(B) * sizeof(float));
+    launch_nchw_to_nhwc(x, Cin * H * W, x32, DT_F32, B, Cin, H * W, Cin, 1.0f, s);
+    launch_f32_to_hl_scaled(x32, Cin, xi, Cin, rows, Cin, sc, s, B);
+    xa.a_scale = hl_scale_inv(sc, B); xa.a_scale_n = B;
+  } else launch_nchw_to_nhwc(x, Cin * H * W, xi, sdt, B, Cin, H * W, Cin, 1.0f, s);
+  Exec ex; ex.s = s; ex.cdt = cdt; ex.sdt = sdt;
+  give_splitk_ws(ex, tmp, B, 4 * H * W, Cout, s);
+  Epi e; e.fold = true;
+  bool took = false; e.fold_done = &took;
+  run_conv(ex, l, xa, Cin, ConvGeom{B, H, W, 2 * H, 2 * W, 3, 1, 1, 1}, Act(yo, Cout, DT_F32), e);
+  if (folded) *folded = took ? 1 : 0;
+  launch_nhwc_to_nchw(yo, DT_F32, Cout, out, B, Cout, 4 * H * W, 1.0f, s);
+  SDXL_HIP(hipStreamSynchronize(s));
+  API_END
+}
 int sdxl_linear(sdxl_ctx* ctx, void* stream, const float* x, const float* weight, const float* bias, int M, int K, int N,
                 int geglu, int dtype, float* out) {
   API_BEGIN
diff --git a/stable-diffusion-xl-burn_amd/csrc/elementwise.hip b/stable-diffusion-xl-burn_amd/csrc/elementwise.hip
--- a/stable-diffusion-xl-burn_amd/csrc/elementwise.hip
+++ b/stable-diffusion-xl-burn_amd/csrc/elementwise.hip
@@ -1,4 +1,5 @@
 #include "kernels.h"
+#include "upsample_fold.h"
 #include <algorithm>
 #include <stdexcept>
 
@@ -837,6 +838,14 @@
   const size_t total = (size_t)Npad * Kpad;
   hipLaunchKernelGGL(pack_conv_kernel, dim3((total + 255) / 256), dim3(256), 0, s, src, dst, dt, Cout, Cin, ks, Kpad, Npad, wscale);
 }
+__global__ void fold_upsample_kernel(const float* src, float* dst, size_t pairs) {
+  const size_t e = (size_t)blockIdx.x * blockDim.x + threadIdx.x;
+  if (e < 16 * pairs) dst[e] = fold_element(src, pairs, e);
+}
+void launch_fold_upsample(const float* src, float* dst, int Cout, int Cin, hipStream_t s) {
+  const size_t pairs = (size_t)Cout * Cin;
+  hipLaunchKernelGGL(fold_upsample_kernel, dim3((unsigned)((16 * pairs + 255) / 256)), dim3(256), 0, s, src, dst, pairs);
+}
 __global__ void pack_bias_kernel(const float* src, float* dst, int N, int Npad, int geglu, int n_offset) {
   const int i = blockIdx.x * blockDim.x + threadIdx.x;
   if (i >= Npad) return;
diff --git a/stable-diffusion-xl-burn_amd/csrc/engine.h b/stable-diffusion-xl-burn_amd/csrc/engine.h
--- a/stable-diffusion-xl-burn_amd/csrc/engine.h
+++ b/stable-diffusion-xl-burn_amd/csrc/engine.h
@@ -126,6 +126,7 @@
   int k_form = 0;
   int dt = -1;
   const float* acc_scale = nullptr;
+  const void* w_fold = nullptr; const float* fold_acc_scale = nullptr;
 };
 struct NormW { const float* gamma = nullptr; const float* beta = nullptr; const float* eps = nullptr; int C = 0; };
 
@@ -141,7 +142,7 @@
   WeightBuilder(const std::vector<ParamSpec>& sp, WeightSource& s, DeviceArena& a, int dtype, hipStream_t stream);
   ~WeightBuilder();
   bool wfrag = true;
-  static size_t arena_bound(const std::vector<ParamSpec>& specs, int dt, bool wfrag = true);
+  static size_t arena_bound(const std::vector<ParamSpec>& specs, int dt, bool wfrag = true, bool fold_up = false);
   const ParamSpec& spec(const std::string& name, size_t* idx = nullptr) const;
   bool has(const std::string& name) const { return index.count(name) != 0; }
   const float* fetch(const std::string& name);
@@ -149,13 +150,15 @@
   Lin fused_linear(const std::vector<std::string>& names, int dt_override = -1);
   Lin linear_hilo(const std::string& name, bool geglu, bool dup = false, bool hl_interleave = false);
   float hl_scale(Lin& l, const std::vector<std::string>& weight_names);
+  float hl_scale_of(const float* dev, size_t n, const float*& acc_scale);
   Lin linear_ln(const std::string& name, bool geglu, const std::string& norm, bool xattn_query = false);
   Lin fused_linear_ln(const std::vector<std::string>& names, const std::string& norm);
   Lin fold_ln(const std::vector<std::string>& names, const std::string& norm, bool geglu, int dt_override = -1, bool shadow = false, Lin* plain = nullptr, bool hilo_dup = false,
               bool hl_interleave = false);
   bool all_f16_exact(const std::vector<std::string>& names);
   float* tmp2 = nullptr; size_t tmp2_numel = 0;
-  Lin conv(const std::string& name);
+  Lin conv(const std::string& name, bool fold_up = false);
+  static bool folds_upsample(const ParamSpec& p, int dt);
   void attach_wfrag(Lin& l, bool fill, bool folded = false);
   NormW norm(const std::string& name);
 };
@@ -241,10 +244,13 @@
   const void* xa_k = nullptr; int xa_nctx = 0; float xa_scale = 0.f;
   const void* xa_k_lo = nullptr;
   float* gn_part = nullptr;
+  bool* fold_done = nullptr;
+  bool fold = false;
   int cls = 0;
   void* shadow = nullptr; int shadow_ld = 0; const float* shadow_gamma = nullptr; bool* shadow_done = nullptr; float shadow_lo_scale = 0.f;
 };
 bool run_conv(Exec& ex, const Lin& w, const Act& a, int cin, const ConvGeom& g, const Act& out, const Epi& e = Epi());
+void set_upsample_fold(int v);
 bool run_linear(Exec& ex, const Lin& w, const Act& a, int M, const Act& out, const Epi& e = Epi());
 Act hl_operand(Exec& ex, const Lin& w, const Act& x, size_t rows, int C, int nb = 1, float* have_max = nullptr);
 void run_groupnorm(Exec& ex, const NormW& n, const Act& x, int B, int HW, const Act& y, bool silu, int groups = 32, float* absmax_out = nullptr);
@@ -393,7 +399,7 @@
   DeviceArena warena_;
   bool has_dec_ = false, has_enc_ = false;
   Lin post_quant_, d_conv_in_, d_conv_out_; NormW d_norm_out_; VaeMidW d_mid_;
-  struct DecBlk { VaeResW r[3]; Lin up; bool has_up = false; };
+  struct DecBlk { VaeResW r[3]; Lin up; bool has_up = false; int up_fold = -1; };
   std::vector<DecBlk> d_blocks_;
   Lin quant_, e_conv_in_, e_conv_out_; NormW e_norm_out_; VaeMidW e_mid_;
   struct EncBlk { VaeResW r[2]; Lin down; bool has_down = false; };
diff --git a/stable-diffusion-xl-burn_amd/csrc/igemm_common.h b/stable-diffusion-xl-burn_amd/csrc/igemm_common.h
--- a/stable-diffusion-xl-burn_amd/csrc/igemm_common.h
+++ b/stable-diffusion-xl-burn_amd/csrc/igemm_common.h
@@ -143,6 +143,13 @@
   }
 };
 
+__device__ __forceinline__ size_t igemm_out_row(const IgemmParams& p, int m) {
+  if (p.ph_rows == 0) return (size_t)m;
+  const int ph = m / p.ph_rows, r = m - ph * p.ph_rows;
+  const int hw = p.Hin * p.Win, e = r / hw, q = r - e * hw, i = q / p.Win, j = q - i * p.Win;
+  return ((size_t)e * (2 * p.Hin) + (2 * i + (ph >> 1))) * (size_t)(2 * p.Win) + (size_t)(2 * j + (ph & 1));
+}
+
 template <int TM, int TN>
 __device__ __forceinline__ void igemm_epilogue(const IgemmParams& p, const f32x16 (&acc)[TM][TN], int mw, int nw, int fr, int fh,
                                                const float (&lnA)[TM], const float (&lnC)[TM]) {
@@ -153,6 +160,7 @@
     const int m = mw + i * 32 + fr;
     if (m >= p.M) continue;
     const int bidx = m / p.rpb;
+    const size_t mo = igemm_out_row(p, m);
     const int key = m - bidx * p.rpb;
     const float lna = lnA[i], lnc = lnC[i];
 #pragma unroll
@@ -212,16 +220,16 @@
           }
           if (vec && p.c_dt == DT_F16 && (p.ldc & 3) == 0) {
             half4 h; h[0] = (half_t)v[0]; h[1] = (half_t)v[1]; h[2] = (half_t)v[2]; h[3] = (half_t)v[3];
-            *reinterpret_cast<half4*>(reinterpret_cast<half_t*>(p.C) + (size_t)m * p.ldc + nout) = h;
+            *reinterpret_cast<half4*>(reinterpret_cast<half_t*>(p.C) + mo * p.ldc + nout) = h;
           } else if (vec && p.c_dt == DT_F32 && (p.ldc & 3) == 0) {
             f32x4 o = {v[0], v[1], v[2], v[3]};
-            *reinterpret_cast<f32x4*>(reinterpret_cast<float*>(p.C) + (size_t)m * p.ldc + nout) = o;
+            *reinterpret_cast<f32x4*>(reinterpret_cast<float*>(p.C) + mo * p.ldc + nout) = o;
           } else {
 #pragma unroll
             for (int r = 0; r < 4; ++r)
               if (nout + r < nlim) {
-                if (p.c_dt == DT_F16) reinterpret_cast<half_t*>(p.C)[(size_t)m * p.ldc + nout + r] = (half_t)v[r];
-                else reinterpret_cast<float*>(p.C)[(size_t)m * p.ldc + nout + r] = v[r];
+                if (p.c_dt == DT_F16) reinterpret_cast<half_t*>(p.C)[mo * p.ldc + nout + r] = (half_t)v[r];
+                else reinterpret_cast<float*>(p.C)[mo * p.ldc + nout + r] = v[r];
               }
           }
         } else {
@@ -403,6 +411,7 @@
       const bool valid = m < p.M && n0 < nlim;
       float rr[8] = {0.f, 0.f, 0.f, 0.f, 0.f, 0.f, 0.f, 0.f};
       if (valid) {
+      const size_t mo = igemm_out_row(p, m);
       float v[8] = {a[0], a[1], a[2], a[3], b[0], b[1], b[2], b[3]};
       const bool full = n0 + 8 <= nlim;
       if (rfast[it]) {
@@ -436,7 +445,7 @@
         for (int e = 0; e < 8; ++e) rr[e] = p.c_dt == DT_F16 ? (float)(half_t)v[e] : v[e];
       }
       if (p.c_dt == DT_F16) {
-        half_t* cp = reinterpret_cast<half_t*>(p.C) + (size_t)m * p.ldc + n0;
+        half_t* cp = reinterpret_cast<half_t*>(p.C) + mo * p.ldc + n0;
         if (full && (reinterpret_cast<uintptr_t>(cp) & 15) == 0) {
           half8 h;
 #pragma unroll
@@ -447,9 +456,9 @@
           for (int e = 0; e < 8; ++e) if (n0 + e < nlim) cp[e] = (half_t)v[e];
         }
       } else if (p.c_dt == DT_HL) {
-        if (full) store_hl8(reinterpret_cast<float*>(p.C) + (size_t)m * p.ldc, n0, v);
+        if (full) store_hl8(reinterpret_cast<float*>(p.C) + mo * p.ldc, n0, v);
       } else {
-        float* cp = reinterpret_cast<float*>(p.C) + (size_t)m * p.ldc + n0;
+        float* cp = reinterpret_cast<float*>(p.C) + mo * p.ldc + n0;
         if (full && (reinterpret_cast<uintptr_t>(cp) & 15) == 0) {
           *reinterpret_cast<f32x4*>(cp) = f32x4{v[0], v[1], v[2], v[3]};
           *reinterpret_cast<f32x4*>(cp + 4) = f32x4{v[4], v[5], v[6], v[7]};
@@ -605,12 +614,14 @@
   constexpr int NP = NQ / 2;
   const int nwo = GEGLU ? (nw >> 1) : nw;
   int m[TM], bidx[TM];
+  size_t mo[TM];
   bool mok[TM];
 #pragma unroll
   for (int i = 0; i < TM; ++i) {
     m[i] = mw + i * 32 + fr;
     mok[i] = m[i] < p.M;
     bidx[i] = (p.ebias && mok[i]) ? m[i] / p.rpb : 0;
+    mo[i] = mok[i] ? igemm_out_row(p, m[i]) : 0;
   }
   const bool r16 = p.R && p.r_dt == DT_F16, r32 = p.R && p.r_dt == DT_F32;
   half8 rh[TM][TN][NP];
@@ -690,7 +701,7 @@
           half8 h;
 #pragma unroll
           for (int e = 0; e < 8; ++e) h[e] = (half_t)w[e];
-          if (mok[i]) *reinterpret_cast<half8*>(reinterpret_cast<half_t*>(p.C) + (size_t)m[i] * p.ldc + n0) = h;
+          if (mok[i]) *reinterpret_cast<half8*>(reinterpret_cast<half_t*>(p.C) + mo[i] * p.ldc + n0) = h;
           if constexpr (TN == 2 && !GEGLU) {
             if (p.stat_out) {
 #pragma unroll
@@ -698,9 +709,9 @@
             }
           }
         } else if (p.c_dt == DT_HL) {
-          if (mok[i]) store_hl8(reinterpret_cast<float*>(p.C) + (size_t)m[i] * p.ldc, n0, w);
+          if (mok[i]) store_hl8(reinterpret_cast<float*>(p.C) + mo[i] * p.ldc, n0, w);
         } else if (mok[i]) {
-          float* cp = reinterpret_cast<float*>(p.C) + (size_t)m[i] * p.ldc + n0;
+          float* cp = reinterpret_cast<float*>(p.C) + mo[i] * p.ldc + n0;
           *reinterpret_cast<f32x4*>(cp) = f32x4{w[0], w[1], w[2], w[3]};
           *reinterpret_cast<f32x4*>(cp + 4) = f32x4{w[4], w[5], w[6], w[7]};
         }
diff --git a/stable-diffusion-xl-burn_amd/csrc/igemm_glds.hip b/stable-diffusion-xl-burn_amd/csrc/igemm_glds.hip
--- a/stable-diffusion-xl-burn_amd/csrc/igemm_glds.hip
+++ b/stable-diffusion-xl-burn_amd/csrc/igemm_glds.hip
@@ -186,6 +186,8 @@
   if ((size_t)p.N * p.K > (size_t)p.M * p.Cin) { tn = bid / tilesM; tm = bid - tn * tilesM; }
   else { tm = bid / tilesN; tn = bid - tm * tilesN; }
   const int m0 = tm * BM, n0 = tn * BN;
+  const int ph = p.ph_rows ? m0 / p.ph_rows : 0;
+  const int mph = ph * p.ph_rows, pady = p.pad - (ph >> 1), padx = p.pad - (ph & 1);
   bool tsw_swapped = false;
   if constexpr (TSW) {
     const int ok = n0 >= p.n_split && n0 + BN <= p.N && p.c_dt == DT_F16 && p.act == 0 && !p.epi_staged && (p.rpb % BM) == 0 && m0 + BM <= p.M &&
@@ -203,7 +205,7 @@
 #pragma unroll
   for (int j = 0; j < BJ; ++j) {
     const int row = (j * NW + wave) * 8 + lrow;
-    wptr[j] = reinterpret_cast<const T*>(p.W) + (size_t)(n0 + row) * p.Kpad + (slot ^ ((row >> 1) & 7)) * CE;
+    wptr[j] = reinterpret_cast<const T*>(reinterpret_cast<const char*>(p.W) + (size_t)ph * p.ph_wbytes) + (size_t)(n0 + row) * p.Kpad + (slot ^ ((row >> 1) & 7)) * CE;
   }
   const int nk_all = p.Kpad / KT;
   const int kbeg = SK > 1 ? (int)((long)slice * nk_all / SK) : 0;
@@ -241,9 +243,10 @@
     if (!lin_rows) {
       if (m < p.M) {
         int b, rem, oy;
-        if (pow2) { b = m >> sh_hw; rem = m & (HWo - 1); oy = rem >> sh_w; }
-        else { b = m / HWo; rem = m - b * HWo; oy = rem / p.Wout; }
-        rb[j] = b; ry[j] = oy * p.stride - p.pad; rx[j] = (rem - oy * p.Wout) * p.stride - p.pad;
+        const int ml = m - mph;
+        if (pow2) { b = ml >> sh_hw; rem = ml & (HWo - 1); oy = rem >> sh_w; }
+        else { b = ml / HWo; rem = ml - b * HWo; oy = rem / p.Wout; }
+        rb[j] = b; ry[j] = oy * p.stride - pady; rx[j] = (rem - oy * p.Wout) * p.stride - padx;
       } else { rb[j] = -1; ry[j] = -(1 << 28); rx[j] = 0; }
     }
   }
@@ -442,7 +445,7 @@
 #pragma unroll
     for (int i = 0; i < TM; ++i) {
       const int m = m0 + wm * WM + i * 32 + fr;
-      const int be = p.a_scale_rpb > 0 ? (m < p.M ? m : p.M - 1) / p.a_scale_rpb : 0;
+      const int be = p.a_scale_rpb > 0 ? ((m < p.M ? m : p.M - 1) - mph) / p.a_scale_rpb : 0;
       lnA[i] = wsc * (p.a_scale ? p.a_scale[be] : 1.f); lnC[i] = 0.f;
     }
     const int wx = (p.acc_scale && p.hl_wexact_ok && p.acc_scale[1] != 0.f) ? 1 : 0;
diff --git a/stable-diffusion-xl-burn_amd/csrc/kernels.h b/stable-diffusion-xl-burn_amd/csrc/kernels.h
--- a/stable-diffusion-xl-burn_amd/csrc/kernels.h
+++ b/stable-diffusion-xl-burn_amd/csrc/kernels.h
@@ -45,6 +45,7 @@
   int epi_staged;
   void* shadow; int shadow_ld; const float* shadow_gamma;
   float shadow_lo_scale;
+  int ph_rows; unsigned ph_wbytes;
 };
 struct SelectKnobs {
   int igemm_variant = 0;
@@ -76,6 +77,7 @@
 bool igemm_wreg_selected(const IgemmParams& p, const SelectKnobs& k);
 bool igemm_wreg_xattn_selected(const IgemmParams& p, const SelectKnobs& k);
 bool igemm_xattn_ok(int a_dt, int c_dt, int M, int N, int K, int rpb, int n_ctx);
+bool igemm_phase_ok(const IgemmParams& p, int compute_dt, const SelectKnobs& k);
 size_t xattn_pack_bytes(int B, int C);
 void launch_xattn_pack(const void* K, const void* Vt, void* out, int B, int C, int n_ctx, int vt_ld, hipStream_t s);
 int igemm_splitk_slices(const IgemmParams& p);
@@ -253,6 +255,7 @@
 void launch_beta_dot(const float* w, const float* beta, const float* bias, float* out, int K, int N, hipStream_t s);
 void launch_pack_conv(const float* src, void* dst, int dt, int Cout, int Cin, int ks, int Kpad, int Npad,
                       hipStream_t s, float wscale = 1.0f);
+void launch_fold_upsample(const float* src, float* dst, int Cout, int Cin, hipStream_t s);
 void launch_absmax(const float* src, size_t n, float* out_dev, hipStream_t s, bool accumulate = false);
 void launch_pack_bias(const float* src, float* dst, int N, int Npad, int geglu, int n_offset, hipStream_t s);
 
diff --git a/stable-diffusion-xl-burn_amd/csrc/select.cpp b/stable-diffusion-xl-burn_amd/csrc/select.cpp
--- a/stable-diffusion-xl-burn_amd/csrc/select.cpp
+++ b/stable-diffusion-xl-burn_amd/csrc/select.cpp
@@ -88,6 +88,25 @@
     if (cost < best) { best = cost; number = n; }
   }
   if (number == 36 && nk >= 40) number = 44;
+  return number;
+}
+
+bool phase_shape_ok(const IgemmParams& p, int kt) {
+  if (p.ph_rows <= 0 || p.ph_wbytes == 0 || p.B <= 0 || p.ph_rows != p.B * p.Hin * p.Win || p.M != 4 * p.ph_rows) return false;
+  if (p.ksize != 2 || p.stride != 1 || p.up != 0 || p.pad != 1 || p.Hout != p.Hin || p.Wout != p.Win) return false;
+  if ((p.Hin * p.Win) % 128 != 0 || p.Cin % kt != 0 || p.K != 4 * p.Cin || p.Kpad != p.K) return false;
+  return p.act == 0 && p.n_split >= p.N && !p.R && !p.ebias && !p.stat_out && !p.gn_part && !p.ln_stat && !p.xa_k && !p.shadow;
+}
+int pick_phase_tile(const IgemmParams& p, int nk, bool hl) {
+  double best = 1e300;
+  int number = 36;
+  for (int n : {35, 36, 38, 49}) {
+    const Tile& t = tile(n);
+    if (p.ph_rows % t.bm != 0 || !tile_takes(t, p) || (hl && n == 38)) continue;
+    const double cost = tile_cost(p.M, p.N, nk, t.bm, t.bn, t.w);
+    if (cost < best) { best = cost; number = n; }
+  }
+  if (!hl && number == 36 && nk >= 40) number = 44;
   return number;
 }
 
@@ -179,6 +198,11 @@
   if (p.stat_out && (v == 2 || v == 5 || v == 19 || v == 38)) return false;
   const bool was_auto = v == 0;
   const int nk = p.Kpad / 64;
+  if (p.ph_rows) {
+    if (!phase_shape_ok(p, 64)) throw std::runtime_error("igemm: the phase form of an upsample convolution was given a launch it does not take");
+    c = from_tile(pick_phase_tile(p, nk, false), DT_F16, p);
+    return true;
+  }
   if (p.xa_k) {
     if (p.act != 0 || p.n_split < p.N || p.stat_out || p.R || p.ebias ||
         !igemm_xattn_ok(p.a_dt, p.c_dt, p.M, p.N, p.K, p.rpb, p.xa_nctx))
@@ -268,6 +292,11 @@
     if (p.n_split < p.N && ((p.ct_ld & 15) != 0 || (p.rpb & 7) != 0 || (p.M % 8) != 0 || misaligned16(p.Ct))) return false;
   }
   if (p.ebias && (p.ebias_ld & 3) != 0) return false;
+  if (p.ph_rows) {
+    if (!phase_shape_ok(p, 32)) throw std::runtime_error("igemm: the phase form of an upsample convolution was given a launch it does not take");
+    c = from_tile(pick_phase_tile(p, p.Kpad / 32, true), DT_HL, p);
+    return true;
+  }
   const int t96mode = k.hl_tile96;
   const bool splitk = (t96mode & 16) && igemm_splitk_slices(p) > 1;
   const bool plain160 = p.N % 160 == 0 && p.n_split >= p.N && !p.stat_out && p.act == 0;
@@ -346,6 +375,11 @@
   return a_dt == DT_F16 && (c_dt == DT_F16 || c_dt == DT_HL) && M > 0 && N % 64 == 0 && K % 64 == 0 && rpb > 0 && rpb % 64 == 0 && M % rpb == 0 &&
          n_ctx >= 1 && n_ctx <= 96;
 }
+bool igemm_phase_ok(const IgemmParams& p, int compute_dt, const SelectKnobs& k) {
+  if (k.igemm_variant < 0 || !phase_shape_ok(p, compute_dt == DT_HL ? 32 : 64)) return false;
+  IgemmChoice c{};
+  return compute_dt == DT_F16 ? select_f16(p, 0, k, c) : (compute_dt == DT_HL && select_hl(p, k, c));
+}
 bool igemm_wreg_selected(const IgemmParams& p, const SelectKnobs& k) { return wreg_takes(p, k, false) && k.igemm_wreg && wreg_pair_grid_fits(p); }
 bool igemm_wreg_xattn_selected(const IgemmParams& p, const SelectKnobs& k) {
   return wreg_takes(p, k, true) && k.igemm_wreg && k.wreg_xattn && wreg_pair_grid_fits(p);
@@ -357,6 +391,7 @@
   const int v = k.igemm_variant;
   if (compute_dt == DT_F16 && v >= 0 && select_f16(p, v, k, c)) return c;
   if (compute_dt == DT_F16 && v > 0 && select_f16(p, 0, k, c)) return c;
+  if (p.ph_rows && compute_dt != DT_HL) throw std::runtime_error("the phase form of an upsample convolution needs the f16 / split-operand direct-to-LDS kernels (igemm_phase_ok)");
   if (p.shadow && compute_dt != DT_F16) throw std::runtime_error("an f16 shadow output needs an f16 GEMM (weights-in-registers kernel)");
   if (compute_dt == DT_F32 && v >= 0 && select_f32(p, k, c)) return c;
   if (compute_dt == DT_HL) {
diff --git a/stable-diffusion-xl-burn_amd/csrc/unet.cpp b/stable-diffusion-xl-burn_amd/csrc/unet.cpp
--- a/stable-diffusion-xl-burn_amd/csrc/unet.cpp
+++ b/stable-diffusion-xl-burn_amd/csrc/unet.cpp
@@ -275,7 +275,7 @@
     x2 = x2 || pl.qkv == LF_X2 || pl.out1 == LF_X2 || pl.q2 == LF_X2 || pl.out2 == LF_X2 || pl.geglu == LF_X2 || pl.ff == LF_X2;
     attn16_ = attn16_ || pl.attn_f16;
   }
-  size_t bound = WeightBuilder::arena_bound(specs, cdt_);
+  size_t bound = WeightBuilder::arena_bound(specs, cdt_, true, fuse_ln_);
   if (x2)
     for (const ParamSpec& ps : specs) if (ps.kind == PK_LINEAR_W) bound += round_up(ps.shape[1], 128) * round_up((size_t)ps.shape[0], 64) * 4 + 256;
   warena_.reserve(bound);
@@ -295,7 +295,7 @@
       default:
         b.res = load_res(wb, p + ".res", d.c_in, d.c_out, emb_names, emb_off);
         if (d.kind == BK_REST || d.kind == BK_RESTU) b.st = load_st(wb, p + ".transformer", d.c_out, d.n_head, d.depth, fuse_ln_, plans[sti++]);
-        if (d.kind == BK_RESTU || d.kind == BK_RESU) b.conv = wb.conv(p + ".upsample.conv");
+        if (d.kind == BK_RESTU || d.kind == BK_RESU) b.conv = wb.conv(p + ".upsample.conv", fuse_ln_);
     }
     return b;
   };
@@ -677,7 +677,9 @@
       res_block(ex, b.res, cat[j], B, h, w, dest);
     }
     if (up) {
-      run_conv(ex, b.conv, hl_op(ex, b.conv, dest, (size_t)B * h * w, b.d.c_out, DM_CONV_UPDOWN, B), b.d.c_out, ConvGeom{B, h, w, 2 * h, 2 * w, 3, 1, 1, 1}, next, tag_epi(DM_CONV_UPDOWN));
+      Epi up_epi = tag_epi(DM_CONV_UPDOWN);
+      up_epi.fold = true;
+      run_conv(ex, b.conv, hl_op(ex, b.conv, dest, (size_t)B * h * w, b.d.c_out, DM_CONV_UPDOWN, B), b.d.c_out, ConvGeom{B, h, w, 2 * h, 2 * w, 3, 1, 1, 1}, next, up_epi);
       h *= 2; w *= 2;
     }
     ex.act->reset(mk);
diff --git a/stable-diffusion-xl-burn_amd/csrc/upsample_fold.h b/stable-diffusion-xl-burn_amd/csrc/upsample_fold.h
--- /dev/null
+++ b/stable-diffusion-xl-burn_amd/csrc/upsample_fold.h
@@ -0,0 +1,35 @@
+#pragma once
+#include <stddef.h>
+
+#if defined(__HIPCC__)
+#define SDXL_HD __host__ __device__
+#else
+#define SDXL_HD
+#endif
+
+namespace sdxl {
+
+SDXL_HD inline int fold_first(int a, int d) { return a == 0 ? (d == 0 ? 0 : 1) : (d == 0 ? 0 : 2); }
+SDXL_HD inline int fold_count(int a, int d) { return (a == 0) == (d == 0) ? 1 : 2; }
+
+SDXL_HD inline float fold_tap(const float* w9, int a, int b, int dy, int dx) {
+  const int y0 = fold_first(a, dy), ny = fold_count(a, dy), x0 = fold_first(b, dx), nx = fold_count(b, dx);
+  float acc = w9[y0 * 3 + x0];
+  for (int ky = y0; ky < y0 + ny; ++ky)
+    for (int kx = x0; kx < x0 + nx; ++kx)
+      if (ky != y0 || kx != x0) acc = acc + w9[ky * 3 + kx];
+  return acc;
+}
+
+SDXL_HD inline float fold_element(const float* w, size_t pairs, size_t e) {
+  const size_t ph = e / (pairs * 4), r = e - ph * pairs * 4, pair = r >> 2;
+  const int tap = (int)(r & 3);
+  return fold_tap(w + pair * 9, (int)(ph >> 1), (int)(ph & 1), tap >> 1, tap & 1);
+}
+
+inline void fold_upsample_weights(const float* w, float* out, size_t cout, size_t cin) {
+  const size_t pairs = cout * cin;
+  for (size_t e = 0; e < 16 * pairs; ++e) out[e] = fold_element(w, pairs, e);
+}
+
+}
diff --git a/stable-diffusion-xl-burn_amd/csrc/vae.cpp b/stable-diffusion-xl-burn_amd/csrc/vae.cpp
--- a/stable-diffusion-xl-burn_amd/csrc/vae.cpp
+++ b/stable-diffusion-xl-burn_amd/csrc/vae.cpp
@@ -26,7 +26,7 @@
     : cfg_(cfg), cdt_(compute_dt) {
   const std::vector<ParamSpec> dspecs = vae_decoder_param_specs(cfg_), especs = vae_encoder_param_specs(cfg_);
   size_t bound = 0;
-  if (dec_src) bound += WeightBuilder::arena_bound(dspecs, cdt_, false);
+  if (dec_src) bound += WeightBuilder::arena_bound(dspecs, cdt_, false, cdt_ == DT_HL);
   if (enc_src) bound += WeightBuilder::arena_bound(especs, cdt_, false);
   warena_.reserve(bound + 4096);
   if (dec_src) {
@@ -42,7 +42,7 @@
       b.r[1] = load_res(wb, p + ".res2", cfg_.dec[i].second, cfg_.dec[i].second);
       b.r[2] = load_res(wb, p + ".res3", cfg_.dec[i].second, cfg_.dec[i].second);
       b.has_up = i + 1 != cfg_.dec.size();
-      if (b.has_up) b.up = wb.conv(p + ".upsampler");
+      if (b.has_up) b.up = wb.conv(p + ".upsampler", cdt_ == DT_HL);
       d_blocks_.push_back(b);
     }
     d_norm_out_ = wb.norm("decoder.norm_out");
@@ -187,7 +187,7 @@
   run_conv(ex, d_conv_in_, z, 4, ConvGeom{n, h, w, h, w, 3, 1, 1, 0}, cur);
   mid(ex, d_mid_, cur, n, h, w);
   for (size_t i = 0; i < d_blocks_.size(); ++i) {
-    const DecBlk& b = d_blocks_[i];
+    DecBlk& b = d_blocks_[i];
     const int co = cfg_.dec[i].second;
     const size_t M = (size_t)n * h * w;
     Act next = b.has_up ? ex.alloc(4 * M, co, ex.sdt) : ex.alloc(M, co, ex.sdt);
@@ -198,7 +198,17 @@
     res_block(ex, b.r[1], a, n, h, w, bb);
     if (b.has_up) {
       res_block(ex, b.r[2], bb, n, h, w, a);
-      run_conv(ex, b.up, hl_operand(ex, b.up, a, M, co, n), co, ConvGeom{n, h, w, 2 * h, 2 * w, 3, 1, 1, 1}, next);
+      Epi eu;
+      if (!ex.dry && b.up.w_fold) {
+        if (b.up_fold < 0) {
+          float sc[2] = {0.f, 0.f};
+          SDXL_HIP(hipMemcpyAsync(sc, b.up.acc_scale, sizeof(sc), hipMemcpyDeviceToHost, ex.s));
+          SDXL_HIP(hipStreamSynchronize(ex.s));
+          b.up_fold = sc[1] == 0.f ? 1 : 0;
+        }
+        eu.fold = b.up_fold == 1;
+      }
+      run_conv(ex, b.up, hl_operand(ex, b.up, a, M, co, n), co, ConvGeom{n, h, w, 2 * h, 2 * w, 3, 1, 1, 1}, next, eu);
       h *= 2; w *= 2;
     } else {
       res_block(ex, b.r[2], bb, n, h, w, next);
diff --git a/stable-diffusion-xl-burn_amd/csrc/weights.cpp b/stable-diffusion-xl-burn_amd/csrc/weights.cpp
--- a/stable-diffusion-xl-burn_amd/csrc/weights.cpp
+++ b/stable-diffusion-xl-burn_amd/csrc/weights.cpp
@@ -1,5 +1,6 @@
 #include "engine.h"
 
+#include <atomic>
 #include <cstdio>
 #include <cstdlib>
 #include <cstring>
@@ -146,7 +147,7 @@
 }
 WeightBuilder::~WeightBuilder() { if (tmp) (void)hipFree(tmp); if (tmp2) (void)hipFree(tmp2); }
 
-size_t WeightBuilder::arena_bound(const std::vector<ParamSpec>& specs, int dt, bool wfrag) {
+size_t WeightBuilder::arena_bound(const std::vector<ParamSpec>& specs, int dt, bool wfrag, bool fold_up) {
   size_t total = 1 << 20;
   for (const ParamSpec& p : specs) {
     if (p.kind == PK_LINEAR_W) total += round_up(p.shape[1], 128) * round_up(p.shape[0], 64) * dt_size(dt) + 768;
@@ -157,6 +158,9 @@
     if (p.kind == PK_LINEAR_W) total += round_up(p.shape[1], 128) * 4 + 256;
     if (wfrag && dt == DT_F16 && p.kind == PK_LINEAR_W) total += round_up(p.shape[1], 128) * round_up(p.shape[0], 64) * 2 + 256;
     if (wfrag && dt == DT_F16 && p.kind == PK_CONV_W && p.shape[2] == 1) total += round_up(p.shape[0], 128) * round_up((size_t)p.shape[1], 64) * 2 + 256;
+    auto ends_with = [&](const char* t) { const size_t n = std::strlen(t); return p.name.size() >= n && p.name.compare(p.name.size() - n, n, t) == 0; };
+    if (fold_up && (ends_with(".upsample.conv.weight") || ends_with(".upsampler.weight")) && folds_upsample(p, dt))
+      total += 4 * round_up(p.shape[0], 128) * 4 * (size_t)p.shape[1] * dt_size(dt) + 768;
   }
   return total;
 }
@@ -173,12 +177,14 @@
   last_fetched = name;
   return tmp;
 }
-float WeightBuilder::hl_scale(Lin& l, const std::vector<std::string>& weight_names) {
-  float* sc = (float*)arena.alloc(2 * sizeof(float));
-  l.acc_scale = sc;
-  if (src.empty()) return 1.f;
+template <typename Each>
+static float hl_scale_over(WeightBuilder& wb, const float*& acc_scale, Each each) {
+  float* sc = (float*)wb.arena.alloc(2 * sizeof(float));
+  acc_scale = sc;
+  if (wb.src.empty()) return 1.f;
+  hipStream_t st = wb.st;
   SDXL_HIP(hipMemsetAsync(sc, 0, 2 * sizeof(float), st));
-  for (const std::string& n : weight_names) launch_absmax(fetch(n), spec(n).numel(), sc, st, true);
+  each([&](const float* t, size_t n) { launch_absmax(t, n, sc, st, true); });
   float h = 0.f;
   SDXL_HIP(hipMemcpyAsync(&h, sc, sizeof(float), hipMemcpyDeviceToHost, st));
   SDXL_HIP(hipStreamSynchronize(st));
@@ -189,8 +195,14 @@
   SDXL_HIP(hipMemcpyAsync(sc, &inv, sizeof(float), hipMemcpyHostToDevice, st));
   SDXL_HIP(hipStreamSynchronize(st));
   bool first = true;
-  for (const std::string& n : weight_names) { launch_f16_exact(fetch(n), spec(n).numel(), wscale, sc + 1, st, !first); first = false; }
+  each([&](const float* t, size_t n) { launch_f16_exact(t, n, wscale, sc + 1, st, !first); first = false; });
   return wscale;
+}
+float WeightBuilder::hl_scale(Lin& l, const std::vector<std::string>& weight_names) {
+  return hl_scale_over(*this, l.acc_scale, [&](auto f) { for (const std::string& n : weight_names) f(fetch(n), spec(n).numel()); });
+}
+float WeightBuilder::hl_scale_of(const float* dev, size_t n, const float*& acc_scale) {
+  return hl_scale_over(*this, acc_scale, [&](auto f) { f(dev, n); });
 }
 
 void WeightBuilder::attach_wfrag(Lin& l, bool fill, bool folded) {
@@ -358,7 +370,10 @@
   else launch_colsum_packed(w, dt, l.Kpad, l.Npad, cs, st);
   return l;
 }
-Lin WeightBuilder::conv(const std::string& name) {
+bool WeightBuilder::folds_upsample(const ParamSpec& p, int dt) {
+  return p.kind == PK_CONV_W && p.shape[2] == 3 && p.shape[3] == 3 && ((dt == DT_F16 && p.shape[1] % 64 == 0) || (dt == DT_HL && p.shape[1] % 32 == 0));
+}
+Lin WeightBuilder::conv(const std::string& name, bool fold_up) {
   const ParamSpec& s = spec(name + ".weight");
   Lin l; l.N = s.shape[0]; l.cin = s.shape[1]; l.ksize = s.shape[2];
   l.K = l.cin * l.ksize * l.ksize;
@@ -370,8 +385,21 @@
   float* b = (float*)arena.alloc((size_t)l.Npad * sizeof(float));
   l.w = w; l.b = b;
   const float wscale = wdt == DT_HL ? hl_scale(l, {name + ".weight"}) : 1.f;
+  const bool fold = fold_up && folds_upsample(s, wdt);
+  const size_t fold_numel = 16 * (size_t)l.N * l.cin, fold_kpad = 4 * (size_t)l.cin;
+  char* wfold = fold ? (char*)arena.alloc(4 * l.Npad * fold_kpad * dt_size(wdt)) : nullptr;
+  l.w_fold = wfold;
+  if (fold && !src.empty() && fold_numel > tmp2_numel) {
+    if (tmp2) SDXL_HIP(hipFree(tmp2));
+    SDXL_HIP(hipMalloc((void**)&tmp2, fold_numel * sizeof(float)));
+    tmp2_numel = fold_numel;
+  }
+  if (fold && !src.empty()) launch_fold_upsample(fetch(name + ".weight"), tmp2, l.N, l.cin, st);
+  const float fscale = fold && wdt == DT_HL ? hl_scale_of(tmp2, fold_numel, l.fold_acc_scale) : 1.f;
   if (src.empty()) { attach_wfrag(l, false); return l; }
   launch_pack_conv(fetch(name + ".weight"), w, wdt, l.N, l.cin, l.ksize, l.Kpad, l.Npad, st, wscale);
+  for (int ph = 0; fold && ph < 4; ++ph)
+    launch_pack_conv(tmp2 + (size_t)ph * 4 * l.N * l.cin, wfold + (size_t)ph * l.Npad * fold_kpad * dt_size(wdt), wdt, l.N, l.cin, 2, (int)fold_kpad, l.Npad, st, fscale);
   launch_pack_bias(fetch(name + ".bias"), b, l.N, l.Npad, 0, 0, st);
   attach_wfrag(l, true);
   return l;
@@ -418,6 +446,8 @@
     std::fprintf(stderr, "[warm] %zu entries, %.1f MB read per forward, %.1f MB of it warmed\n", n, tb / 1048576.0, cb / 1048576.0);
   }
 }
+static std::atomic<int> g_upsample_fold{1};
+void set_upsample_fold(int v) { g_upsample_fold = v; }
 bool run_conv(Exec& ex, const Lin& w, const Act& a, int cin, const ConvGeom& g, const Act& out, const Epi& e) {
   if (ex.dry) return false;
   SDXL_REQUIRE(cin == w.cin, "run_conv: channel mismatch");
@@ -454,6 +484,17 @@
     if (!ok) { p.shadow = nullptr; p.shadow_gamma = nullptr; p.stat_out = nullptr; p.shadow_lo_scale = 0.f; }
     if (e.shadow_done) *e.shadow_done = ok;
   }
+  size_t wbytes_f16 = (size_t)w.Npad * w.Kpad * 2;
+  if (g.up == 1 && e.fold && w.w_fold && g_upsample_fold.load() && g.ksize == 3 && g.stride == 1 && g.pad == 1 && g.Hout == 2 * g.Hin && g.Wout == 2 * g.Win) {
+    const int wdt_ = w.dt >= 0 ? w.dt : ex.cdt;
+    IgemmParams q = p;
+    q.W = w.w_fold; q.Wf = nullptr; q.acc_scale = w.fold_acc_scale;
+    q.ksize = 2; q.up = 0; q.Hout = g.Hin; q.Wout = g.Win; q.K = q.Kpad = 4 * cin;
+    q.ph_rows = g.B * g.Hin * g.Win; q.ph_wbytes = (unsigned)((size_t)w.Npad * q.Kpad * dt_size(wdt_));
+    q.a_scale_rpb = p.a_scale_rpb / 4;
+    if (igemm_phase_ok(q, wdt_, knobs)) { p = q; wbytes_f16 = 4 * (size_t)w.Npad * q.Kpad * 2; }
+  }
+  if (e.fold_done) *e.fold_done = p.ph_rows != 0;
   SDXL_REQUIRE(!e.xa_k || igemm_xattn_ok(a.dt, out.dt, p.M, p.N, p.K, p.rpb, e.xa_nctx), "fused cross-attention: unsupported shape");
   SDXL_REQUIRE(!e.ln_stat || (w.ln_k ? w.ln_k : w.K) % 64 == 0, "LayerNorm-folded GEMM needs K % 64 == 0");
   SDXL_REQUIRE(!e.stat_out || (w.N % 64 == 0 && (e.n_split < 0 || e.n_split >= w.N) && e.act == 0), "row statistics need a plain N % 64 == 0 output");
@@ -464,7 +505,7 @@
   if (ex.warm && (w.dt >= 0 ? w.dt : ex.cdt) == DT_F16) {
     WarmSeq& ws = *ex.warm;
     const bool host = igemm_wreg_selected(p, knobs) || igemm_wreg_xattn_selected(p, knobs);
-    const size_t wbytes = (size_t)w.Npad * w.Kpad * 2;
+    const size_t wbytes = wbytes_f16;
     const char* lo; const char* hi;
     if (host) {
       const char* f = reinterpret_cast<const char*>(p.Wf), *b = reinterpret_cast<const char*>(w.b);
```

Result: faster. 1.414 images/sec, median of 6 (+1.1%).
